# crispitagorico/sigkernel

Hardware: AMD Instinct MI355X
Metric: Gram entries/sec (fp64) (higher is better)
Workload: dtype f64; 1 GPU; BASELINE configs[2]: batch 512x512, len 128, dim 8, LinearKernel, dyadic 1, fp64, compute_Gram sym=False; step=compute_Gram, batch_x=512, rows_per_gpu=512, batch_y=512, len_x=128, len_y=128, dim=8, static_kernel=linear, dyadic_order=1, parallelism=SigKernel(process_group): gram rows sharded over 1 GPU(s), 1 all-gather per Gram

## Files before the change

include/sigkernel_amd.h:

```cpp
#ifndef SIGKERNEL_AMD_H
#define SIGKERNEL_AMD_H

#include <stddef.h>
#include <stdint.h>

#ifdef __cplusplus
extern "C" {
#endif

typedef enum sk_status {
    SK_OK = 0,
    SK_ERR_BAD_ARG = 1,
    SK_ERR_UNSUPPORTED = 2,
    SK_ERR_LAUNCH = 3,
    SK_ERR_WORKSPACE = 4,
    SK_ERR_NO_DEVICE = 5
} sk_status;

#define SK_SCHEME_DEFAULT 0
#define SK_SCHEME_NAIVE 1

#define SK_FLAG_NONE 0
#define SK_FLAG_EXACT 1
#define SK_FLAG_SIMPLE 2
// ... 50 lines not shown
int sk_static_adjoint_f64(int kind, double param, const double *X, const double *Y, const double *W, int64_t ldw,
                          const double *scale, int64_t A, int64_t B, int M, int N, int D, double *out, void *stream);
int sk_static_adjoint_f32(int kind, double param, const float *X, const float *Y, const float *W, int64_t ldw,
                          const float *scale, int64_t A, int64_t B, int M, int N, int D, float *out, void *stream);

int sk_static_adjoint_param_f64(int kind, double param, const double *X, const double *Y, const double *W, int64_t ldw,
                                const double *scale, int64_t A, int64_t B, int M, int N, int D, double *out_dX, double *out_partials,
                                int64_t *n_partials, void *stream);

int sk_linear_adjoint_f64(const double *dYt, int64_t ldy, const double *W, int64_t ldw, const double *scale, int64_t A,
                          int64_t B, int Mc, int Nc, int D, double *out, void *stream);
int sk_linear_adjoint_f32(const double *dYt, int64_t ldy, const float *W, int64_t ldw, const float *scale, int64_t A, int64_t B,
                          int Mc, int Nc, int D, float *out, void *stream);

int sk_linear_adjoint_fused_f64(const double *dXr, const double *dYt, int64_t A, int64_t B, int Mrows, int Mc, int Nc, int Ncp,
                                int dyadic, int scheme, const double *edges, const double *scale, double *tpart,
                                size_t tpart_doubles, double *err, double *ypart, size_t ypart_doubles, int *ppg_out, int *rows_out,
                                int *ycols_out, const double *kfinal, double screen, double tol, void *rescue_ws,
                                size_t rescue_ws_bytes, void *stream);

int sk_rbf_adjoint_fused_f64(const double *Xr, const double *Yt, int64_t A, int64_t B, int Mrows, int Mc, int Nc, int Ncp, int D,
                             int dyadic, int scheme, double sigma, const double *edges, const double *scale, double *gpart,
                             size_t gpart_doubles, double *err, double *ypart, size_t ypart_doubles, int *ppg_out, int *rows_out,
                             int *outw_out, int *ycols_out, const double *kfinal, double screen, double tol, void *rescue_ws,
                             size_t rescue_ws_bytes, void *stream);

size_t sk_solve_deriv_static_workspace_bytes(int64_t P, int Mc, int Nc, int dyadic, int D, int *mrows);
int sk_solve_deriv_static_f64(int kind, double param, const double *X0r, const double *X1r, const double *X2r, const double *Yt, int64_t A,
                              int64_t B, int Mrows, int Mc, int Nc, int Ncp, int D, int fd, int dyadic, int scheme, double eps, double *out_k,
                              double *out_kd, double *out_kdd, void *workspace, size_t workspace_bytes, void *stream);

int sk_rbf_adjoint_fused_mb_layout(int64_t P, int Mc, int Nc, int dyadic, int D, int *mrows, int *rows, int *outw, int *ncols,
                                   int64_t *edge_doubles, size_t *workspace_bytes);
int sk_rbf_adjoint_fused_mb_f64(const double *Xr, const void *Yt, int yt_f32, int64_t A, int64_t B, int Mrows, int Mc, int Nc, int Ncp, int D, int fd,
                                int dyadic, int scheme, double sigma, const double *edges, const double *scale, double *gpart,
                                size_t gpart_doubles, double *n0, size_t n0_doubles, double *err, void *workspace, size_t workspace_bytes,
                                const double *yt64, const double *kfinal, double screen, double tol, void *rescue_ws, size_t rescue_ws_bytes,
                                void *stream);

int sk_linear_adjoint_fused_mb_layout(int64_t P, int Mc, int Nc, int dyadic, int D, int *mrows, int *rows, int *outw, int64_t *edge_doubles,
                                      size_t *workspace_bytes);
int sk_linear_adjoint_fused_mb_f64(const double *dXr, const double *dYt, int64_t A, int64_t B, int Mrows, int Mc, int Nc, int Ncp, int D, int fd,
                                   int dyadic, int scheme, const double *edges, const double *scale, double *gpart, size_t gpart_doubles,
                                   double *err, void *workspace, size_t workspace_bytes, const double *kfinal, double screen, double tol,
                                   void *rescue_ws, size_t rescue_ws_bytes, void *stream);

size_t sk_fused_rescue_workspace_bytes(int kind, int64_t P, int Mc, int Nc, int dyadic, int blocks);

int sk_static_adjoint2_f64(int kind, double param, const double *X, const double *Y, const double *dXr, int Mrows,
                           const double *W, int64_t ldw, const double *scale, int64_t A, int64_t B, int b0, int M, int N, int D,
                           double *out, void *stream);
int sk_static_adjoint2_f32(int kind, double param, const float *X, const float *Y, const double *dXr, int Mrows, const float *W,
                           int64_t ldw, const float *scale, int64_t A, int64_t B, int b0, int M, int N, int D, float *out,
                           void *stream);

int sk_increments_adjoint_f64(const double *W, int64_t ldw, const double *scale, int64_t P, int M, int N, double *dG,
                              void *stream);
int sk_increments_adjoint_f32(const float *W, int64_t ldw, const float *scale, int64_t P, int M, int N, float *dG,
                              void *stream);

int sk_prep_paths_f64(const double *X, int64_t A, int M, int D, int diff, int dim_major, double scale, double *out, int rows, int fd,
                      void *stream);
int sk_prep_paths_f32(const float *X, int64_t A, int M, int D, int diff, int dim_major, double scale, double *out, int rows, int fd,
                      void *stream);
int sk_prep_pair_f64(const double *X, int64_t A, int M, const double *Y, int64_t B, int N, int D, int diff, double scale_x, double scale_y,
                     double *out_x, int rows_x, double *out_y, int rows_y, int fd, void *stream);
int sk_prep_pair_f32(const float *X, int64_t A, int M, const float *Y, int64_t B, int N, int D, int diff, double scale_x, double scale_y,
                     double *out_x, int rows_x, double *out_y, int rows_y, int fd, void *stream);

int sk_solve_fwd_f64(const double *inc_c, int64_t ld, int64_t P, int Mc, int Nc, int dyadic, int scheme, int flags,
                     double *out_final, double *out_grid, double *out_edges, void *stream);
int sk_solve_fwd_f32(const float *inc_c, int64_t ld, int64_t P, int Mc, int Nc, int dyadic, int scheme, int flags,
                     float *out_final, float *out_grid, double *out_edges, void *stream);

int sk_solve_fwd_linear_f64(const double *dXr, const double *dYt, int64_t A, int64_t B, int Mrows, int Mc, int Nc, int Ncp, int D,
                            int dyadic, int scheme, double *out_final, void *queue, void *stream);
int sk_solve_fwd_linear_f32(const double *dXr, const double *dYt, int64_t A, int64_t B, int Mrows, int Mc, int Nc, int Ncp, int D,
                            int dyadic, int scheme, float *out_final, void *queue, void *stream);

int sk_solve_fwd_rbf_f64(const double *Xr, const double *Yt, int64_t A, int64_t B, int Mrows, int Mc, int Nc, int Ncp, int D,
                         int dyadic, int scheme, double inv_sigma, double *out_final, void *queue, void *stream);
int sk_solve_fwd_rbf_f32(const double *Xr, const double *Yt, int64_t A, int64_t B, int Mrows, int Mc, int Nc, int Ncp, int D,
                         int dyadic, int scheme, double inv_sigma, float *out_final, void *queue, void *stream);
int sk_solve_prefix_linear_f64(const double *dXr, const double *dYt, int64_t A, int64_t B, int Mrows, int Mc, int Nc, int Ncp, int D,
                               int dyadic, int scheme, double *out, int64_t ldo, void *queue, void *stream);
int sk_solve_prefix_linear_f32(const double *dXr, const double *dYt, int64_t A, int64_t B, int Mrows, int Mc, int Nc, int Ncp, int D,
                               int dyadic, int scheme, float *out, int64_t ldo, void *queue, void *stream);
int sk_solve_prefix_rbf_f64(const double *Xr, const double *Yt, int64_t A, int64_t B, int Mrows, int Mc, int Nc, int Ncp, int D,
                            int dyadic, int scheme, double inv_sigma, double *out, int64_t ldo, void *queue, void *stream);
int sk_solve_prefix_rbf_f32(const double *Xr, const double *Yt, int64_t A, int64_t B, int Mrows, int Mc, int Nc, int Ncp, int D,
                            int dyadic, int scheme, double inv_sigma, float *out, int64_t ldo, void *queue, void *stream);
#define SK_NODES_ALL 0
#define SK_NODES_DIAGONAL 1
#define SK_NODES_LAST_ROW 2
#define SK_NODES_LAST_COL 3
int sk_solve_prefix_nodes_linear_f64(const double *dXr, const double *dYt, int64_t A, int64_t B, int Mrows, int Mc, int Nc, int Ncp, int D,
                                     int dyadic, int scheme, int nodes, double *out, int64_t ldo, void *queue, void *stream);
int sk_solve_prefix_nodes_linear_f32(const double *dXr, const double *dYt, int64_t A, int64_t B, int Mrows, int Mc, int Nc, int Ncp, int D,
                                     int dyadic, int scheme, int nodes, float *out, int64_t ldo, void *queue, void *stream);
int sk_solve_prefix_nodes_rbf_f64(const double *Xr, const double *Yt, int64_t A, int64_t B, int Mrows, int Mc, int Nc, int Ncp, int D,
                                  int dyadic, int scheme, double inv_sigma, int nodes, double *out, int64_t ldo, void *queue, void *stream);
int sk_solve_prefix_nodes_rbf_f32(const double *Xr, const double *Yt, int64_t A, int64_t B, int Mrows, int Mc, int Nc, int Ncp, int D,
                                  int dyadic, int scheme, double inv_sigma, int nodes, float *out, int64_t ldo, void *queue, void *stream);
#define SK_NODES_AT 4
int sk_solve_prefix_at_linear_f64(const double *dXr, const double *dYt, int64_t A, int64_t B, int Mrows, int Mc, int Nc, int Ncp, int D,
                                  int dyadic, int scheme, const int *len_x, const int *len_y, double *out, void *queue, void *stream);
int sk_solve_prefix_at_linear_f32(const double *dXr, const double *dYt, int64_t A, int64_t B, int Mrows, int Mc, int Nc, int Ncp, int D,
                                  int dyadic, int scheme, const int *len_x, const int *len_y, float *out, void *queue, void *stream);
int sk_solve_prefix_at_rbf_f64(const double *Xr, const double *Yt, int64_t A, int64_t B, int Mrows, int Mc, int Nc, int Ncp, int D,
                               int dyadic, int scheme, double inv_sigma, const int *len_x, const int *len_y, double *out, void *queue,
                               void *stream);
int sk_solve_prefix_at_rbf_f32(const double *Xr, const double *Yt, int64_t A, int64_t B, int Mrows, int Mc, int Nc, int Ncp, int D,
                               int dyadic, int scheme, double inv_sigma, const int *len_x, const int *len_y, float *out, void *queue,
                               void *stream);
int sk_truncated_gram_f64(const double *Xr, const double *Yt, int64_t A, int64_t B, int Mrows, int M, int N, int Ncp, int D, int fd,
                          int num_levels, int order, const double *sigma, double *out, void *stream);
int sk_truncated_gram_f32(const double *Xr, const double *Yt, int64_t A, int64_t B, int Mrows, int M, int N, int Ncp, int D, int fd,
                          int num_levels, int order, const double *sigma, float *out, void *stream);
int sk_truncated_paired_f64(const double *Xr, const double *Yt, int64_t P, int Mrows, int M, int N, int Ncp, int D, int fd, int num_levels,
                            int order, const double *sigma, double *out, void *stream);
int sk_truncated_paired_f32(const double *Xr, const double *Yt, int64_t P, int Mrows, int M, int N, int Ncp, int D, int fd, int num_levels,
                            int order, const double *sigma, float *out, void *stream);
int sk_truncated_levels_f64(const double *Xr, const double *Yt, int64_t A, int64_t B, int Mrows, int M, int N, int Ncp, int D, int fd,
                            int num_levels, int order, double *out, void *stream);
int sk_truncated_levels_f32(const double *Xr, const double *Yt, int64_t A, int64_t B, int Mrows, int M, int N, int Ncp, int D, int fd,
                            int num_levels, int order, float *out, void *stream);
int sk_truncated_levels_paired_f64(const double *Xr, const double *Yt, int64_t P, int Mrows, int M, int N, int Ncp, int D, int fd,
                                   int num_levels, int order, double *out, void *stream);
int sk_truncated_levels_paired_f32(const double *Xr, const double *Yt, int64_t P, int Mrows, int M, int N, int Ncp, int D, int fd,
                                   int num_levels, int order, float *out, void *stream);
int sk_truncated_points_f64(const double *Xr, const double *Yt, int64_t A, int64_t B, int Mrows, int M, int N, int Ncp, int D, int fd,
                            int num_levels, int order, int kind, double param, int paired, int levels, const double *sigma, double *out,
                            void *stream);
int sk_truncated_points_f32(const double *Xr, const double *Yt, int64_t A, int64_t B, int Mrows, int M, int N, int Ncp, int D, int fd,
                            int num_levels, int order, int kind, double param, int paired, int levels, const double *sigma, float *out,
                            void *stream);
int sk_truncated_long_plan(int64_t A, int64_t B, int M, int N, int D, int num_levels, int paired, size_t workspace_bytes, int64_t *plan);
int sk_truncated_long_f64(const double *Xr, const double *Yt, int64_t A, int64_t B, int Mrows, int M, int N, int Ncp, int D, int fd,
                          int num_levels, int order, int paired, int levels, const double *sigma, double *slab, size_t slab_bytes, double *out,
                          void *stream);
int sk_truncated_long_f32(const double *Xr, const double *Yt, int64_t A, int64_t B, int Mrows, int M, int N, int Ncp, int D, int fd,
                          int num_levels, int order, int paired, int levels, const double *sigma, double *slab, size_t slab_bytes, float *out,
                          void *stream);
int sk_truncated_long_adjoint_plan(int64_t A, int64_t B, int M, int N, int D, int num_levels, int paired, size_t workspace_bytes,
                                   int64_t *plan);
int sk_truncated_long_adjoint(const double *Xr, const double *Yt, int64_t A, int64_t B, int Mrows, int M, int N, int Ncp, int D, int fd,
                              int num_levels, const double *w, double *Tpart, int64_t n_chunks, double *slab, size_t slab_bytes, void *stream,
                              int paired);
int sk_truncated_wide_adjoint_plan(int64_t A, int64_t B, int M, int N, int D, int num_levels, int paired, size_t workspace_bytes,
                                   int64_t *plan);
int sk_truncated_wide_adjoint(const double *Xr, const double *Yt, int64_t A, int64_t B, int Mrows, int M, int N, int Ncp, int D, int fd,
                              int num_levels, const double *w, double *Tpart, int64_t n_chunks, double *slab, size_t slab_bytes, void *stream,
                              int paired);
int sk_truncated_adjoint_plan(int64_t A, int64_t B, int M, int N, int D, int num_levels, int paired, size_t workspace_bytes, int64_t *plan);
int sk_truncated_adjoint(const double *Xr, const double *Yt, int64_t A, int64_t B, int Mrows, int M, int N, int Ncp, int D, int fd,
                         int num_levels, const double *w, double *Tpart, int64_t n_chunks, double *slab, size_t slab_bytes, void *stream,
                         int paired);
int sk_truncated_points_adjoint_plan(int64_t A, int64_t B, int M, int N, int D, int num_levels, int paired, size_t workspace_bytes,
                                     int64_t *plan);
int sk_truncated_points_adjoint(const double *Xr, const double *Yt, int64_t A, int64_t B, int Mrows, int M, int N, int Ncp, int D, int fd,
                                int num_levels, double param, const double *w, double *Tpart, int64_t n_chunks, double *slab,
                                size_t slab_bytes, void *stream, int paired);
int sk_solve_fwd_linear_sym_f64(const double *dXr, const double *dXt, const int *pair_tab, int64_t A, int Mrows, int Mc, int Nc, int Ncp, int D, int dyadic,
                                int scheme, double *out, void *queue, void *stream);
int sk_solve_fwd_linear_sym_f32(const double *dXr, const double *dXt, const int *pair_tab, int64_t A, int Mrows, int Mc, int Nc, int Ncp, int D, int dyadic,
                                int scheme, float *out, void *queue, void *stream);
// ... 79 lines not shown
```

sigkernel_amd/_lib.py:

```python
import ctypes
import os

import torch

from ._routes import routes

_HERE = os.path.dirname(os.path.abspath(__file__))
LIB_PATH = os.path.join(_HERE, "libsigkernel_amd.so")

SK_OK = 0
OP_FORWARD, OP_ADJOINT, OP_ADJOINT_SYM, OP_PREFIX, OP_TRUNCATED, OP_TRUNCATED_ADJOINT, OP_TRUNCATED_RBF = 0, 1, 2, 3, 4, 5, 6
OP_TRUNCATED_RBF_ADJOINT = 7
OP_TRUNCATED_LONG = 8
OP_TRUNCATED_LONG_ADJOINT = 9
OP_TRUNCATED_WIDE_ADJOINT = 10
ROUTE_STREAM, ROUTE_FUSED, ROUTE_FUSED_MB, ROUTE_FUSED_MB_SWAP, ROUTE_FUSED_SWAP = 0, 1, 2, 3, 4
ROUTE_NO_STREAM = 1
ROUTE_NO_SWAP = 2
SCHEME_DEFAULT = 0
SCHEME_NAIVE = 1
FLAG_EXACT = 1
FLAG_SIMPLE = 2
FLAG_FAST_ONLY = 4
FLAG_EDGES_GIVEN = 8
FLAG_DISCRETE = 16
FLAG_RAGGED = 32
FLAG_SOURCES = 64
PREFIX_NODES = {"all": 0, "diagonal": 1, "last_row": 2, "last_col": 3}


def prefix_nodes_len(nodes, M, N):
    return {"diagonal": min(M, N), "last_row": N, "last_col": M}[nodes]

_lib = None

_vp = ctypes.c_void_p
_i64 = ctypes.c_int64
_int = ctypes.c_int
_sz = ctypes.c_size_t

SIGNATURES = {
    "sk_version": (_int, []),
    "sk_build_info": (ctypes.c_char_p, []),
    "sk_route_query": (_int, [_int, _int, _int, _int, _int, _int, _int, _int, _int]),
    "sk_cost_query": (ctypes.c_double, [_int]),
    "sk_cost_name": (ctypes.c_char_p, [_int]),
    "sk_cost_note": (ctypes.c_char_p, [_int]),
    "sk_solve_fwd_static_cols": (_int, [_int, _int]),
    "sk_reload_knobs": (None, []),
    "sk_launch_trace": (_int, [_int]),
    "sk_launch_trace_dump": (ctypes.c_size_t, [ctypes.c_char_p, ctypes.c_size_t, _int]),
    "sk_linear_prescale": (ctypes.c_double, [_int]),
    "sk_pair_div_magic": (_int, [_i64, ctypes.POINTER(ctypes.c_uint32), ctypes.POINTER(ctypes.c_int)]),
    "sk_status_string": (ctypes.c_char_p, [_int]),
    "sk_device_count": (_int, []),
    "sk_increments_f64": (_int, [_vp, _i64, _int, _int, _vp, _i64, _vp]),
    "sk_increments_f32": (_int, [_vp, _i64, _int, _int, _vp, _i64, _vp]),
    "sk_static_increments_f64": (_int, [_int, ctypes.c_double, _vp, _vp, _i64, _i64, _int, _int, _int, _vp, _i64, _vp]),
    "sk_static_increments_f32": (_int, [_int, ctypes.c_double, _vp, _vp, _i64, _i64, _int, _int, _int, _vp, _i64, _vp]),
    "sk_static_adjoint_f64": (_int, [_int, ctypes.c_double, _vp, _vp, _vp, _i64, _vp, _i64, _i64, _int, _int, _int, _vp, _vp]),
    "sk_static_adjoint_f32": (_int, [_int, ctypes.c_double, _vp, _vp, _vp, _i64, _vp, _i64, _i64, _int, _int, _int, _vp, _vp]),
    "sk_static_adjoint_param_f64": (_int, [_int, ctypes.c_double, _vp, _vp, _vp, _i64, _vp, _i64, _i64, _int, _int, _int, _vp, _vp,
                                           ctypes.POINTER(ctypes.c_int64), _vp]),
    "sk_linear_adjoint_f64": (_int, [_vp, _i64, _vp, _i64, _vp, _i64, _i64, _int, _int, _int, _vp, _vp]),
    "sk_linear_adjoint_f32": (_int, [_vp, _i64, _vp, _i64, _vp, _i64, _i64, _int, _int, _int, _vp, _vp]),
    "sk_static_adjoint2_f64": (_int, [_int, ctypes.c_double, _vp, _vp, _vp, _int, _vp, _i64, _vp, _i64, _i64, _int, _int, _int, _int,
                                      _vp, _vp]),
    "sk_static_adjoint2_f32": (_int, [_int, ctypes.c_double, _vp, _vp, _vp, _int, _vp, _i64, _vp, _i64, _i64, _int, _int, _int, _int,
                                      _vp, _vp]),
    "sk_increments_adjoint_f64": (_int, [_vp, _i64, _vp, _i64, _int, _int, _vp, _vp]),
    "sk_increments_adjoint_f32": (_int, [_vp, _i64, _vp, _i64, _int, _int, _vp, _vp]),
    "sk_solve_fwd_f64": (_int, [_vp, _i64, _i64, _int, _int, _int, _int, _int, _vp, _vp, _vp, _vp]),
    "sk_solve_fwd_f32": (_int, [_vp, _i64, _i64, _int, _int, _int, _int, _int, _vp, _vp, _vp, _vp]),
    "sk_solve_fwd_linear_f64": (_int, [_vp, _vp, _i64, _i64, _int, _int, _int, _int, _int, _int, _int, _vp, _vp, _vp]),
    "sk_solve_fwd_linear_f32": (_int, [_vp, _vp, _i64, _i64, _int, _int, _int, _int, _int, _int, _int, _vp, _vp, _vp]),
    "sk_solve_fwd_rbf_f64": (_int, [_vp, _vp, _i64, _i64, _int, _int, _int, _int, _int, _int, _int, ctypes.c_double, _vp, _vp, _vp]),
    "sk_solve_fwd_rbf_f32": (_int, [_vp, _vp, _i64, _i64, _int, _int, _int, _int, _int, _int, _int, ctypes.c_double, _vp, _vp, _vp]),
    "sk_solve_prefix_linear_f64": (_int, [_vp, _vp, _i64, _i64, _int, _int, _int, _int, _int, _int, _int, _vp, _i64, _vp, _vp]),
    "sk_solve_prefix_linear_f32": (_int, [_vp, _vp, _i64, _i64, _int, _int, _int, _int, _int, _int, _int, _vp, _i64, _vp, _vp]),
    "sk_solve_prefix_rbf_f64": (_int, [_vp, _vp, _i64, _i64, _int, _int, _int, _int, _int, _int, _int, ctypes.c_double, _vp, _i64, _vp, _vp]),
    "sk_solve_prefix_rbf_f32": (_int, [_vp, _vp, _i64, _i64, _int, _int, _int, _int, _int, _int, _int, ctypes.c_double, _vp, _i64, _vp, _vp]),
    "sk_solve_prefix_nodes_linear_f64": (_int, [_vp, _vp, _i64, _i64, _int, _int, _int, _int, _int, _int, _int, _int, _vp, _i64, _vp, _vp]),
    "sk_solve_prefix_nodes_linear_f32": (_int, [_vp, _vp, _i64, _i64, _int, _int, _int, _int, _int, _int, _int, _int, _vp, _i64, _vp, _vp]),
    "sk_solve_prefix_nodes_rbf_f64": (_int, [_vp, _vp, _i64, _i64, _int, _int, _int, _int, _int, _int, _int, ctypes.c_double, _int, _vp, _i64, _vp, _vp]),
    "sk_solve_prefix_nodes_rbf_f32": (_int, [_vp, _vp, _i64, _i64, _int, _int, _int, _int, _int, _int, _int, ctypes.c_double, _int, _vp, _i64, _vp, _vp]),
    "sk_solve_prefix_at_linear_f64": (_int, [_vp, _vp, _i64, _i64, _int, _int, _int, _int, _int, _int, _int, _vp, _vp, _vp, _vp, _vp]),
    "sk_solve_prefix_at_linear_f32": (_int, [_vp, _vp, _i64, _i64, _int, _int, _int, _int, _int, _int, _int, _vp, _vp, _vp, _vp, _vp]),
    "sk_solve_prefix_at_rbf_f64": (_int, [_vp, _vp, _i64, _i64, _int, _int, _int, _int, _int, _int, _int, ctypes.c_double, _vp, _vp, _vp, _vp, _vp]),
    "sk_solve_prefix_at_rbf_f32": (_int, [_vp, _vp, _i64, _i64, _int, _int, _int, _int, _int, _int, _int, ctypes.c_double, _vp, _vp, _vp, _vp, _vp]),
    "sk_truncated_gram_f64": (_int, [_vp, _vp, _i64, _i64, _int, _int, _int, _int, _int, _int, _int, _int, _vp, _vp, _vp]),
    "sk_truncated_gram_f32": (_int, [_vp, _vp, _i64, _i64, _int, _int, _int, _int, _int, _int, _int, _int, _vp, _vp, _vp]),
    "sk_truncated_paired_f64": (_int, [_vp, _vp, _i64, _int, _int, _int, _int, _int, _int, _int, _int, _vp, _vp, _vp]),
    "sk_truncated_paired_f32": (_int, [_vp, _vp, _i64, _int, _int, _int, _int, _int, _int, _int, _int, _vp, _vp, _vp]),
    "sk_truncated_levels_f64": (_int, [_vp, _vp, _i64, _i64, _int, _int, _int, _int, _int, _int, _int, _int, _vp, _vp]),
    "sk_truncated_levels_f32": (_int, [_vp, _vp, _i64, _i64, _int, _int, _int, _int, _int, _int, _int, _int, _vp, _vp]),
    "sk_truncated_levels_paired_f64": (_int, [_vp, _vp, _i64, _int, _int, _int, _int, _int, _int, _int, _int, _vp, _vp]),
    "sk_truncated_levels_paired_f32": (_int, [_vp, _vp, _i64, _int, _int, _int, _int, _int, _int, _int, _int, _vp, _vp]),
    "sk_truncated_points_f64": (_int, [_vp, _vp, _i64, _i64, _int, _int, _int, _int, _int, _int, _int, _int, _int, ctypes.c_double, _int, _int, _vp, _vp, _vp]),
    "sk_truncated_points_f32": (_int, [_vp, _vp, _i64, _i64, _int, _int, _int, _int, _int, _int, _int, _int, _int, ctypes.c_double, _int, _int, _vp, _vp, _vp]),
    "sk_truncated_long_plan": (_int, [_i64, _i64, _int, _int, _int, _int, _int, _sz, _vp]),
    "sk_truncated_long_f64": (_int, [_vp, _vp, _i64, _i64, _int, _int, _int, _int, _int, _int, _int, _int, _int, _int, _vp, _vp, _sz, _vp, _vp]),
    "sk_truncated_long_f32": (_int, [_vp, _vp, _i64, _i64, _int, _int, _int, _int, _int, _int, _int, _int, _int, _int, _vp, _vp, _sz, _vp, _vp]),
    "sk_truncated_adjoint_plan": (_int, [_i64, _i64, _int, _int, _int, _int, _int, _sz, _vp]),
    "sk_truncated_long_adjoint_plan": (_int, [_i64, _i64, _int, _int, _int, _int, _int, _sz, _vp]),
    "sk_truncated_long_adjoint": (_int, [_vp, _vp, _i64, _i64, _int, _int, _int, _int, _int, _int, _int, _vp, _vp, _i64, _vp, _sz, _vp, _int]),
    "sk_truncated_wide_adjoint_plan": (_int, [_i64, _i64, _int, _int, _int, _int, _int, _sz, _vp]),
    "sk_truncated_wide_adjoint": (_int, [_vp, _vp, _i64, _i64, _int, _int, _int, _int, _int, _int, _int, _vp, _vp, _i64, _vp, _sz, _vp, _int]),
    "sk_truncated_adjoint": (_int, [_vp, _vp, _i64, _i64, _int, _int, _int, _int, _int, _int, _int, _vp, _vp, _i64, _vp, _sz, _vp, _int]),
    "sk_truncated_points_adjoint_plan": (_int, [_i64, _i64, _int, _int, _int, _int, _int, _sz, _vp]),
    "sk_truncated_points_adjoint": (_int, [_vp, _vp, _i64, _i64, _int, _int, _int, _int, _int, _int, _int, ctypes.c_double, _vp, _vp, _i64, _vp, _sz,
                                           _vp, _int]),
    "sk_prep_pair_f64": (_int, [_vp, _i64, _int, _vp, _i64, _int, _int, _int, ctypes.c_double, ctypes.c_double, _vp, _int, _vp, _int, _int, _vp]),
    "sk_prep_pair_f32": (_int, [_vp, _i64, _int, _vp, _i64, _int, _int, _int, ctypes.c_double, ctypes.c_double, _vp, _int, _vp, _int, _int, _vp]),
    "sk_solve_fwd_static_workspace_bytes": (_sz, [_int, _i64, _int, _int, _int, _int]),
    "sk_solve_fwd_static_rows": (_int, [_int, _int, _int]),
    "sk_solve_fwd_static_split": (_int, [_int, _i64, _int, _int, _int, _int]),
    "sk_solve_fwd_static_f64": (_int, [_int, ctypes.c_double, _vp, _vp, _i64, _i64, _int, _int, _int, _int, _int, _int, _int, _int, _vp,
                                       _vp, _vp, _sz, _vp]),
    "sk_solve_fwd_static_f32": (_int, [_int, ctypes.c_double, _vp, _vp, _int, _i64, _i64, _int, _int, _int, _int, _int, _int, _int, _int,
                                       _vp, _vp, _vp, _sz, _vp]),
    "sk_solve_deriv_static_workspace_bytes": (_sz, [_i64, _int, _int, _int, _int, _vp]),
    "sk_solve_deriv_static_f64": (_int, [_int, ctypes.c_double, _vp, _vp, _vp, _vp, _i64, _i64, _int, _int, _int, _int, _int, _int, _int, _int,
                                         ctypes.c_double, _vp, _vp, _vp, _vp, _sz, _vp]),
    "sk_linear_adjoint_fused_mb_layout": (_int, [_i64, _int, _int, _int, _int, _vp, _vp, _vp, _vp, _vp]),
    "sk_linear_adjoint_fused_mb_f64": (_int, [_vp, _vp, _i64, _i64, _int, _int, _int, _int, _int, _int, _int, _int, _vp, _vp, _vp, _sz, _vp, _vp,
                                              _sz, _vp, ctypes.c_double, ctypes.c_double, _vp, _sz, _vp]),
    "sk_rbf_adjoint_fused_mb_layout": (_int, [_i64, _int, _int, _int, _int, _vp, _vp, _vp, _vp, _vp, _vp]),
    "sk_rbf_adjoint_fused_mb_f64": (_int, [_vp, _vp, _int, _i64, _i64, _int, _int, _int, _int, _int, _int, _int, _int, ctypes.c_double, _vp, _vp,
                                           _vp, _sz, _vp, _sz, _vp, _vp, _sz, _vp, _vp, ctypes.c_double, ctypes.c_double, _vp, _sz, _vp]),
    "sk_solve_fwd_linear_sym_f64": (_int, [_vp, _vp, _vp, _i64, _int, _int, _int, _int, _int, _int, _int, _vp, _vp, _vp]),
    "sk_solve_fwd_linear_sym_f32": (_int, [_vp, _vp, _vp, _i64, _int, _int, _int, _int, _int, _int, _int, _vp, _vp, _vp]),
    "sk_solve_fwd_rbf_sym_f64": (_int, [_vp, _vp, _vp, _i64, _int, _int, _int, _int, _int, _int, _int, ctypes.c_double, _vp, _vp, _vp]),
    "sk_solve_fwd_rbf_sym_f32": (_int, [_vp, _vp, _vp, _i64, _int, _int, _int, _int, _int, _int, _int, ctypes.c_double, _vp, _vp, _vp]),
    "sk_solve_fwd_rbf_edges_f64": (_int, [_vp, _vp, _i64, _i64, _int, _int, _int, _int, _int, _int, _int, ctypes.c_double, _vp, _vp, _vp, _vp]),
    "sk_solve_fwd_linear_edges_f64": (_int, [_vp, _vp, _i64, _i64, _int, _int, _int, _int, _int, _int, _int, _vp, _vp, _vp, _vp]),
    "sk_linear_adjoint_fused_f64": (_int, [_vp, _vp, _i64, _i64, _int, _int, _int, _int, _int, _int, _vp, _vp, _vp, _sz, _vp, _vp, _sz, _vp,
                                           _vp, _vp, _vp, ctypes.c_double, ctypes.c_double, _vp, _sz, _vp]),
    "sk_rbf_adjoint_fused_f64": (_int, [_vp, _vp, _i64, _i64, _int, _int, _int, _int, _int, _int, _int, ctypes.c_double, _vp, _vp, _vp,
                                        _sz, _vp, _vp, _sz, _vp, _vp, _vp, _vp, _vp, ctypes.c_double, ctypes.c_double, _vp, _sz, _vp]),
    "sk_fused_rescue_workspace_bytes": (_sz, [_int, _i64, _int, _int, _int, _int]),
    "sk_adj_workspace_bytes": (_sz, [_i64, _int, _int, _int, _int, _int]),
    "sk_adj_rescue_slot_bytes": (_sz, [_int, _int, _int]),
    "sk_plan_wave_shares": (_int, [_i64, _int, _i64, _i64, _int, _int, _vp, _vp, _vp]),
    "sk_plan_group_chunks": (_int, [_i64, _i64, _i64, _i64, _int, _int, _int, _i64, _vp, _vp, _vp]),
    "sk_adj_rescue_f64": (_int, [_vp, _i64, _i64, _int, _int, _int, _int, _vp, ctypes.c_double, _vp, _vp, _i64, _vp, _sz, _vp]),
    "sk_adj_rescue_f32": (_int, [_vp, _i64, _i64, _int, _int, _int, _int, _vp, ctypes.c_double, _vp, _vp, _i64, _vp, _sz, _vp]),
    "sk_prep_paths_f64": (_int, [_vp, _i64, _int, _int, _int, _int, ctypes.c_double, _vp, _int, _int, _vp]),
    "sk_prep_paths_f32": (_int, [_vp, _i64, _int, _int, _int, _int, ctypes.c_double, _vp, _int, _int, _vp]),
    "sk_strip_edges_bytes": (_sz, [_i64, _int, _int, _int, _int]),
    "sk_solve_fwd_edges_f64": (_int, [_vp, _i64, _i64, _int, _int, _int, _int, _vp, _vp, _vp]),
    "sk_solve_fwd_edges_f32": (_int, [_vp, _i64, _i64, _int, _int, _int, _int, _vp, _vp, _vp]),
    "sk_solve_adj_f64": (_int, [_vp, _i64, _i64, _int, _int, _int, _int, _int, _vp, _vp, _i64, _vp, _vp, _sz, _vp]),
    "sk_solve_adj_f32": (_int, [_vp, _i64, _i64, _int, _int, _int, _int, _int, _vp, _vp, _i64, _vp, _vp, _sz, _vp]),
    "sk_deriv_increments_f64": (_int, [_vp, _vp, _vp, ctypes.c_double, _i64, _int, _int, _vp, _vp, _vp, _i64, _vp]),
    "sk_deriv_increments_f32": (_int, [_vp, _vp, _vp, ctypes.c_double, _i64, _int, _int, _vp, _vp, _vp, _i64, _vp]),
    "sk_static_deriv_increments_f64": (_int, [_int, ctypes.c_double, _vp, _vp, _vp, _vp, _i64, _i64, _int, _int, _int,
                                              ctypes.c_double, _vp, _vp, _vp, _i64, _vp]),
    "sk_static_deriv_increments_f32": (_int, [_int, ctypes.c_double, _vp, _vp, _vp, _vp, _i64, _i64, _int, _int, _int,
                                              ctypes.c_double, _vp, _vp, _vp, _i64, _vp]),
    "sk_solve_deriv_f64": (_int, [_vp, _vp, _vp, _i64, _i64, _int, _int, _int, _int, _vp, _vp, _vp, _vp]),
# ... 97 lines not shown


def _suffix(t):
    if t.dtype == torch.float64:
        return "f64"
    if t.dtype == torch.float32:
        return "f32"
    raise TypeError("sigkernel_amd supports float64 and float32 tensors, got %s" % t.dtype)


def _dev(t, name):
    if t.device.type != "cuda":
        raise RuntimeError(
            "sigkernel_amd runs on MI355X only: tensor `%s` is on %s; move it to a HIP device "
            "('cuda' in PyTorch-ROCm). There is no CPU fallback." % (name, t.device))
    if not t.is_contiguous():
        raise ValueError("tensor `%s` must be contiguous" % name)
    return t


def _rbf_extra_row(Mc, dyadic):
    rc = 4 >> min(int(dyadic), 2)
    cap = 8 * rc
    while cap < Mc:
        cap *= 2
    return 1 if (cap == Mc and cap < 64 * rc) else 0


def _padded_ld(n, elem_size):
    q = 128 // elem_size
    return (n + q - 1) // q * q


def _row_stride(t, name):
    if t.device.type != "cuda":
        _dev(t, name)
    Mc, Nc = t.shape[-2:]
    if t.dim() >= 2 and t.stride(-1) == 1 and t.stride(-2) >= Nc:
        ld = t.stride(-2)
        expect, ok = Mc * ld, True
        for size, stride in zip(reversed(t.shape[:-2]), reversed(t.stride()[:-2])):
            if size != 1 and stride != expect:
                ok = False
                break
            expect *= size
        if ok:
            return t, ld
    t = t.contiguous()
    return t, Nc


_raw_stream = getattr(torch._C, "_cuda_getCurrentRawStream", None)


def _stream(t):
    if _raw_stream is not None:
        idx = t.device.index
        return _raw_stream(torch.cuda.current_device() if idx is None else idx)
    return torch.cuda.current_stream(t.device).cuda_stream


class _NoGuard:
    def __enter__(self):
        return None

    def __exit__(self, *exc):
        return False


_NO_GUARD = _NoGuard()


def _device(dev):
    idx = dev.index
    if idx is None or idx == torch.cuda.current_device():
        return _NO_GUARD
    return torch.cuda.device(dev)


def _ptr(t):
    return None if t is None else t.data_ptr()


def _queue(dev, pairs=1 << 30):
    return torch.empty(8, dtype=torch.int64, device=dev) if pairs >= 16384 else None


def _prep_paths(X, diff, dim_major, scale, rows, fd=8):
    A, M, D = X.shape
    out = torch.empty((A, fd, rows) if dim_major else (A, rows, fd), dtype=torch.float64, device=X.device)
    fn = getattr(load(), "sk_prep_paths_" + _suffix(X))
    _check(fn(_ptr(X), A, M, D, int(bool(diff)), int(bool(dim_major)), float(scale), _ptr(out), int(rows), int(fd), _stream(X)),
           "sk_prep_paths")
    return out


def _prep_pair(X, Y, diff, scale_x, rows_x, rows_y, fd=8):
    A, M, D = X.shape
    B, N = Y.shape[0], Y.shape[1]
    nx = A * rows_x * fd
    buf = torch.empty(nx + B * fd * rows_y, dtype=torch.float64, device=X.device)
    out_x, out_y = buf[:nx].view(A, rows_x, fd), buf[nx:].view(B, fd, rows_y)
    fn = getattr(load(), "sk_prep_pair_" + _suffix(X))
    _check(fn(_ptr(X), A, M, _ptr(Y), B, N, D, int(bool(diff)), float(scale_x), 1.0, _ptr(out_x), int(rows_x), _ptr(out_y), int(rows_y), int(fd),
              _stream(X)), "sk_prep_pair")
    return out_x, out_y


def _truncated_staging(D, N):
    return (8 if D <= 8 else 16), (N + 15) // 16 * 16


_TRUNCATED_ADJOINTS = {
    "plain": (OP_TRUNCATED_ADJOINT, "sk_truncated_adjoint_plan", "sk_truncated_adjoint"),
    "points": (OP_TRUNCATED_RBF_ADJOINT, "sk_truncated_points_adjoint_plan", "sk_truncated_points_adjoint"),
    "long": (OP_TRUNCATED_LONG_ADJOINT, "sk_truncated_long_adjoint_plan", "sk_truncated_long_adjoint"),
    "wide": (OP_TRUNCATED_WIDE_ADJOINT, "sk_truncated_wide_adjoint_plan", "sk_truncated_wide_adjoint"),
}


class _WorstResidual:
    __slots__ = ("err",)

    def __init__(self, err):
        self.err = err

    def tensor(self):
        return self.err.max()

    def __float__(self):
        return float(self.err.max())


def _pair_gemm_sum(Wv, Yv, scale, gram):
    if not gram:
        T = torch.matmul(Wv, Yv)
        return T * scale[:, None, None] if scale is not None else T
    A, B, R, D = Wv.shape[0], Wv.shape[1], Wv.shape[2], Yv.shape[2]
    step = max(1, int((256 << 20) // max(1, A * R * D * Wv.element_size())))
    T = None
    for b0 in range(0, B, step):
        Tm = torch.matmul(Wv[:, b0:b0 + step], Yv[b0:b0 + step])
        if scale is not None:
            Tm = Tm.mul_(scale[:, b0:b0 + step, None, None])
        T = Tm.sum(1) if T is None else T.add_(Tm.sum(1))
        del Tm
    if T is None:
        T = torch.zeros(A, R, D, dtype=Wv.dtype, device=Wv.device)
    return T


class HipBackend:

    name = "hip"
    last_split_status = None

    @staticmethod
    def route(op, kind, D, M, N, dyadic, naive, elem_size, no_stream=False, no_swap=False):
        return int(load().sk_route_query(int(op), int(kind), int(D), int(M), int(N), int(dyadic), SCHEME_NAIVE if naive else SCHEME_DEFAULT,
                                         int(elem_size), (ROUTE_NO_STREAM if no_stream else 0) | (ROUTE_NO_SWAP if no_swap else 0)))

    def increments(self, G):
        _dev(G, "G")
        M, N = G.shape[-2:]
        P = G.numel() // (M * N)
        ld = _padded_ld(N - 1, G.element_size())
        out = torch.empty(G.shape[:-2] + (M - 1, ld), dtype=G.dtype, device=G.device)
        with _device(G.device):
            fn = getattr(load(), "sk_increments_" + _suffix(G))
            _check(fn(_ptr(G), P, M, N, _ptr(out), ld, _stream(G)), "sk_increments")
        return out[..., : N - 1]

    MAX_FUSED_DIM = 32

    def static_increments(self, kind, param, X, Y, gram):
        _dev(X, "X")
        _dev(Y, "Y")
        A, M, D = X.shape
        B, N = Y.shape[0], Y.shape[1]
        if M < 2 or N < 2:
            return None
        ld = _padded_ld(N - 1, X.element_size())
        shape = (A, B, M - 1, ld) if gram else (A, M - 1, ld)
        out = torch.empty(shape, dtype=X.dtype, device=X.device)
        with _device(X.device):
            fn = getattr(load(), "sk_static_increments_" + _suffix(X))
            _check(fn(int(kind), float(param), _ptr(X), _ptr(Y), A, B if gram else 0, M, N, D, _ptr(out), ld, _stream(X)),
                   "sk_static_increments")
        return out[..., : N - 1]

    def solve_fwd_fused_linear(self, X, Y, scale, dyadic, naive, gram, keep_edges=False):
        _dev(X, "X")
        _dev(Y, "Y")
        A, M, D = X.shape
        B, N = Y.shape[0], Y.shape[1]
        Mc, Nc = M - 1, N - 1
        if D > 8 or dyadic > 2 or Mc < 1 or Nc < 1 or Mc > 64 * (4 >> min(dyadic, 2)):
            return None
        Mrows, Ncp = _stage_rows(0, M, gram), (Nc + 15) // 16 * 16
        dev = X.device
        out = torch.empty((A, B) if gram else (A,), dtype=X.dtype, device=dev)
        scheme = SCHEME_NAIVE if naive else SCHEME_DEFAULT
        lib = load()
        with _device(dev):
            kappa = float(lib.sk_linear_prescale(int(dyadic)))
            dXr, dYt = _prep_pair(X, Y, True, kappa * float(scale) ** 2, Mrows, Ncp)
            if keep_edges and X.dtype == torch.float64 and 0 <= dyadic <= 2:
                P = A * B if gram else A
                nbytes = int(lib.sk_strip_edges_bytes(P, Mc, Nc, int(dyadic), 8))
                if nbytes:
                    edges = torch.empty(nbytes // 8, dtype=torch.float64, device=dev)
                    rc = lib.sk_solve_fwd_linear_edges_f64(_ptr(dXr), _ptr(dYt), A, B if gram else 0, Mrows, Mc, Nc, Ncp, D,
                                                           int(dyadic), scheme, _ptr(out), _ptr(edges), _ptr(_queue(dev, A * B if gram else A)), _stream(X))
                    if rc == SK_OK:
                        return out, edges
                    if rc != 2:
                        _check(rc, "sk_solve_fwd_linear_edges")
            fn = getattr(lib, "sk_solve_fwd_linear_" + _suffix(X))
            rc = fn(_ptr(dXr), _ptr(dYt), A, B if gram else 0, Mrows, Mc, Nc, Ncp, D, int(dyadic), scheme, _ptr(out), _ptr(_queue(dev, A * B if gram else A)), _stream(X))
        if rc == 2:
            return None
        _check(rc, "sk_solve_fwd_linear")
        return (out, None) if keep_edges else out

    def solve_fwd_fused_rbf(self, X, Y, sigma, dyadic, naive, gram, keep_edges=False):
        _dev(X, "X")
        _dev(Y, "Y")
        A, M, D = X.shape
        B, N = Y.shape[0], Y.shape[1]
        Mc, Nc = M - 1, N - 1
        if D > 8 or dyadic > 2 or Mc < 1 or Nc < 1 or M > 64 * (4 >> min(dyadic, 2)) or not float(sigma) > 0:
            return None
        Mrows, Ncp = _stage_rows(1, M, gram), (N + 15) // 16 * 16
        dev = X.device
        out = torch.empty((A, B) if gram else (A,), dtype=X.dtype, device=dev)
        scheme = SCHEME_NAIVE if naive else SCHEME_DEFAULT
        lib = load()
        with _device(dev):
            Xr, Yt = _prep_pair(X, Y, False, 1.0, Mrows, Ncp)
            if keep_edges and X.dtype == torch.float64:
                P = A * B if gram else A
                nbytes = int(lib.sk_strip_edges_bytes(P, Mc + _rbf_extra_row(Mc, dyadic), Nc + (1 if Nc % 16 == 0 else 0), int(dyadic), 8))
                if nbytes:
                    edges = torch.empty(nbytes // 8, dtype=torch.float64, device=dev)
                    rc = lib.sk_solve_fwd_rbf_edges_f64(_ptr(Xr), _ptr(Yt), A, B if gram else 0, Mrows, Mc, Nc, Ncp, D, int(dyadic),
                                                        scheme, 1.0 / float(sigma), _ptr(out), _ptr(edges), _ptr(_queue(dev, A * B if gram else A)), _stream(X))
                    if rc == SK_OK:
                        return out, edges
                    if rc != 2:
                        _check(rc, "sk_solve_fwd_rbf_edges")
            fn = getattr(lib, "sk_solve_fwd_rbf_" + _suffix(X))
            rc = fn(_ptr(Xr), _ptr(Yt), A, B if gram else 0, Mrows, Mc, Nc, Ncp, D, int(dyadic), scheme, 1.0 / float(sigma),
                    _ptr(out), _ptr(_queue(dev, A * B if gram else A)), _stream(X))
        if rc == 2:
            return None
        _check(rc, "sk_solve_fwd_rbf")
        return (out, None) if keep_edges else out

    def solve_prefix_fused(self, kind, param, X, Y, dyadic, naive, gram, out=None, nodes="all"):
        _dev(X, "X")
        _dev(Y, "Y")
        if nodes not in PREFIX_NODES:
            raise ValueError("nodes must be one of %s, not %r" % (", ".join(repr(n) for n in PREFIX_NODES), nodes))
        A, M, D = X.shape
        B, N = Y.shape[0], Y.shape[1]
        Mc, Nc = M - 1, N - 1
        if Mc < 1 or Nc < 1 or (kind == 1 and not float(param) > 0) or \
                self.route(OP_PREFIX, kind, D, M, N, dyadic, naive, X.element_size()) != ROUTE_FUSED:
            return None
        mode = PREFIX_NODES[nodes]
        tail = (M, N) if mode == 0 else (prefix_nodes_len(nodes, M, N),)
        shape = ((A, B) if gram else (A,)) + tail
        if out is None:
            out = torch.empty(shape, dtype=X.dtype, device=X.device)
        if tuple(out.shape) != shape or out.dtype != X.dtype or out.device != X.device:
            raise ValueError("out must be a %s tensor of shape %s on %s" % (X.dtype, shape, X.device))
        if A == 0 or (gram and B == 0):
            return out
        ldo = out.stride(1) if gram else out.stride(0)
        if mode == 0:
            if out.stride(-1) != 1 or out.stride(-2) != N or ldo < M * N or (gram and A > 1 and out.stride(0) != B * ldo):
                raise ValueError("out: every pair's (M, N) grid must be dense and the pairs evenly spaced")
        elif out.stride(-1) != 1 or ldo < tail[0] or (gram and A > 1 and out.stride(0) != B * ldo):
            raise ValueError("out: every pair's slice must be dense and the pairs evenly spaced")
        Mrows = _stage_rows(kind, M, gram)
        Ncp = ((Nc if kind == 0 else N) + 15) // 16 * 16
        dev = X.device
        scheme = SCHEME_NAIVE if naive else SCHEME_DEFAULT
        lib = load()
        pairs = A * B if gram else A
        which = ("sk_solve_prefix_" if mode == 0 else "sk_solve_prefix_nodes_") + ("linear_" if kind == 0 else "rbf_") + _suffix(X)
        sel = () if mode == 0 else (mode,)
        with _device(dev):
            if kind == 0:
                kappa = float(lib.sk_linear_prescale(int(dyadic)))
                dXr, dYt = _prep_pair(X, Y, True, kappa * float(param) ** 2, Mrows, Ncp)
                rc = getattr(lib, which)(_ptr(dXr), _ptr(dYt), A, B if gram else 0, Mrows, Mc, Nc, Ncp, D, int(dyadic), scheme, *sel,
                                         _ptr(out), ldo, _ptr(_queue(dev, pairs)), _stream(X))
            else:
                Xr, Yt = _prep_pair(X, Y, False, 1.0, Mrows, Ncp)
                rc = getattr(lib, which)(_ptr(Xr), _ptr(Yt), A, B if gram else 0, Mrows, Mc, Nc, Ncp, D, int(dyadic), scheme,
                                         1.0 / float(param), *sel, _ptr(out), ldo, _ptr(_queue(dev, pairs)), _stream(X))
        if rc == 2:
            return None
        _check(rc, "sk_solve_prefix")
        if mode == 0:
            out[..., 0, :] = 1
        else:
            out[..., 0] = 1
        return out

    def solve_prefix_at(self, kind, param, X, Y, len_x, len_y, dyadic, naive, gram):
        _dev(X, "X")
        _dev(Y, "Y")
        A, M, D = X.shape
        B, N = Y.shape[0], Y.shape[1]
        Mc, Nc = M - 1, N - 1
        if Mc < 1 or Nc < 1 or (kind == 1 and not float(param) > 0) or \
                self.route(OP_PREFIX, kind, D, M, N, dyadic, naive, X.element_size()) != ROUTE_FUSED:
            return None
        for name, t, n in (("len_x", len_x, A), ("len_y", len_y, B)):
            if t.dtype != torch.int32 or t.device != X.device or tuple(t.shape) != (n,) or not t.is_contiguous():
                raise ValueError("%s must be a contiguous int32 tensor of shape (%d,) on %s" % (name, n, X.device))
        out = torch.ones((A, B) if gram else (A,), dtype=X.dtype, device=X.device)
        if A == 0 or (gram and B == 0):
            return out
        Mrows = _stage_rows(kind, M, gram)
        Ncp = ((Nc if kind == 0 else N) + 15) // 16 * 16
        dev = X.device
        scheme = SCHEME_NAIVE if naive else SCHEME_DEFAULT
        lib = load()
        pairs = A * B if gram else A
        fn = getattr(lib, "sk_solve_prefix_at_" + ("linear_" if kind == 0 else "rbf_") + _suffix(X))
        with _device(dev):
            if kind == 0:
                kappa = float(lib.sk_linear_prescale(int(dyadic)))
# ... 1057 lines not shown
```

sigkernel_amd/csrc/sk_abi.hip:

```cpp
#include <algorithm>
#include <atomic>
#include <cstdlib>
#include <cstring>
#include <mutex>
#include <string>
#include <unordered_map>
#include <utility>
#include <vector>

#include "sk_internal.h"
#include "sk_wave_common.h"

using namespace sk;

namespace {

bool bad_common(const void *inc, int64_t P, int Mc, int Nc, int dyadic, int scheme, int flags) {
    if (!inc || P < 0 || Mc < 1 || Nc < 1 || dyadic < 0 || dyadic > 16) return true;
    if (scheme != SK_SCHEME_DEFAULT && scheme != SK_SCHEME_NAIVE) return true;
    if (flags & ~(SK_FLAG_EXACT | SK_FLAG_SIMPLE | SK_FLAG_FAST_ONLY | SK_FLAG_EDGES_GIVEN)) return true;
    if ((flags & SK_FLAG_EDGES_GIVEN) && (flags & (SK_FLAG_EXACT | SK_FLAG_SIMPLE))) return true;
    if ((flags & SK_FLAG_FAST_ONLY) && (flags & (SK_FLAG_EXACT | SK_FLAG_SIMPLE))) return true;
    if (((int64_t)Mc << dyadic) > (1 << 24) || ((int64_t)Nc << dyadic) > (1 << 24)) return true;
    return false;
// ... 133 lines not shown
template <typename TO>
int solve_prefix_at(int kind, const double *Xr, const double *Yt, int64_t A, int64_t B, int Mrows, int Mc, int Nc, int Ncp, int D, int dyadic,
                    int scheme, double inv_sigma, const int *len_x, const int *len_y, TO *out, void *queue, void *stream) {
    if (D < 1 || !Xr || !Yt || !out || A < 0 || B < 0 || Mc < 1 || Nc < 1 || dyadic < 0 || dyadic > 16) return SK_ERR_BAD_ARG;
    if (scheme != SK_SCHEME_DEFAULT && scheme != SK_SCHEME_NAIVE) return SK_ERR_BAD_ARG;
    if (kind == 1 && (!(inv_sigma > 0.0) || !(inv_sigma < 1e300))) return SK_ERR_BAD_ARG;
    if (!len_x || !len_y) return SK_ERR_BAD_ARG;
    if (A == 0) return SK_OK;
    const Geom g = make_geom(B > 0 ? A * B : A, Mc, Nc, dyadic, scheme);
    return launch_fwd_prefix<TO>(kind, Xr, Yt, A, B, Mrows, Ncp, D, g, inv_sigma, out, 1, queue, (hipStream_t)stream, SK_NODES_AT, len_x, len_y);
}

template <typename TO>
int truncated(const double *Xr, const double *Yt, int64_t A, int64_t B, int Mrows, int M, int N, int Ncp, int D, int fd, int num_levels,
              int order, const double *sigma, TO *out, void *stream, int paired, int levels, int kind = 0, double param = 0.0,
              bool long_mode = false, double *slab = nullptr, size_t slab_bytes = 0) {
    if (paired) B = A;
    if ((kind != 0 && kind != 1) || (long_mode && kind) || (kind == 1 && (!(param > 0.0) || !(param < 1e300)))) return SK_ERR_BAD_ARG;
    if (D < 1 || !Xr || !Yt || !out || (!sigma && !levels) || A < 0 || B < 0 || M < 1 || N < 1 || num_levels < 1 || Mrows < M || Ncp < N ||
        fd < D || (slab_bytes && !slab))
        return SK_ERR_BAD_ARG;
    if (A == 0 || B == 0) return SK_OK;
    if (long_mode)
        return launch_truncated_long<TO>(Xr, Yt, A, B, Mrows, M, N, Ncp, D, fd, num_levels, order, sigma, out, (hipStream_t)stream, paired, levels,
                                         slab, slab_bytes);
    return launch_truncated<TO>(Xr, Yt, A, B, Mrows, M, N, Ncp, D, fd, num_levels, order, sigma, out, (hipStream_t)stream, paired, levels, kind,
                                param);
}

int truncated_adjoint_plan_abi(int mode, int64_t A, int64_t B, int M, int N, int D, int num_levels, int paired, size_t workspace_bytes,
                               int64_t *plan, bool block_entry) {
    if (!plan || A < 1 || B < 1 || M < 1 || N < 1 || D < 1 || num_levels < 1) return SK_ERR_BAD_ARG;
    size_t block = 0;
    const int rc = truncated_adjoint_plan(mode, A, B, M, N, D, num_levels, paired, workspace_bytes, plan, plan + 1, &block);
    if (rc == SK_OK) {
        plan[2] = plan[1] * (int64_t)block;
        if (block_entry) plan[3] = (int64_t)block;
    }
    return rc;
}

int truncated_adjoint_abi(int mode, const double *Xr, const double *Yt, int64_t A, int64_t B, int Mrows, int M, int N, int Ncp, int D, int fd,
                          int num_levels, double param, const double *w, double *Tpart, int64_t n_chunks, double *slab, size_t slab_bytes,
                          void *stream, int paired, bool pairs_must_match, bool slab_required, bool param_required) {
    if (paired && !pairs_must_match) B = A;
    if (D < 1 || !Xr || !Yt || !w || !Tpart || A < 0 || B < 0 || M < 1 || N < 1 || num_levels < 1 || Mrows < M || Ncp < N || fd < D ||
        (slab_required ? !slab || !slab_bytes : slab_bytes && !slab) || (paired && A != B) || (param_required && !(param > 0.0)))
        return SK_ERR_BAD_ARG;
    if (A == 0 || B == 0) return SK_OK;
    return launch_truncated_adjoint(mode, Xr, Yt, A, B, Mrows, M, N, Ncp, D, fd, num_levels, param, w, Tpart, n_chunks, slab, slab_bytes,
                                    (hipStream_t)stream, paired);
}

}

namespace sk {
namespace {
int knob_int(const char *name) {
    const char *v = getenv(name);
    return v && *v ? atoi(v) : 0;
}
RankW knob_shares(const char *name) {
    RankW r{};
    const char *e = getenv(name);
    if (e && *e)
        for (const char *q = e; *q && r.n < 4; ++r.n) {
            r.w[r.n] = atof(q);
            while (*q && *q != ',') ++q;
            if (*q == ',') ++q;
        }
    return r;
}
Knobs parse_knobs() {
    Knobs k{};
    k.wave_wpc = knob_int("SK_WAVE_WPC"); k.wave_wpb = knob_int("SK_WAVE_WPB");
    k.adj_wpc = knob_int("SK_ADJ_WPC"); k.adj_wpb = knob_int("SK_ADJ_WPB");
    k.adjf_wpc = knob_int("SK_ADJF_WPC"); k.adjf_wpb = knob_int("SK_ADJF_WPB");
    k.adjr_wpc = knob_int("SK_ADJR_WPC"); k.adjr_wpb = knob_int("SK_ADJR_WPB");
    k.adjmb_wpc = knob_int("SK_ADJMB_WPC"); k.adjmb_wpb = knob_int("SK_ADJMB_WPB"); k.adjmb_q_static = knob_int("SK_ADJMB_Q_STATIC");
    k.derivf_wpc = knob_int("SK_DERIVF_WPC"); k.derivf_wpb = knob_int("SK_DERIVF_WPB"); k.derivf_noshift = knob_int("SK_DERIVF_NOSHIFT");
    k.deriv_wpc = knob_int("SK_DERIV_WPC"); k.deriv_wpb = knob_int("SK_DERIV_WPB");
    k.fused_wpc = knob_int("SK_FUSED_WPC"); k.fused_wpb = knob_int("SK_FUSED_WPB"); k.fused_q_static = knob_int("SK_FUSED_Q_STATIC");
    k.fused_mid = getenv("SK_FUSED_MID") ? knob_int("SK_FUSED_MID") : 1;
    k.fusedmb_wpc = knob_int("SK_FUSEDMB_WPC"); k.fusedmb_wpb = knob_int("SK_FUSEDMB_WPB"); k.fusedmb_q_static = knob_int("SK_FUSEDMB_Q_STATIC");
    k.fusedmb_split = getenv("SK_FUSEDMB_SPLIT") ? knob_int("SK_FUSEDMB_SPLIT") : 1;
    k.fusedmb_lead = knob_int("SK_FUSEDMB_LEAD");
    k.prefix_store = knob_int("SK_PREFIX_STORE");
    k.rank_w = knob_shares("SK_RANK_W"); k.wave_rank_w = knob_shares("SK_WAVE_RANK_W"); k.adj_rank_w = knob_shares("SK_ADJ_RANK_W");
    k.adjf_rank_w = knob_shares("SK_ADJF_RANK_W"); k.adjr_rank_w = knob_shares("SK_ADJR_RANK_W");
    k.deriv_rank_w = knob_shares("SK_DERIV_RANK_W"); k.fused_rank_w = knob_shares("SK_FUSED_RANK_W");
    k.fusedmb_rank_w = knob_shares("SK_FUSEDMB_RANK_W");
    return k;
}
Knobs g_knobs = parse_knobs();
std::atomic<int> g_cu_count[16];
std::atomic<int> g_trace{knob_int("SK_TRACE_LAUNCHES") != 0 ? 1 : 0};
std::mutex g_trace_mu;
std::unordered_map<const void *, unsigned long long> g_trace_counts;
}
const Knobs &knobs() { return g_knobs; }
bool trace_on() { return g_trace.load(std::memory_order_relaxed) != 0; }
void trace_launch(const void *host_stub) {
    std::lock_guard<std::mutex> lock(g_trace_mu);
    g_trace_counts[host_stub] += 1;
}
int device_cu_count() {
    int dev = 0;
    if (hipGetDevice(&dev) != hipSuccess || dev < 0 || dev >= 16) return 256;
    int n = g_cu_count[dev].load(std::memory_order_relaxed);
    if (n == 0) {
        int v = 0;
        n = hipDeviceGetAttribute(&v, hipDeviceAttributeMultiprocessorCount, dev) == hipSuccess && v > 0 ? v : 256;
        g_cu_count[dev].store(n, std::memory_order_relaxed);
    }
    return n;
}
}

extern "C" {

int sk_version(void) { return 340; }

int sk_launch_trace(int enable) {
    const int prev = sk::g_trace.load(std::memory_order_relaxed);
    if (enable == 0 || enable == 1) sk::g_trace.store(enable, std::memory_order_relaxed);
    return prev;
}

size_t sk_launch_trace_dump(char *buf, size_t n, int reset) {
    std::string out;
    {
        std::lock_guard<std::mutex> lock(sk::g_trace_mu);
        std::vector<std::pair<std::string, unsigned long long>> rows;
        for (const auto &kv : sk::g_trace_counts) {
            const char *name = hipKernelNameRefByPtr(kv.first, nullptr);
            rows.emplace_back(name ? name : "?", kv.second);
        }
        std::sort(rows.begin(), rows.end());
        for (const auto &r : rows) out += std::to_string(r.second) + "\t" + r.first + "\n";
        if (reset) sk::g_trace_counts.clear();
    }
    if (buf && n) {
        const size_t c = out.size() < n - 1 ? out.size() : n - 1;
        memcpy(buf, out.data(), c);
        buf[c] = 0;
    }
    return out.size() + 1;
}

void sk_reload_knobs(void) { sk::g_knobs = sk::parse_knobs(); }

double sk_linear_prescale(int dyadic) { return dyadic < 0 || dyadic > 16 ? 0.0 : 1.0 / ((double)(1LL << (2 * dyadic)) * 3.4641016151377544); }

int sk_plan_wave_shares(int64_t P, int G, int64_t waves, int64_t resident, int wpb, int n_cu, int64_t *first, int64_t *end, int *ppg) {
    if (P < 0 || G < 1 || waves < 1 || wpb < 1 || n_cu < 1 || !first || !end || !ppg) return SK_ERR_BAD_ARG;
    const sk::RankSplit rs = sk::rank_split(P, G, waves, resident, wpb, n_cu, sk::RankW{});
    for (int64_t w = 0; w < waves; ++w) sk::rank_share(rs, w, G, P, ppg[w], first[w], end[w]);
    return rs.nranks;
}

int sk_plan_group_chunks(int64_t A, int64_t B, int64_t PPG, int64_t max_groups, int G, int wpb, int n_cu, int64_t n_groups,
                         int64_t *first, int64_t *slot, int *ppg) {
    if (A < 1 || B < 0 || PPG < 1 || G < 1 || wpb < 1 || n_cu < 1 || !first || !slot || !ppg) return SK_ERR_BAD_ARG;
    const sk::ChunkSplit cs = sk::chunk_split(A, B, PPG, max_groups, G, wpb, n_cu, sk::RankW{});
    const int64_t P = B > 0 ? A * B : A;
    for (int64_t gi = 0; gi < n_groups; ++gi) sk::chunk_share(cs, gi, A, B, P, first[gi], slot[gi], ppg[gi]);
// ... 52 lines not shown
                                         (hipStream_t)stream);
}
int sk_static_adjoint_f32(int kind, double param, const float *X, const float *Y, const float *W, int64_t ldw,
                          const float *scale, int64_t A, int64_t B, int M, int N, int D, float *out, void *stream) {
    if (!X || !Y || !W || !out || A < 0 || B < 0 || M < 2 || N < 2 || D < 1 || (kind != 0 && kind != 1)) return SK_ERR_BAD_ARG;
    if ((ldw != 0 && ldw < N - 1) || (kind == 1 && !(param > 0))) return SK_ERR_BAD_ARG;
    if (A == 0) return SK_OK;
    return launch_static_adjoint<float>(kind, param, X, Y, W, ldw ? ldw : N - 1, scale, A, B, M, N, D, out,
                                        (hipStream_t)stream);
}

int sk_static_adjoint_param_f64(int kind, double param, const double *X, const double *Y, const double *W, int64_t ldw,
                                const double *scale, int64_t A, int64_t B, int M, int N, int D, double *out_dX, double *out_partials,
                                int64_t *n_partials, void *stream) {
    if (!n_partials || A < 0 || B < 0 || M < 2 || N < 2 || D < 1 || (kind != 0 && kind != 1)) return SK_ERR_BAD_ARG;
    if (kind == 0 || D > 32) return SK_ERR_UNSUPPORTED;
    const int64_t need = static_adjoint_param_partials(A, M, D);
    if (!out_dX && !out_partials) {
        *n_partials = need;
        return SK_OK;
    }
    if (!X || !Y || !W || !out_dX || !out_partials || *n_partials != need) return SK_ERR_BAD_ARG;
    if ((ldw != 0 && ldw < N - 1) || !(param > 0) || out_partials != out_dX + A * (int64_t)M * D) return SK_ERR_BAD_ARG;
    if (A == 0) return SK_OK;
    return launch_static_adjoint_param(param, X, Y, W, ldw ? ldw : N - 1, scale, A, B, M, N, D, out_dX, (hipStream_t)stream);
}

int sk_linear_adjoint_f64(const double *dYt, int64_t ldy, const double *W, int64_t ldw, const double *scale, int64_t A,
                          int64_t B, int Mc, int Nc, int D, double *out, void *stream) {
    if (!dYt || !W || !out || A < 0 || B < 0 || Mc < 1 || Nc < 1 || D < 1 || ldy < Nc || (ldw != 0 && ldw < Nc)) return SK_ERR_BAD_ARG;
    if (A == 0) return SK_OK;
    return launch_linear_adjoint_dyt<double>(dYt, ldy, W, ldw ? ldw : Nc, scale, A, B, Mc, Nc, D, out, (hipStream_t)stream);
}
int sk_linear_adjoint_f32(const double *dYt, int64_t ldy, const float *W, int64_t ldw, const float *scale, int64_t A, int64_t B,
                          int Mc, int Nc, int D, float *out, void *stream) {
    if (!dYt || !W || !out || A < 0 || B < 0 || Mc < 1 || Nc < 1 || D < 1 || ldy < Nc || (ldw != 0 && ldw < Nc)) return SK_ERR_BAD_ARG;
    if (A == 0) return SK_OK;
    return launch_linear_adjoint_dyt<float>(dYt, ldy, W, ldw ? ldw : Nc, scale, A, B, Mc, Nc, D, out, (hipStream_t)stream);
}

int sk_static_adjoint2_f64(int kind, double param, const double *X, const double *Y, const double *dXr, int Mrows,
                           const double *W, int64_t ldw, const double *scale, int64_t A, int64_t B, int b0, int M, int N, int D,
                           double *out, void *stream) {
    if (!W || !out || A < 0 || B < 1 || b0 < 0 || b0 > B || M < 2 || N < 2 || D < 1 || (kind != 0 && kind != 1)) return SK_ERR_BAD_ARG;
    if ((ldw != 0 && ldw < N - 1) || (kind == 1 && (!(param > 0) || !X || !Y)) || (kind == 0 && (!dXr || Mrows < M - 1)))
        return SK_ERR_BAD_ARG;
    if (A == 0) return SK_OK;
    return launch_static_adjoint2<double>(kind, param, X, Y, dXr, Mrows, W, ldw ? ldw : N - 1, scale, A, B, b0, M, N, D, out,
                                          (hipStream_t)stream);
}
int sk_static_adjoint2_f32(int kind, double param, const float *X, const float *Y, const double *dXr, int Mrows, const float *W,
                           int64_t ldw, const float *scale, int64_t A, int64_t B, int b0, int M, int N, int D, float *out,
                           void *stream) {
    if (!W || !out || A < 0 || B < 1 || b0 < 0 || b0 > B || M < 2 || N < 2 || D < 1 || (kind != 0 && kind != 1)) return SK_ERR_BAD_ARG;
    if ((ldw != 0 && ldw < N - 1) || (kind == 1 && (!(param > 0) || !X || !Y)) || (kind == 0 && (!dXr || Mrows < M - 1)))
        return SK_ERR_BAD_ARG;
    if (A == 0) return SK_OK;
    return launch_static_adjoint2<float>(kind, param, X, Y, dXr, Mrows, W, ldw ? ldw : N - 1, scale, A, B, b0, M, N, D, out,
                                         (hipStream_t)stream);
}

int sk_increments_adjoint_f64(const double *W, int64_t ldw, const double *scale, int64_t P, int M, int N, double *dG,
                              void *stream) {
    if (!W || !dG || P < 0 || M < 2 || N < 2 || (ldw != 0 && ldw < N - 1)) return SK_ERR_BAD_ARG;
    if (P == 0) return SK_OK;
    return launch_increments_adjoint<double>(W, ldw ? ldw : N - 1, scale, P, M, N, dG, (hipStream_t)stream);
}
int sk_increments_adjoint_f32(const float *W, int64_t ldw, const float *scale, int64_t P, int M, int N, float *dG,
                              void *stream) {
    if (!W || !dG || P < 0 || M < 2 || N < 2 || (ldw != 0 && ldw < N - 1)) return SK_ERR_BAD_ARG;
    if (P == 0) return SK_OK;
    return launch_increments_adjoint<float>(W, ldw ? ldw : N - 1, scale, P, M, N, dG, (hipStream_t)stream);
}

int sk_solve_fwd_f64(const double *inc_c, int64_t ld, int64_t P, int Mc, int Nc, int dyadic, int scheme, int flags, double *out_final,
                     double *out_grid, double *out_edges, void *stream) {
    return solve_fwd<double>(inc_c, ld, P, Mc, Nc, dyadic, scheme, flags, out_final, out_grid, out_edges, stream);
}
int sk_solve_fwd_f32(const float *inc_c, int64_t ld, int64_t P, int Mc, int Nc, int dyadic, int scheme, int flags, float *out_final,
                     float *out_grid, double *out_edges, void *stream) {
    return solve_fwd<float>(inc_c, ld, P, Mc, Nc, dyadic, scheme, flags, out_final, out_grid, out_edges, stream);
}

int sk_solve_fwd_linear_f64(const double *dXr, const double *dYt, int64_t A, int64_t B, int Mrows, int Mc, int Nc, int Ncp, int D,
                            int dyadic, int scheme, double *out_final, void *queue, void *stream) {
    if (D < 1 || !dXr || !dYt || !out_final || A < 0 || B < 0 || Mc < 1 || Nc < 1 || dyadic < 0 || dyadic > 16) return SK_ERR_BAD_ARG;
    if (scheme != SK_SCHEME_DEFAULT && scheme != SK_SCHEME_NAIVE) return SK_ERR_BAD_ARG;
    if (A == 0) return SK_OK;
    const Geom g = make_geom(B > 0 ? A * B : A, Mc, Nc, dyadic, scheme);
    return launch_fwd_fused_linear<double>(dXr, dYt, A, B, Mrows, Ncp, D, g, out_final, nullptr, queue, (hipStream_t)stream);
}
int sk_solve_fwd_linear_f32(const double *dXr, const double *dYt, int64_t A, int64_t B, int Mrows, int Mc, int Nc, int Ncp, int D,
                            int dyadic, int scheme, float *out_final, void *queue, void *stream) {
    if (D < 1 || !dXr || !dYt || !out_final || A < 0 || B < 0 || Mc < 1 || Nc < 1 || dyadic < 0 || dyadic > 16) return SK_ERR_BAD_ARG;
    if (scheme != SK_SCHEME_DEFAULT && scheme != SK_SCHEME_NAIVE) return SK_ERR_BAD_ARG;
    if (A == 0) return SK_OK;
    const Geom g = make_geom(B > 0 ? A * B : A, Mc, Nc, dyadic, scheme);
    return launch_fwd_fused_linear<float>(dXr, dYt, A, B, Mrows, Ncp, D, g, out_final, nullptr, queue, (hipStream_t)stream);
}

int sk_solve_fwd_rbf_f64(const double *Xr, const double *Yt, int64_t A, int64_t B, int Mrows, int Mc, int Nc, int Ncp, int D, int dyadic,
                         int scheme, double inv_sigma, double *out_final, void *queue, void *stream) {
    if (D < 1 || !Xr || !Yt || !out_final || A < 0 || B < 0 || Mc < 1 || Nc < 1 || dyadic < 0 || dyadic > 16) return SK_ERR_BAD_ARG;
    if (scheme != SK_SCHEME_DEFAULT && scheme != SK_SCHEME_NAIVE) return SK_ERR_BAD_ARG;
    if (!(inv_sigma > 0.0) || !(inv_sigma < 1e300)) return SK_ERR_BAD_ARG;
    if (A == 0) return SK_OK;
    const Geom g = make_geom(B > 0 ? A * B : A, Mc, Nc, dyadic, scheme);
    return launch_fwd_fused_rbf<double>(Xr, Yt, A, B, Mrows, Ncp, D, g, inv_sigma, out_final, nullptr, queue, (hipStream_t)stream);
}
int sk_solve_fwd_rbf_f32(const double *Xr, const double *Yt, int64_t A, int64_t B, int Mrows, int Mc, int Nc, int Ncp, int D, int dyadic,
                         int scheme, double inv_sigma, float *out_final, void *queue, void *stream) {
    if (D < 1 || !Xr || !Yt || !out_final || A < 0 || B < 0 || Mc < 1 || Nc < 1 || dyadic < 0 || dyadic > 16) return SK_ERR_BAD_ARG;
    if (scheme != SK_SCHEME_DEFAULT && scheme != SK_SCHEME_NAIVE) return SK_ERR_BAD_ARG;
    if (!(inv_sigma > 0.0) || !(inv_sigma < 1e300)) return SK_ERR_BAD_ARG;
    if (A == 0) return SK_OK;
    const Geom g = make_geom(B > 0 ? A * B : A, Mc, Nc, dyadic, scheme);
    return launch_fwd_fused_rbf<float>(Xr, Yt, A, B, Mrows, Ncp, D, g, inv_sigma, out_final, nullptr, queue, (hipStream_t)stream);
}

int sk_solve_prefix_linear_f64(const double *dXr, const double *dYt, int64_t A, int64_t B, int Mrows, int Mc, int Nc, int Ncp, int D,
                               int dyadic, int scheme, double *out, int64_t ldo, void *queue, void *stream) {
    return solve_prefix<double>(0, dXr, dYt, A, B, Mrows, Mc, Nc, Ncp, D, dyadic, scheme, 0.0, out, ldo, queue, stream);
}
int sk_solve_prefix_linear_f32(const double *dXr, const double *dYt, int64_t A, int64_t B, int Mrows, int Mc, int Nc, int Ncp, int D,
                               int dyadic, int scheme, float *out, int64_t ldo, void *queue, void *stream) {
    return solve_prefix<float>(0, dXr, dYt, A, B, Mrows, Mc, Nc, Ncp, D, dyadic, scheme, 0.0, out, ldo, queue, stream);
}
int sk_truncated_gram_f64(const double *Xr, const double *Yt, int64_t A, int64_t B, int Mrows, int M, int N, int Ncp, int D, int fd,
                          int num_levels, int order, const double *sigma, double *out, void *stream) {
    return truncated<double>(Xr, Yt, A, B, Mrows, M, N, Ncp, D, fd, num_levels, order, sigma, out, stream, 0, 0);
}
int sk_truncated_gram_f32(const double *Xr, const double *Yt, int64_t A, int64_t B, int Mrows, int M, int N, int Ncp, int D, int fd,
                          int num_levels, int order, const double *sigma, float *out, void *stream) {
    return truncated<float>(Xr, Yt, A, B, Mrows, M, N, Ncp, D, fd, num_levels, order, sigma, out, stream, 0, 0);
}
int sk_truncated_paired_f64(const double *Xr, const double *Yt, int64_t P, int Mrows, int M, int N, int Ncp, int D, int fd, int num_levels,
                            int order, const double *sigma, double *out, void *stream) {
    return truncated<double>(Xr, Yt, P, P, Mrows, M, N, Ncp, D, fd, num_levels, order, sigma, out, stream, 1, 0);
}
int sk_truncated_paired_f32(const double *Xr, const double *Yt, int64_t P, int Mrows, int M, int N, int Ncp, int D, int fd, int num_levels,
                            int order, const double *sigma, float *out, void *stream) {
    return truncated<float>(Xr, Yt, P, P, Mrows, M, N, Ncp, D, fd, num_levels, order, sigma, out, stream, 1, 0);
}
int sk_truncated_levels_f64(const double *Xr, const double *Yt, int64_t A, int64_t B, int Mrows, int M, int N, int Ncp, int D, int fd,
                            int num_levels, int order, double *out, void *stream) {
    return truncated<double>(Xr, Yt, A, B, Mrows, M, N, Ncp, D, fd, num_levels, order, nullptr, out, stream, 0, 1);
}
int sk_truncated_levels_f32(const double *Xr, const double *Yt, int64_t A, int64_t B, int Mrows, int M, int N, int Ncp, int D, int fd,
                            int num_levels, int order, float *out, void *stream) {
    return truncated<float>(Xr, Yt, A, B, Mrows, M, N, Ncp, D, fd, num_levels, order, nullptr, out, stream, 0, 1);
}
int sk_truncated_levels_paired_f64(const double *Xr, const double *Yt, int64_t P, int Mrows, int M, int N, int Ncp, int D, int fd,
                                   int num_levels, int order, double *out, void *stream) {
    return truncated<double>(Xr, Yt, P, P, Mrows, M, N, Ncp, D, fd, num_levels, order, nullptr, out, stream, 1, 1);
}
int sk_truncated_levels_paired_f32(const double *Xr, const double *Yt, int64_t P, int Mrows, int M, int N, int Ncp, int D, int fd,
                                   int num_levels, int order, float *out, void *stream) {
    return truncated<float>(Xr, Yt, P, P, Mrows, M, N, Ncp, D, fd, num_levels, order, nullptr, out, stream, 1, 1);
}
int sk_truncated_points_f64(const double *Xr, const double *Yt, int64_t A, int64_t B, int Mrows, int M, int N, int Ncp, int D, int fd,
                            int num_levels, int order, int kind, double param, int paired, int levels, const double *sigma, double *out, void *stream) {
    return truncated<double>(Xr, Yt, A, B, Mrows, M, N, Ncp, D, fd, num_levels, order, sigma, out, stream, paired, levels, kind, param);
}
int sk_truncated_points_f32(const double *Xr, const double *Yt, int64_t A, int64_t B, int Mrows, int M, int N, int Ncp, int D, int fd,
                            int num_levels, int order, int kind, double param, int paired, int levels, const double *sigma, float *out, void *stream) {
    return truncated<float>(Xr, Yt, A, B, Mrows, M, N, Ncp, D, fd, num_levels, order, sigma, out, stream, paired, levels, kind, param);
}
int sk_truncated_long_plan(int64_t A, int64_t B, int M, int N, int D, int num_levels, int paired, size_t workspace_bytes, int64_t *plan) {
    if (!plan || A < 1 || B < 1 || M < 1 || N < 1 || D < 1 || num_levels < 1) return SK_ERR_BAD_ARG;
    size_t block = 0;
    const int rc = truncated_long_plan(A, B, M, N, D, num_levels, paired, workspace_bytes, plan, &block);
    if (rc == SK_OK) {
        plan[1] = (int64_t)block;
        plan[2] = plan[0] * (int64_t)block;
    }
    return rc;
}
int sk_truncated_long_f64(const double *Xr, const double *Yt, int64_t A, int64_t B, int Mrows, int M, int N, int Ncp, int D, int fd,
                          int num_levels, int order, int paired, int levels, const double *sigma, double *slab, size_t slab_bytes, double *out,
                          void *stream) {
    return truncated<double>(Xr, Yt, A, B, Mrows, M, N, Ncp, D, fd, num_levels, order, sigma, out, stream, paired, levels, 0, 0.0, true, slab, slab_bytes);
}
int sk_truncated_long_f32(const double *Xr, const double *Yt, int64_t A, int64_t B, int Mrows, int M, int N, int Ncp, int D, int fd,
                          int num_levels, int order, int paired, int levels, const double *sigma, double *slab, size_t slab_bytes, float *out,
                          void *stream) {
    return truncated<float>(Xr, Yt, A, B, Mrows, M, N, Ncp, D, fd, num_levels, order, sigma, out, stream, paired, levels, 0, 0.0, true, slab, slab_bytes);
}
int sk_truncated_adjoint_plan(int64_t A, int64_t B, int M, int N, int D, int num_levels, int paired, size_t workspace_bytes, int64_t *plan) {
    return truncated_adjoint_plan_abi(TR_ADJOINT, A, B, M, N, D, num_levels, paired, workspace_bytes, plan, false);
}
int sk_truncated_adjoint(const double *Xr, const double *Yt, int64_t A, int64_t B, int Mrows, int M, int N, int Ncp, int D, int fd,
                         int num_levels, const double *w, double *Tpart, int64_t n_chunks, double *slab, size_t slab_bytes, void *stream,
                         int paired) {
    return truncated_adjoint_abi(TR_ADJOINT, Xr, Yt, A, B, Mrows, M, N, Ncp, D, fd, num_levels, 0.0, w, Tpart, n_chunks, slab, slab_bytes, stream,
                                 paired, false, false, false);
}
int sk_truncated_long_adjoint_plan(int64_t A, int64_t B, int M, int N, int D, int num_levels, int paired, size_t workspace_bytes,
                                   int64_t *plan) {
    return truncated_adjoint_plan_abi(TR_LONG_ADJOINT, A, B, M, N, D, num_levels, paired, workspace_bytes, plan, true);
}
// ... 434 lines not shown
```

sigkernel_amd/csrc/sk_internal.h:

```cpp
#pragma once
#include <hip/hip_runtime.h>
#include <stdint.h>
#include "../../include/sigkernel_amd.h"

namespace sk {

struct RankW { int n; double w[4]; };
struct Knobs {
    int wave_wpc, wave_wpb;
    int adj_wpc, adj_wpb;
    int adjf_wpc, adjf_wpb;
    int adjr_wpc, adjr_wpb;
    int adjmb_wpc, adjmb_wpb, adjmb_q_static;
    int derivf_wpc, derivf_wpb, derivf_noshift;
    int deriv_wpc, deriv_wpb;
    int fused_wpc, fused_wpb, fused_q_static, fused_mid;
    int fusedmb_wpc, fusedmb_wpb, fusedmb_q_static, fusedmb_split, fusedmb_lead;
    int prefix_store;
    RankW rank_w, wave_rank_w, adj_rank_w, adjf_rank_w, adjr_rank_w, deriv_rank_w, fused_rank_w, fusedmb_rank_w;
};
const Knobs &knobs();
double cost_value(int which);
const char *cost_name(int which);
const char *cost_note(int which);
double cost_by_name(const char *name);
int device_cu_count();

bool trace_on();
void trace_launch(const void *host_stub);
#define SK_LAUNCH(kern, ...)                                                   \
    do {                                                                        \
        if (::sk::trace_on()) ::sk::trace_launch((const void *)(kern));         \
        hipLaunchKernelGGL(kern, __VA_ARGS__);                                  \
    } while (0)

struct ChunkSplit {
    int nr;
    int cpr, nch;
    int64_t gpr;
    int size[4];
    int off[4];
    int uneven;
    int ppp;
    int B;
};

struct FusedRescue {
    const double *kfinal;
    double screen, tol;
    void *ws;
    size_t ws_bytes;
};

struct Geom {
    int64_t P;
    int Mc, Nc, dyadic;
    int MM, NN;
    int naive;
    int64_t ld;
};

inline Geom make_geom(int64_t P, int Mc, int Nc, int dyadic, int scheme, int64_t ld = 0) {
    Geom g;
    g.P = P; g.Mc = Mc; g.Nc = Nc; g.dyadic = dyadic;
    g.MM = Mc << dyadic; g.NN = Nc << dyadic;
    g.naive = (scheme == SK_SCHEME_NAIVE);
    g.ld = ld > 0 ? ld : Nc;
    return g;
}

template <typename T>
int launch_fwd_simple(const T *inc_c, const Geom &g, T *out_final, T *out_grid, double *out_edges, hipStream_t s);
template <typename T>
int launch_adj_simple(const T *inc_c, const Geom &g, T *out_final, T *W, int64_t ldw, void *ws, size_t ws_bytes, hipStream_t s,
                      bool discrete = false, bool ragged = false, bool sources = false);
size_t adj_ragged_head_bytes(int64_t P);
template <typename T>
int launch_deriv_simple(const T *inc, const T *inc_d, const T *inc_dd, const Geom &g, T *out_k, T *out_kd, T *out_kdd,
                        hipStream_t s);
template <typename T>
int launch_adj_rescue(const T *inc_c, const Geom &g, const double *err, double tol, T *out_final, T *W, int64_t ldw, void *ws,
                      size_t ws_bytes, hipStream_t s);
size_t adj_simple_workspace_bytes(const Geom &g);
size_t simple_lds_bytes(const Geom &g);

template <typename T>
int launch_fwd_wave(const T *inc_c, int64_t ld, const Geom &g, T *out_final, double *strip_edges, hipStream_t s);

struct Strip {
    int NUp, logL, nb, RC;
    int NNp, MMp;
    bool ok;
};
inline Strip strip_geom(const Geom &g, int elem_size) {
    Strip st{};
    const int CW = 16 / elem_size, DY = g.dyadic;
    st.RC = DY == 0 ? 4 : DY == 1 ? 2 : 1;
    const int NU = (g.Nc + CW - 1) / CW;
    st.NUp = (NU + 7) / 8 * 8;
    st.logL = 3;
    while (st.logL < 6 && (st.RC << st.logL) < g.Mc) ++st.logL;
    int L = 1 << st.logL;
    st.nb = (g.Mc + L * st.RC - 1) / (L * st.RC);
    st.ok = true;
    if (st.nb > 1) {
        while (L > st.NUp && st.logL > 3) { --st.logL; L >>= 1; }
        if (L > st.NUp) st.ok = false;
        st.nb = (g.Mc + L * st.RC - 1) / (L * st.RC);
    }
    st.NNp = (st.NUp * CW) << DY;
    st.MMp = (st.nb * L * st.RC) << DY;
    return st;
}
inline Geom rbf_edge_geom(const Geom &g) {
    Geom e = g;
    if (g.Nc % 16 == 0) { e.Nc += 1; e.NN = e.Nc << e.dyadic; }
    const int rc = g.dyadic == 0 ? 4 : g.dyadic == 1 ? 2 : 1;
    int cap = 8 * rc;
    while (cap < g.Mc) cap *= 2;
    if (cap == g.Mc && cap < 64 * rc) { e.Mc += 1; e.MM = e.Mc << e.dyadic; }
    return e;
}
inline size_t strip_edge_doubles(const Geom &g, int elem_size) {
    const Strip st = strip_geom(g, elem_size);
    return st.ok ? (size_t)st.NNp + (size_t)st.MMp : 0;
}

template <typename T>
int launch_adj_wave(const T *inc_c, int64_t ld, const Geom &g, const double *edges, T *W, int64_t ldw, double *err,
                    hipStream_t s);

template <typename T>
int launch_deriv_wave(const T *inc, const T *inc_d, const T *inc_dd, int64_t ld, const Geom &g, T *out_k, T *out_kd,
                      T *out_kdd, hipStream_t s);

template <typename TO>
int launch_fwd_fused_linear(const double *dXr, const double *dYt, int64_t A, int64_t B, int Mrows, int Ncp, int D, const Geom &g,
                            TO *out, double *strip_edges, void *queue, hipStream_t s, int tri = 0, const int64_t *loss = nullptr);

template <typename TO>
int launch_fwd_fused_rbf(const double *Xr, const double *Yt, int64_t A, int64_t B, int Mrows, int Ncp, int D, const Geom &g,
                         double inv_sigma, TO *out, double *strip_edges, void *queue, hipStream_t s, int tri = 0, const int64_t *loss = nullptr);

template <typename TO>
int launch_fwd_prefix(int kind, const double *dXr, const double *dYt, int64_t A, int64_t B, int Mrows, int Ncp, int D, const Geom &g,
                      double inv_sigma, TO *out, int64_t ldo, void *queue, hipStream_t s, int nodes = 0, const int *len_x = nullptr,
                      const int *len_y = nullptr);
bool prefix_in_scope(int kind, int D, int Mc, int dyadic);

template <typename TO>
int launch_truncated(const double *Xr, const double *Yt, int64_t A, int64_t B, int Mrows, int M, int N, int Ncp, int D, int fd, int L,
                     int order, const double *sigma, TO *out, hipStream_t s, int paired = 0, int levels = 0, int kind = 0, double param = 0.0);
bool truncated_in_scope(int D, int M, int N, int L, int order);
bool truncated_points_in_scope(int D, int M, int N, int L, int order);
int truncated_long_plan(int64_t A, int64_t B, int M, int N, int D, int L, int paired, size_t workspace, int64_t *blocks, size_t *block_bytes);
template <typename TO>
int launch_truncated_long(const double *Xr, const double *Yt, int64_t A, int64_t B, int Mrows, int M, int N, int Ncp, int D, int fd, int L,
                          int order, const double *sigma, TO *out, hipStream_t s, int paired, int levels, double *slab, size_t slab_bytes);
bool truncated_long_in_scope(int D, int M, int N, int L, int order);
int truncated_long_logw(int M, int Ncp, int fd, int paired);
int64_t truncated_long_steps(int D, int M, int N);
enum TruncMode : int { TR_FORWARD = 0, TR_ADJOINT = 1, TR_POINTS = 2, TR_POINTS_ADJOINT = 3, TR_LONG = 4, TR_LONG_ADJOINT = 5, TR_WIDE_ADJOINT = 6 };
int truncated_adjoint_plan(int mode, int64_t A, int64_t B, int M, int N, int D, int L, int paired, size_t workspace, int64_t *n_chunks,
                           int64_t *blocks, size_t *block_bytes);
int launch_truncated_adjoint(int mode, const double *Xr, const double *Yt, int64_t A, int64_t B, int Mrows, int M, int N, int Ncp, int D, int fd,
                             int L, double param, const double *w, double *Tpart, int64_t n_chunks, double *slab, size_t slab_bytes,
                             hipStream_t s, int paired);
bool truncated_adjoint_in_scope(int D, int M, int N, int L, int order);
bool truncated_points_adjoint_in_scope(int D, int M, int N, int L, int order);
bool truncated_long_adjoint_in_scope(int D, int M, int N, int L, int order);
bool truncated_wide_adjoint_in_scope(int D, int M, int N, int L, int order);

template <typename T>
int launch_prep_cat(const T *X, int64_t A, const T *Y, int64_t B, int M, int D, int diff, double scale_rows, double scale_rows2, double *out_rows,
                    double *out_rows2, int rows, double *out_cols, int cols, int FDp, int *pair_tab, int64_t tri_n, hipStream_t s);
int launch_loss_value(const double *out, int64_t A, int64_t B, int with_yy, double *value, double *wb, hipStream_t s);
int launch_loss_weights(int64_t A, int64_t B, const double *grad_out, double *go, hipStream_t s);
int launch_rbf_adjoint_finish(const double *gpart, int64_t A, int64_t chunks, int rows, int outw, const double *X, int M, int D, double sigma,
                              const double *gscale, double *grad, hipStream_t s);
int launch_linear_adjoint_finish(const double *tpart, int64_t A, int64_t chunks, int rows, int M, int D, double scale2, const double *gscale,
                                 double *grad, hipStream_t s);

template <typename TO>
int launch_fwd_fused_mb(int kind, const double *Xr, const void *Yt, int yt_f32, int64_t A, int64_t B, int Mrows, int Ncp, int D,
                        int fd, const Geom &g, double inv_sigma, TO *out, double *edges, void *ws, size_t ws_bytes, hipStream_t s);
size_t fused_mb_workspace_bytes(int kind, int64_t P, int Mc, int Nc, int dyadic, int D);
int fused_mb_split(int kind, int64_t P, int Mc, int Nc, int dyadic, int D);
int fused_mb_rows(int kind, int Mc, int dyadic, bool edges = false);
int fused_mb_cols(int kind, int Nc);

int route_query(int op, int kind, int D, int M, int N, int dyadic, int naive, int elem_size, int flags);

size_t deriv_fused_workspace_bytes(int64_t P, int Mc, int Nc, int dyadic, int D, int *mrows);
int launch_deriv_fused(int kind, const double *X0r, const double *X1r, const double *X2r, const double *Yt, int64_t A, int64_t B, int Mrows,
                       int Ncp, int D, int fd, const Geom &g, double inv_sigma, double eps, double *out_k, double *out_kd, double *out_kdd,
                       void *ws, size_t ws_bytes, hipStream_t s);

bool adj_fused_mb_layout(int64_t P, int Mc, int Nc, int dyadic, int D, int *mrows, int *rows, int *outw, int *ncols, int64_t *edge_doubles,
                         int *nb, int *nup, size_t *ws_bytes, int kind = 1);
int launch_adj_fused_linear_mb(const double *dXr, const double *dYt, int64_t A, int64_t B, int Mrows, int Ncp, int D, int fd, const Geom &g,
                               const double *edges, const double *scale, double *gpart, size_t gpart_doubles, double *err, void *ws,
                               size_t ws_bytes, const FusedRescue *rescue, hipStream_t s);
int launch_adj_fused_rbf_mb(const double *Xr, const void *Yt, int yt_f32, int64_t A, int64_t B, int Mrows, int Ncp, int D, int fd, const Geom &g,
                            double inv_sigma, const double *edges, const double *scale, double *gpart, size_t gpart_doubles, double *n0,
                            size_t n0_doubles, double *err, void *ws, size_t ws_bytes, const FusedRescue *rescue, const double *Yt64,
                            hipStream_t s);

int launch_adj_fused_linear(const double *dXr, const double *dYt, int64_t A, int64_t B, int Mrows, int Ncp, const Geom &g,
                            const double *edges, const double *scale, double *tpart, size_t tpart_doubles, double *err, double *ypart,
                            size_t ypart_doubles, int *ppg_out, int *rows_out, int *ycols_out, const FusedRescue *rescue, hipStream_t s);

template <typename T>
int launch_prep_pair(const T *X, int64_t A, int M, const T *Y, int64_t B, int N, int D, int diff, double scale_x, double scale_y, double *out_x,
                     int rows_x, double *out_y, int rows_y, int FDp, hipStream_t s);
template <typename T>
int launch_prep_paths(const T *X, int64_t A, int M, int D, int diff, int dim_major, double scale, double *out, int rows, int FDp,
                      hipStream_t s);

int launch_adj_fused_rbf(const double *Xr, const double *Yt, int64_t A, int64_t B, int Mrows, int Ncp, int D, const Geom &g,
                         double inv_sigma, const double *edges, const double *scale, double *gpart, size_t gpart_doubles, double *err,
                         double *ypart, size_t ypart_doubles, int want_yside, int *ppg_out, int *rows_out, int *outw_out, int *ycols_out,
                         const FusedRescue *rescue, hipStream_t s);

size_t fused_rescue_workspace_bytes(int kind, int64_t P, int Mc, int Nc, int dyadic, int blocks);
int launch_fused_screen(const double *kfinal, const double *scale, int64_t P, double screen, double *scale_eff, double *err, hipStream_t s);
// ... 112 lines not shown
```

sigkernel_amd/csrc/sk_pair_stream.h:

```cpp
#pragma once
#include "sk_wave_common.h"

namespace sk {
namespace {

__device__ __forceinline__ void lds_read_dims_issue(d2_t (&t)[8], unsigned a_even, unsigned a_odd) {
    asm volatile("ds_read_b128 %0, %8\n\t"
                 "ds_read_b128 %1, %9\n\t"
                 "ds_read_b128 %2, %8 offset:256\n\t"
                 "ds_read_b128 %3, %9 offset:256\n\t"
                 "ds_read_b128 %4, %8 offset:512\n\t"
                 "ds_read_b128 %5, %9 offset:512\n\t"
                 "ds_read_b128 %6, %8 offset:768\n\t"
                 "ds_read_b128 %7, %9 offset:768"
                 : "=&v"(t[0]), "=&v"(t[1]), "=&v"(t[2]), "=&v"(t[3]), "=&v"(t[4]), "=&v"(t[5]), "=&v"(t[6]), "=&v"(t[7])
                 : "v"(a_even), "v"(a_odd)
                 : "memory");
}
__device__ __forceinline__ void lds_read_dims_issue(d2_t (&t)[4], unsigned a_even, unsigned a_odd) {
    asm volatile("ds_read_b128 %0, %4\n\t"
                 "ds_read_b128 %1, %5\n\t"
                 "ds_read_b128 %2, %4 offset:256\n\t"
                 "ds_read_b128 %3, %5 offset:256"
                 : "=&v"(t[0]), "=&v"(t[1]), "=&v"(t[2]), "=&v"(t[3])
// ... 32 lines not shown
}
__device__ __forceinline__ void lds_load_row(d2_t (&r)[2], unsigned a) {
    asm volatile("ds_read_b128 %0, %2\n\tds_read_b128 %1, %2 offset:16" : "+v"(r[0]), "+v"(r[1]) : "v"(a) : "memory");
}

constexpr unsigned NOPAIR = 0xffffffffu;

template <bool TRI, int FD, class PRM>
__device__ __forceinline__ int64_t pair_split(const PRM &prm, int64_t p, bool want_b) {
    if (prm.B <= 0) return p;
    if constexpr (TRI) {
        if (prm.tri) {
            const int *tab = reinterpret_cast<const int *>(prm.dYt + prm.B * (int64_t)FD * prm.Ncp);
            return (int64_t)tab[2 * p + (want_b ? 1 : 0)];
        }
    }
    if (want_b) return (int64_t)((uint32_t)p % (uint32_t)prm.B);
    return (int64_t)((uint32_t)p / (uint32_t)prm.B);
}


constexpr int x_window(int kind, int nd, int rc, bool edges) { return (kind == 0 && nd == 8 && rc == 4 && !edges) ? 4 : 8; }
constexpr int y_slab_pitch(int nd) { return nd * 128; }
constexpr int X_SLOTS = 2;
constexpr int x_row_bytes(int nd) { return nd == 4 ? 32 : 64; }

struct OneBandGeom {
    int NUp, logL, L, G, JMAX, GY;
    bool shy;
    size_t lds_bytes;
    int64_t n_pos;
};
struct OneBandShape {
    int kind, Mc, Nc, Mrows, Ncp, RC, nd;
    bool edges;
    int64_t A, B, P;
    int tri, logL_fixed;
};
inline int one_band_geometry(const OneBandShape &in, OneBandGeom &o) {
    const int NU = in.kind == 1 ? (in.Nc + 2) / 2 : (in.Nc + 1) / 2;
    const int rows = in.kind == 1 ? in.Mc + 1 : in.Mc;
    o.NUp = (NU + LINE_UNITS - 1) / LINE_UNITS * LINE_UNITS;
    if (in.Ncp < o.NUp * 2 || (in.Ncp & 1)) return SK_ERR_UNSUPPORTED;
    o.logL = 3;
    while (o.logL < 6 && (in.RC << o.logL) < rows) ++o.logL;
    if (in.logL_fixed > 0) o.logL = in.logL_fixed;
    o.L = 1 << o.logL;
    if (o.L * in.RC < rows) return SK_ERR_UNSUPPORTED;
    if (in.Mrows < o.L * in.RC) return SK_ERR_UNSUPPORTED;
    o.G = WAVE / o.L;
    o.JMAX = (o.L + o.NUp - 1) / o.NUp;
    o.shy = in.B > 0 && in.tri == 0 && !in.edges && o.G >= 2 && in.A > 0 && in.A <= 0x7fffffff && in.P == in.A * in.B;
    o.GY = o.shy ? 1 : o.G;
    o.lds_bytes = (size_t)o.GY * (((o.L >> 3) + 2) * y_slab_pitch(in.nd)) +
                  (size_t)o.G * (X_SLOTS * o.JMAX * in.RC * x_window(in.kind, in.nd, in.RC, in.edges) * x_row_bytes(in.nd));
    o.n_pos = o.shy ? (in.A + o.G - 1) / o.G * in.B : in.P;
    if (o.lds_bytes > 160 * 1024) return SK_ERR_UNSUPPORTED;
    return SK_OK;
}

inline int div_magic(uint32_t B, unsigned &m, int &shift) {
    if (B < 1 || B >= 0x80000000u) return 1;
    int l = 0;
    while ((1ull << l) < B) ++l;
    const unsigned long long num = 1ull << (31 + l);
    const unsigned long long mm = (num + B - 1) / B;
    if (mm >> 32) return 1;
    m = (unsigned)mm;
    shift = l;
    return 0;
}

inline void even_share(int64_t P, int G, int64_t max_waves, int64_t &waves, int64_t &per) {
    waves = (P + G - 1) / G;
    if (waves > max_waves) waves = max_waves;
    per = (P + waves * G - 1) / (waves * G);
}

struct StreamPlan {
    int64_t waves, per;
    int64_t q_first;
    int C0, n_big, logC;
    bool queue;
};
inline int plan_pair_stream(int64_t P, int G, int NUp, int L, int lag, int waves_per_cu, int n_cu, int pct, bool has_queue, StreamPlan &o) {
    const int64_t max_waves = (int64_t)n_cu * waves_per_cu;
    even_share(P, G, max_waves, o.waves, o.per);
    if (o.per > 0x1fffffff / NUp) return SK_ERR_UNSUPPORTED;
    if (P >= 0x7ff00000LL) return SK_ERR_UNSUPPORTED;
    const int span = (L - 1 + lag + 24) / NUp + 2;
    int logC = 0;
    while ((span >> logC) + 1 > 3) ++logC;
    while ((o.per * (100 - pct) / 100) >> (logC + 1) >= 24 && logC < 8) ++logC;
    o.logC = logC;
    o.queue = has_queue && o.waves == max_waves && o.per >= (8 << logC) && pct < 100;
    if (o.queue) {
        o.C0 = (int)(o.per * pct / 100);
        o.n_big = 0;
        o.q_first = o.waves * G * (int64_t)o.C0;
    } else {
        const int64_t base = P / (o.waves * G), rem = P - base * o.waves * G;
        o.C0 = (int)base;
        o.n_big = (int)((rem + G - 1) / G);
        if (base == 0) o.waves = o.n_big;
        o.q_first = P;
    }
    return SK_OK;
}

}
}
```

sigkernel_amd/csrc/sk_route.hip:

```cpp
#include "sk_internal.h"
#include <cstring>

namespace sk {

namespace {
constexpr int MB_MIN_UNITS = 80;

inline int rc_of(int d) { return d == 0 ? 4 : d == 1 ? 2 : 1; }
inline long mb_steps(int kind, int Mc, int Nc, int d) {
    const int nb = (Mc + 64 * rc_of(d) - 1) / (64 * rc_of(d));
    int nup = ((kind == 1 ? (Nc + 2) / 2 : (Nc + 1) / 2) + 7) / 8 * 8;
    if (nup < MB_MIN_UNITS) nup = MB_MIN_UNITS;
    return (long)nb * nup;
}
inline double mb_efficiency(int kind, int Mc, int Nc, int d, int rc) {
    const int rows = Mc + (kind == 1 ? 1 : 0);
    const int nb = (rows + 64 * rc - 1) / (64 * rc);
    const int nu = kind == 1 ? (Nc + 2) / 2 : (Nc + 1) / 2;
    int nup = (nu + 7) / 8 * 8;
    if (nup < MB_MIN_UNITS) nup = MB_MIN_UNITS;
    return (double)rows / (double)(nb * 64 * rc) * (double)nu / (double)nup;
}
struct CostEntry { const char *name; double value; const char *note; };
const CostEntry COSTS[] = {
    {"mb_min_eff", 0.45,
     "least sweep efficiency rows / (bands 64 RC) x units / max(80, units) at which the multi-band fused kernels are the default instead of the "
     "streaming route (forward and adjoint, LinearKernel and RBFKernel alike); r05_thresholds, 128 x 128 pairs, same box: linear dim 12 d = 0: 128 points "
     "(0.40) 1.38 ms multi-band vs 1.18 streamed, 140 points (0.48) 1.37 vs 2.04; rbf dim 7 d = 0, 140 points (0.48) 1.64 vs 2.06; with a "
     "gradient linear dim 12 d = 1, 140 points (0.48) 7.7 vs 9.0 ms"},
    {"stream_one_strip_cells", 128,
     "... but never while BOTH paths have at most this many increments: there the streaming kernels sweep a pair in one strip and win whatever "
     "the efficiency (r05_thresholds: linear dim 12 d = 1 with a gradient, 128 points (0.79): 4.14 ms multi-band vs 3.52 streamed, 100 points "
     "(0.48) 4.14 vs 2.75; rbf dim 12 d = 1, 128 points 5.99 vs 5.36; rbf dim 7 d = 1, 110 points 3.59 vs 3.27) -- round 4's per-kernel "
     "thresholds (0.5 / 0.9 / never) were this cliff seen through the efficiency"},
    {"mb_min_eff_rbf16_forward", 0.85,
     "the rbf FORWARD with 9..16 dims of fp64 paths (16 staged fp64 dims leave the multi-band kernel one wave per SIMD) needs fuller bands: "
     "r05_thresholds2, 64 x 64 pairs, dim 16: d = 2: 140 points (0.64) 1.25 ms multi-band vs 1.13 streamed, 200 (0.75) 1.95 vs 1.82, 300 (0.93) "
     "3.30 vs 3.46, 512 (1.0) 8.2 vs 11.1; d = 0: 140 (0.48) 0.95 vs 0.79, 300 (0.77) 2.59 vs 2.79; with a gradient the multi-band route wins "
     "from 140 points on (0.77 .. 0.39x) and takes the common threshold"},
    {"mb_swap_steps_ratio", 0.8, "forward: solve k(y, x) when that orientation sweeps at most this share of the macro-steps of k(x, y)"},
    {"sym_tiles", 8, "row blocks of compute_Gram(X, X, sym=True) beyond the one-band triangle launch: (T + 1) / (2 T) of the square is solved; "
     "16 with a gradient on 64 T rows and more (C4: -1 %)"},
    {"sym_min_cells", 5e9,
     "grid cells of K_XX from which the blocked triangle (and, for the loss wrappers, the composition of three Gram calls) beats one launch over "
     "the square / the merged block K(X, [X; Y]): 128 x 128 pairs of 64 points take 0.4 ms in one launch, 0.8 ms in 8 blocks; merged loss "
     "15.1 vs 15.5 ms composed at 512 x 512 (4e9 cells, r04_merged_loss), C4 (2.7e11) 349 ms composed"},
    {"sym_min_rows", 32, "least rows per block of the triangular adjoint: 64 paths of length 700 in 8 blocks of 8 rows: backward 60 -> 74 ms"},
    {"sym_stream_min_paths", 224,
     "compute_Gram(X, X, sym=True) without a gradient on the STREAMING route (wide paths, dyadic >= 3, user-defined kernels): paths from "
     "which the blocked triangle replaces the one block of all pairs whatever the grid -- the node evaluation and the increments are most of a "
     "pair's cost there (r06_sym_stream, rbf dim 20, 64 points, d = 1: 192 paths 0.91x, 256 paths 1.52 -> 1.09 ms, 512 paths 5.76 -> 3.48; "
     "rbf dim 3 d = 3: 192 paths 1.15x, 256 paths 0.84x)"},
    {"paired_merge_cells", 2e9,
     "grid cells of a paired batch below which compute_distance solves k(X, X) and k(X, Y) as ONE batch of 2n pairs (launch- and fill-bound there)"},
    {"mmd_streams_max_pairs", 16384,
     "pairs per Gram matrix up to which a CAPTURED composed compute_mmd forks its three matrices onto three streams (replays 10-15 % faster at 16..64 paths)"},
    {"keep_edges_fraction", 0.5, "share of the transient budget the edges kept between forward and backward may take"},
    {"keep_increments_fraction", 0.125,
     "share of the transient budget the STREAMING route's increments of a one-tile Gram block may keep between forward and backward (beside the edges): "
     "backward then skips the second evaluation of the node kernel -- r06_keep_inc, 256 x 256 pairs of 64 points, forward + backward: rbf dim 20 "
     "5.96 -> 5.02 ms, linear dim 20 3.89 -> 3.23; 2.1 GB held there, 6 GB at most under the default budget"},
    {"loss_launch_free_bytes", 268435456.0,
     "bytes the one-launch loss route (sk_solve_fwd_loss_f64: values, weights, pair table and the rectangle's edges, allocated in one piece and held until "
     "backward) may take without asking the device for its free memory -- hipMemGetInfo costs 20-30 us, a tenth of a 32 + 32-path step; above it the "
     "call is held to keep_edges_fraction of the budget like every other route (ADVICE r5)"},
    {"fused_mid_min_pairs_per_rank", 4,
     "pairs per lane group and rank from which a no-queue fused forward that fills the chip deals out shares by wave age rank: 64-row shard of the "
     "headline Gram 0.695 -> 0.640 ms, 128 + 128 path mmd step 1.237 -> 1.171 ms (r05, same box)"},
    {"fused_static_share_linear", 35,
     "per cent of a lane group's equal share the one-band fused forward deals out before its work queue (SK_FUSED_Q_STATIC overrides): the headline "
     "Gram 4.06 ms at 35, 4.09 at 20, 4.10 at 3, 4.42 at 65, 4.80 at 92 -- waves of a SIMD run at different speeds, the queue evens them out"},
    {"fused_static_share_rbf", 20,
     "... the RBF variants (longer macro-steps, a draw costs less of one): 2048 x 2048 pairs, dyadic 2: 52.0 ms at 35, 50.9 at 20, 50.6 at 3; "
     "512 / 1024 paths: 3.41 -> 3.34, 13.0 -> 12.8 ms; C4 335.6 -> 334.5 (profiles/r05_qstatic.txt)"},
    {"mb_split_max_resident_share", 0.5,
     "few pairs of long paths: bands of a pair on several waves when the pairs fill at most this share of the resident waves (r05: 16 x 16 pairs "
     "of 4096 points 18.7 -> 4.7 ms; 32 x 32 pairs of 700 points 2.18 -> 1.96 ms)"},
    {"mb_split_min_units", 256, "... and a band has at least this many two-column units (second paths of ~512 points): the trailing is cheap, and "
     "a band's first windows never reach into the last chunks of the band above"},
};
constexpr int N_COSTS = (int)(sizeof(COSTS) / sizeof(COSTS[0]));
inline double cost(const char *name) {
    for (int i = 0; i < N_COSTS; ++i)
        if (!strcmp(COSTS[i].name, name)) return COSTS[i].value;
    return 0.0;
}
inline bool prefer_stream(int Mc, int Nc, double eff, bool rbf16_forward = false) {
    const int strip = (int)cost("stream_one_strip_cells");
    if (Mc <= strip && Nc <= strip) return true;
    const double eff_stream = Mc > strip ? (double)Mc / (double)(((Mc + strip - 1) / strip) * strip) : 1.0;
    return eff < cost(rbf16_forward ? "mb_min_eff_rbf16_forward" : "mb_min_eff") * (rbf16_forward ? 1.0 : eff_stream);
}
}

double cost_value(int which) { return which >= 0 && which < N_COSTS ? COSTS[which].value : 0.0; }
const char *cost_name(int which) { return which >= 0 && which < N_COSTS ? COSTS[which].name : nullptr; }
const char *cost_note(int which) { return which >= 0 && which < N_COSTS ? COSTS[which].note : nullptr; }
double cost_by_name(const char *name) { return cost(name); }

int64_t truncated_long_steps(int D, int M, int N) {
    const int fd = D <= 8 ? 8 : 16, Ncp = (N + 15) / 16 * 16;
    const int W = 1 << truncated_long_logw(M, Ncp, fd, 0), Tc = 2048 / fd;
    const int64_t bands = (M + 2 * W - 1) / (2 * W), tiles = (N + Tc - 1) / Tc;
    return bands * (N + tiles * (W - 1)) * W;
}

int route_query(int op, int kind, int D, int M, int N, int d, int naive, int elem_size, int flags) {
    const bool may_stream = !(flags & SK_ROUTE_NO_STREAM);
    if (op == SK_OP_TRUNCATED) {
        if (elem_size != 8 && elem_size != 4) return SK_ROUTE_STREAM;
        if (truncated_in_scope(D, M, N, d, kind)) return SK_ROUTE_FUSED;
        if (!(flags & SK_ROUTE_NO_SWAP) && truncated_in_scope(D, N, M, d, kind)) return SK_ROUTE_FUSED_SWAP;
        return SK_ROUTE_STREAM;
    }
    if (op == SK_OP_TRUNCATED_RBF) {
        if (elem_size != 8 && elem_size != 4) return SK_ROUTE_STREAM;
        if (truncated_points_in_scope(D, M, N, d, kind)) return SK_ROUTE_FUSED;
        if (!(flags & SK_ROUTE_NO_SWAP) && truncated_points_in_scope(D, N, M, d, kind)) return SK_ROUTE_FUSED_SWAP;
        return SK_ROUTE_STREAM;
    }
    if (op == SK_OP_TRUNCATED_ADJOINT) {
        if (elem_size != 8 && elem_size != 4) return SK_ROUTE_STREAM;
        return truncated_adjoint_in_scope(D, M, N, d, kind) ? SK_ROUTE_FUSED : SK_ROUTE_STREAM;
    }
    if (op == SK_OP_TRUNCATED_RBF_ADJOINT) {
        if (elem_size != 8 && elem_size != 4) return SK_ROUTE_STREAM;
        return truncated_points_adjoint_in_scope(D, M, N, d, kind) ? SK_ROUTE_FUSED : SK_ROUTE_STREAM;
    }
    if (op == SK_OP_TRUNCATED_LONG) {
        if (elem_size != 8 && elem_size != 4) return SK_ROUTE_STREAM;
        if (!truncated_long_in_scope(D, M, N, d, kind)) return SK_ROUTE_STREAM;
        if ((flags & SK_ROUTE_NO_SWAP) || truncated_long_steps(D, M, N) <= truncated_long_steps(D, N, M)) return SK_ROUTE_FUSED;
        return SK_ROUTE_FUSED_SWAP;
    }
    if (op == SK_OP_TRUNCATED_LONG_ADJOINT) {
        if (elem_size != 8 && elem_size != 4) return SK_ROUTE_STREAM;
        return truncated_long_adjoint_in_scope(D, M, N, d, kind) ? SK_ROUTE_FUSED : SK_ROUTE_STREAM;
    }
    if (op == SK_OP_TRUNCATED_WIDE_ADJOINT) {
        if (elem_size != 8 && elem_size != 4) return SK_ROUTE_STREAM;
        return truncated_wide_adjoint_in_scope(D, M, N, d, kind) ? SK_ROUTE_FUSED : SK_ROUTE_STREAM;
    }
    if ((kind != 0 && kind != 1) || D < 1 || D > 16 || M < 2 || N < 2 || d < 0 || d > 2) return SK_ROUTE_STREAM;
    if (elem_size != 8 && elem_size != 4) return SK_ROUTE_STREAM;
    const int Mc = M - 1, Nc = N - 1;
    if (op == SK_OP_FORWARD) {
        const int rows = kind == 1 ? M : Mc;
        const bool two_rows = kind == 1 && d == 0 && (D > 4 || naive || elem_size != 8);
        bool one_band = D <= 8 && rows <= 64 * (two_rows ? 2 : rc_of(d));
        if (one_band) return SK_ROUTE_FUSED;
        {
            const int rows_s = kind == 1 ? N : Nc;
            const bool one_band_s = D <= 8 && rows_s <= 64 * (two_rows ? 2 : rc_of(d));
            if (one_band_s) return SK_ROUTE_FUSED_SWAP;
        }
        const bool swap = (double)mb_steps(kind, Nc, Mc, d) <= cost("mb_swap_steps_ratio") * (double)mb_steps(kind, Mc, Nc, d);
        const double eff = swap ? mb_efficiency(kind, Nc, Mc, d, rc_of(d)) : mb_efficiency(kind, Mc, Nc, d, rc_of(d));
// ... 29 lines not shown
```

sigkernel_amd/csrc/sk_wave_fused.hip:

```cpp
#include "sk_pair_stream.h"
#include <algorithm>

namespace sk {
namespace {

constexpr int FD = 8;
struct FusedParams {
    const double *dXr;
    const double *dYt;
    void *out;
    double *edges;
    int64_t P, B;
    int Mrows, Ncp;
    int Mc, Nc, NUp, logL, PPG, n_steps;
    int u_f, lam_f, sel_f, naive;
    double inv_sigma;
    int dims;
    int e_NUp, e_L;
    int tri;
    WaveGroup wg;
    unsigned long long *queue;
    int64_t q_first;
    int C0, logC;
    int n_big;
    int rk_n, rk_wpr;
    unsigned long long rk_cnt;
    int shy_A;
    unsigned div_m;
    int div_s;
};
template <int N>
__device__ __forceinline__ void lds_read_units(d2_t (&v)[N], unsigned addr);
__device__ __forceinline__ void lds_read_half_rows(d2_t (&v)[4], unsigned a) {
    asm volatile("ds_read_b128 %0, %4\n\t"
                 "ds_read_b128 %1, %4 offset:16\n\t"
                 "ds_read_b128 %2, %4 offset:64\n\t"
                 "ds_read_b128 %3, %4 offset:80\n\t"
                 "s_waitcnt lgkmcnt(0)"
                 : "=&v"(v[0]), "=&v"(v[1]), "=&v"(v[2]), "=&v"(v[3])
                 : "v"(a)
                 : "memory");
}
__device__ __forceinline__ void lds_read_line(d2_t (&v)[8], unsigned a) {
    asm volatile("ds_read_b128 %0, %8\n\t"
                 "ds_read_b128 %1, %8 offset:16\n\t"
                 "ds_read_b128 %2, %8 offset:32\n\t"
                 "ds_read_b128 %3, %8 offset:48\n\t"
                 "ds_read_b128 %4, %8 offset:64\n\t"
                 "ds_read_b128 %5, %8 offset:80\n\t"
                 "ds_read_b128 %6, %8 offset:96\n\t"
                 "ds_read_b128 %7, %8 offset:112\n\t"
                 "s_waitcnt lgkmcnt(0)"
                 : "=&v"(v[0]), "=&v"(v[1]), "=&v"(v[2]), "=&v"(v[3]), "=&v"(v[4]), "=&v"(v[5]), "=&v"(v[6]), "=&v"(v[7])
                 : "v"(a)
                 : "memory");
}
template <>
__device__ __forceinline__ void lds_read_units<4>(d2_t (&v)[4], unsigned a) {
    asm volatile("ds_read_b128 %0, %4\n\t"
                 "ds_read_b128 %1, %4 offset:16\n\t"
                 "ds_read_b128 %2, %4 offset:32\n\t"
                 "ds_read_b128 %3, %4 offset:48\n\t"
                 "s_waitcnt lgkmcnt(0)"
                 : "=&v"(v[0]), "=&v"(v[1]), "=&v"(v[2]), "=&v"(v[3])
                 : "v"(a)
                 : "memory");
}

template <typename TO, int DY, bool NAIVE, bool FULLWAVE, bool EDGES, int KIND, int ND, int RCX = 0>
__global__ __launch_bounds__(4 * WAVE) void k_fwd_fused(const FusedParams prm) {
    constexpr bool RBF = KIND == 1;
    constexpr bool AHEAD = !(RBF && EDGES && ND == 8);
    constexpr int LAG = RBF ? 2 : 0;
    constexpr int CW = 2;
    constexpr int RC = RCX ? RCX : Tile<DY>::RC, R = RC << DY, S = CW << DY, r = 1 << DY;
    constexpr int XROW = x_row_bytes(ND);
    constexpr int XW = x_window(KIND, ND, RC, EDGES);
    constexpr int XSLAB = RC * XW * XROW;
    constexpr int Y_SLAB_PITCH = y_slab_pitch(ND);
    extern __shared__ __attribute__((aligned(16))) char lds_block[];
    char *lds;
    const int64_t wave_id = wave_slot(prm.wg, lds_block, lds);
    if (wave_id < 0) return;
    const unsigned lds0 = lds_offset(lds);

    const int lane = threadIdx.x & (WAVE - 1);
    const int L = 1 << prm.logL, G = WAVE >> prm.logL;
    const int lam = lane & (L - 1), grp = lane >> prm.logL;
    const int NUp = prm.NUp;
    const int NSLAB = (L >> 3) + 2;
    const unsigned y_bytes = (unsigned)(NSLAB * Y_SLAB_PITCH);
    const bool shy = !EDGES && !FULLWAVE && prm.shy_A > 0;
    const int GY = shy ? 1 : G;
    auto shy_a = [&]() __attribute__((always_inline)) -> int {
        if (EDGES || FULLWAVE) return 0;
        int v = prm.shy_A;
        asm volatile("" : "+s"(v));
        return v;
    };
    const unsigned x_base0 = (unsigned)GY * y_bytes;
    const double sc = 1.0 / (double)(1 << (2 * DY));
    const double c_half = 0.5 * sc, c_12 = sc * sc / 12.0;

    int u, ps;
    {
        ps = floor_div(-lam, NUp);
        u = -lam - ps * NUp;
    }
    int uk = u, psk = ps;
    if (RBF) {
        psk = floor_div(-lam - LAG, NUp);
        uk = -lam - LAG - psk * NUp;
    }
    int yslab, ypar;
    {
        const int s0 = floor_div(-lam, 8);
        yslab = ((s0 % NSLAB) + NSLAB) % NSLAB;
        ypar = (s0 + (shy ? 0 : grp)) & 1;
    }
    const int my_uf = lam == prm.lam_f ? prm.u_f : -1;
    const int lam7 = lam & 7;
    constexpr bool CUR = EDGES;
    constexpr bool MID = false;
    constexpr bool INFLIGHT_X = !(KIND == 1 && DY == 0 && ND == 8 && RCX == 0);
    int tm = 0, tq = 0;
    int c_u0 = lam % NUp, c_uk0 = (lam + LAG) % NUp;
    int c_out = lam == prm.lam_f ? (lam + LAG + prm.u_f) % NUp : -1;
    int c_kq = floor_div(-lam - LAG, NUp), c_kr = (-lam - LAG) - c_kq * NUp;
    int c_u0m1 = (c_u0 + NUp - 1) % NUp;
    asm volatile("" : "+v"(c_u0), "+v"(c_uk0), "+v"(c_out), "+v"(c_kq), "+v"(c_kr), "+v"(c_u0m1));
    constexpr bool RESET_AT_END = !CUR && !RBF && !FULLWAVE && !MID;
    unsigned a_e;
    constexpr bool CARRY = RESET_AT_END;
    unsigned y_off = 0;
    const unsigned P32 = (unsigned)prm.P;
    auto edge_pairs = [&]() __attribute__((always_inline)) -> unsigned {
        return (prm.tri & 3) == 2 ? (unsigned)((prm.tri >> 2) & 0x7fff) * (unsigned)prm.B : P32;
    };
    const int w32 = __builtin_amdgcn_readfirstlane((int)wave_id);
    int c0_ = prm.C0 + (w32 < prm.n_big ? 1 : 0);
    unsigned cb0_ = (unsigned)(GY * (w32 * prm.C0 + (w32 < prm.n_big ? w32 : prm.n_big)));
    if (prm.rk_n > 0) {
        int rr = w32 / prm.rk_wpr;
        rr = rr >= prm.rk_n ? prm.rk_n - 1 : rr;
        const unsigned long long pk = prm.rk_cnt;
        c0_ = (int)((pk >> (16 * rr)) & 0xffffu);
        const unsigned long long below = pk & ((1ull << (16 * rr)) - 1ull);
        const unsigned used = (unsigned)(below & 0xffffu) + (unsigned)((below >> 16) & 0xffffu) + (unsigned)((below >> 32) & 0xffffu);
        cb0_ = (used * (unsigned)prm.rk_wpr + (unsigned)((w32 - rr * prm.rk_wpr) * c0_)) * (unsigned)GY;
    }
    const int C0 = __builtin_amdgcn_readfirstlane(c0_), logC = prm.logC, CQ = 1 << logC;
    unsigned cb0 = (unsigned)__builtin_amdgcn_readfirstlane((int)cb0_), cb1 = NOPAIR, cb2 = NOPAIR, cb3 = NOPAIR;
    int have = 1;
    int t_end = 0x7fffffff;
    auto ring_at = [&](int kk) __attribute__((always_inline)) -> unsigned {
        return (cb0 & -(unsigned)(kk == 0)) | (cb1 & -(unsigned)(kk == 1)) | (cb2 & -(unsigned)(kk == 2)) | (cb3 & -(unsigned)(kk == 3));
    };
    auto chunk_of = [&](int i, int &off) __attribute__((always_inline)) -> int {
        if (i < C0) { off = i; return 0; }
        off = (i - C0) & (CQ - 1);
        return 1 + ((i - C0) >> logC);
    };
    auto stream_pair_left = [&](int g, int i, int &left) __attribute__((always_inline)) -> unsigned {
        left = 0;
        if (i < 0) return NOPAIR;
        int off;
        const int k = chunk_of(i, off);
        const int size = k == 0 ? C0 : CQ;
        left = size - 1 - off;
        const unsigned b = ring_at(k & 3);
        const unsigned p = b + (unsigned)((shy_a() > 0 ? 0 : g * size) + off);
        return (b >= P32 || p >= P32) ? NOPAIR : p;
    };
    auto stream_pair = [&](int g, int i) __attribute__((always_inline)) -> unsigned {
        int left;
        return stream_pair_left(g, i, left);
    };
    auto lane_pair = [&](int i) __attribute__((always_inline)) -> unsigned {
        int left;
        return stream_pair_left(grp, i, left);
    };
    auto ensure = [&](int f) __attribute__((always_inline)) {
        int off;
        const int kf = chunk_of(f, off);
        while (have <= kf) {
            unsigned b = NOPAIR;
            if (prm.queue && t_end == 0x7fffffff) {
                unsigned long long v = 0;
                if (lane == 0) v = atomicAdd(prm.queue, (unsigned long long)((shy_a() > 0 ? 1 : G) * CQ));
                const unsigned long long q = (unsigned long long)prm.q_first +
                                             (((unsigned long long)(unsigned)__builtin_amdgcn_readfirstlane((int)(v >> 32)) << 32) |
                                              (unsigned)__builtin_amdgcn_readfirstlane((int)v));
                b = q < (unsigned long long)P32 ? (unsigned)q : NOPAIR;
            }
            if (b == NOPAIR && t_end == 0x7fffffff)
                t_end = EDGES ? (C0 + (have - 1) * CQ) * NUp + (L - 1) + LAG
                              : (C0 + (have - 1) * CQ - 1) * NUp + prm.u_f + prm.lam_f + LAG + 1;
            const int kk = have & 3;
            const unsigned m0 = -(unsigned)(kk == 0), m1 = -(unsigned)(kk == 1), m2 = -(unsigned)(kk == 2), m3 = -(unsigned)(kk == 3);
            cb0 = (unsigned)__builtin_amdgcn_readfirstlane((int)((cb0 & ~m0) | (b & m0)));
            cb1 = (unsigned)__builtin_amdgcn_readfirstlane((int)((cb1 & ~m1) | (b & m1)));
            cb2 = (unsigned)__builtin_amdgcn_readfirstlane((int)((cb2 & ~m2) | (b & m2)));
            cb3 = (unsigned)__builtin_amdgcn_readfirstlane((int)((cb3 & ~m3) | (b & m3)));
            have += 1;
        }
    };
    const unsigned long long top_lanes = __builtin_amdgcn_ballot_w64(lam == 0);
    const unsigned my_y = lds0 + (shy ? 0u : (unsigned)grp * y_bytes);
    const unsigned y_lim = my_y + y_bytes;
    unsigned y_flip = 0;
    if constexpr (CARRY) {
        y_flip = shy ? 0u : (unsigned)(grp & 1) << 7;
        asm volatile("" : "+v"(y_flip));
    }
    const unsigned ring_bytes = FULLWAVE ? (unsigned)(((WAVE >> 3) + 2) * Y_SLAB_PITCH) : y_bytes;
    {
        const unsigned ya = my_y + (unsigned)(yslab * Y_SLAB_PITCH + ((-lam & 7) << 4));
        a_e = ya + (unsigned)(ypar << 7);
    }
    const int JMAX = (L + NUp - 1) / NUp;
    const unsigned my_x = lds0 + x_base0 + (unsigned)((grp * X_SLOTS * JMAX) * XSLAB + (lam / NUp) * XSLAB) +
                          (unsigned)((lam & (XW - 1)) * RC * XROW);

    auto div_b = [&](unsigned p) __attribute__((always_inline)) -> unsigned {
        unsigned m = prm.div_m;
        int sh = prm.div_s;
        asm volatile("" : "+s"(m), "+s"(sh));
        return __umulhi(p << 1, m) >> sh;
    };
    auto split_ab = [&](unsigned p, bool want_b) __attribute__((always_inline)) -> int {
        if (prm.B <= 0) return (int)p;
        if (prm.tri) {
            const int *tab = reinterpret_cast<const int *>(prm.dYt + prm.B * (int64_t)FD * prm.Ncp);
            return __builtin_amdgcn_readfirstlane(tab[2 * (int64_t)p + (want_b ? 1 : 0)]);
        }
        const unsigned q = div_b(p);
        return (int)(want_b ? p - q * (unsigned)prm.B : q);
    };
    constexpr bool PARK = !(EDGES && ((KIND == 0 && DY == 0 && ND == 4 && !FULLWAVE) || (KIND == 1 && DY == 2 && ND == 8 && FULLWAVE)));
    int pos_ab = 0;
    auto dma_lane = [&]() __attribute__((always_inline)) -> int {
        int l = lane;
        if constexpr (!PARK) asm volatile("" : "+v"(l));
        return l;
    };
    const int NS = L >> 3;
    int y_pi = 0, y_u0 = 0, y_slot = 0, y_par = 0;
    auto issue_y = [&]() __attribute__((always_inline)) {
        const int gy = shy_a() > 0 ? 1 : G;
        if constexpr (!PARK) pos_ab = 0;
        const int ln = dma_lane();
        if (!PARK || y_u0 == 0) {
            ensure(y_pi);
            for (int g = 0; g < gy; ++g) {
                const unsigned sp = stream_pair(g, y_pi);
                const int b = split_ab(sp == NOPAIR ? 0u : sp, true);
                pos_ab = lane == 8 + g ? b : pos_ab;
            }
        }
        for (int g = 0; g < gy; ++g) {
            const int b = __builtin_amdgcn_readlane(pos_ab, 8 + g);
            const int krow = (ln >> 3) ^ ((y_par + g) & 1);
            const char *src = reinterpret_cast<const char *>(prm.dYt) + (int64_t)b * (FD * 8) * (int64_t)prm.Ncp;
            const unsigned so = ((unsigned)krow * (unsigned)prm.Ncp + (unsigned)(y_u0 + (ln & 7)) * 2u) * 8u;
            if (ND == 8 || ln < 32)
                __builtin_amdgcn_global_load_lds(src + so, (lds_void *)(lds + g * y_bytes + y_slot * Y_SLAB_PITCH), 16, 0, 0);
        }
        y_slot = y_slot + 1 == NSLAB ? 0 : y_slot + 1;
        y_par ^= 1;
        y_u0 += 8;
        if (y_u0 == NUp) { y_u0 = 0; y_pi += 1; }
    };
    int x_q0 = 0, x_lam0 = 0, x_slot = 0;
    auto issue_x = [&]() __attribute__((always_inline)) {
        if constexpr (!PARK) pos_ab = 0;
        const int ln = dma_lane();
        if (!PARK || x_lam0 == 0) {
            ensure(x_q0);
            const int sA = shy_a();
            for (int jd = 0; jd < (PARK ? 1 : JMAX); ++jd) {
                const int at = ((x_q0 - jd) & (NS - 1)) * G;
                int qa = 0;
                for (int g = 0; g < G; ++g) {
                    if (sA <= 0 || g == 0) {
                        const unsigned sp = stream_pair(g, x_q0 - jd);
                        qa = split_ab(sp == NOPAIR ? 0u : sp, false);
                    }
                    int a = qa;
                    if constexpr (!EDGES && !FULLWAVE) {
                        if (sA > 0) {
                            const int64_t ag = (int64_t)qa * G + g;
                            a = ag >= sA ? 0 : (int)ag;
                        }
                    }
                    pos_ab = lane == at + g ? a : pos_ab;
                }
            }
        }
        for (int j = 0; j < JMAX; ++j) {
            const int lamj = x_lam0 + j * NUp;
            if (lamj >= L) break;
            const int at = ((x_q0 - j) & (NS - 1)) * G;
            for (int g = 0; g < G; ++g) {
                const int a = __builtin_amdgcn_readlane(pos_ab, at + g);
                const char *src = reinterpret_cast<const char *>(prm.dXr + ((int64_t)a * prm.Mrows + (int64_t)lamj * RC) * FD);
                char *dst = lds + x_base0 + ((g * X_SLOTS + x_slot) * JMAX + j) * XSLAB;
#pragma unroll
                for (int c = 0; c < (XSLAB + 1023) / 1024; ++c)
                    if (c * 1024 + ln * 16 < XSLAB) {
                        const unsigned so = XROW == 64 ? c * 1024 + ln * 16 : (c * 32 + (ln >> 1)) * 64 + (ln & 1) * 16;
                        __builtin_amdgcn_global_load_lds(src + so, (lds_void *)(dst + c * 1024), 16, 0, 0);
                    }
            }
        }
        x_slot = x_slot + 1 == X_SLOTS ? 0 : x_slot + 1;
        x_lam0 += XW;
        if (x_lam0 == NUp) { x_lam0 = 0; x_q0 += 1; }
    };

    d2_t dxq[RC][ND / 2];
#pragma unroll
    for (int k = 0; k < RC; ++k)
#pragma unroll
        for (int j = 0; j < ND / 2; ++j) dxq[k][j] = d2_t{0.0, 0.0};
    auto load_x_rows = [&](unsigned xa) {
        if constexpr (RC % 2 == 0 && ND == 8) {
#pragma unroll
            for (int k = 0; k < RC; k += 2) lds_load_line(dxq[k], dxq[k + 1], xa + k * 64u);
        } else if constexpr (RC % 2 == 0) {
#pragma unroll
            for (int k = 0; k < RC; k += 2) lds_load_two_half_rows(dxq[k], dxq[k + 1], xa + k * (unsigned)XROW);
        } else {
#pragma unroll
            for (int k = 0; k < RC; ++k) lds_load_row(dxq[k], xa + k * (unsigned)XROW);
        }
    };
    double own[RBF ? RC : 1][6], bel[4];
    constexpr bool PIN_EXP = RBF && !EDGES;
    ExpCoef expc;
    if (PIN_EXP) expc.init();
#pragma unroll
    for (int k = 0; k < (RBF ? RC : 1); ++k)
#pragma unroll
        for (int c = 0; c < 6; ++c) own[k][c] = 1.0;
#pragma unroll
    for (int c = 0; c < 4; ++c) bel[c] = 1.0;
    double left[R], bot[S], ktop[S], corner = 1.0;
#pragma unroll
    for (int i = 0; i < R; ++i) left[i] = 1.0;
#pragma unroll
    for (int i = 0; i < S; ++i) { bot[i] = 1.0; ktop[i] = 1.0; }

    const int EP = EDGES ? (prm.e_NUp * S + prm.e_L * R) : 0;
    int erow_lim = EDGES && lam == prm.lam_f ? prm.e_NUp : 0;
    int ecol_uf = EDGES && lam < prm.e_L ? prm.u_f : -1;
    int ecol_off = EDGES ? prm.e_NUp * S + lam * R : 0;
    asm volatile("" : "+v"(erow_lim), "+v"(ecol_uf), "+v"(ecol_off));
    double *ep_cur = nullptr, *nx_ptr = nullptr;
    int ep_left = 0, nx_left = 0;
    int ep_ok = 0, nx_ok = 0;
    int ep_k = 0;
    auto refresh_next = [&]() __attribute__((always_inline)) {
        if (EDGES) {
            if (ep_k < have) {
                asm volatile("");
                const int size = ep_k == 0 ? C0 : CQ;
                const unsigned b = ring_at(ep_k & 3);
                const unsigned p = b + (unsigned)(grp * size);
                const unsigned ne = edge_pairs();
                const bool ok = b < P32 && p < P32 && p < ne;
                nx_ptr = ok ? prm.edges + (uint64_t)p * (uint64_t)(unsigned)EP : nullptr;
                nx_left = size - 1;
                const unsigned room = ok ? ne - 1u - p : 0u;
                nx_ok = (int)(room < (unsigned)(size - 1) ? room : (unsigned)(size - 1));
            }
        }
    };
    auto sweep_pair_is = [&](int pk) __attribute__((always_inline)) {
        if (EDGES) {
            if (ep_left > 0) {
                ep_left -= 1;
                if (ep_ok > 0) {
                    ep_ok -= 1;
                    ep_cur += EP;
                } else {
                    ep_cur = nullptr;
                }
            } else if (pk >= 0) {
                ep_cur = nx_ptr;
                ep_left = nx_left;
                ep_ok = nx_ok;
                ep_k += 1;
            } else {
                ep_cur = nullptr;
            }
        }
    };
    double *e_ptr = nullptr;
    double erow[S];
    int erow_at = -1, ecol_at = -1;
    const int k_f = (prm.Mc - 1) % RC;
    const bool row_in_bot = k_f == RC - 1;

    d2_t dyn[ND];
    auto read_y = [&]() {
        if constexpr (CUR) {
            const unsigned ya = my_y + (unsigned)(yslab * Y_SLAB_PITCH + ((u & 7) << 4));
            lds_read_dims_issue(dyn, ya + (unsigned)(ypar << 7), ya + (unsigned)((ypar ^ 1) << 7));
        } else {
            lds_read_dims_issue(dyn, a_e, a_e ^ 128u);
        }
    };
    unsigned x_rd_off = 0;
    static_assert(X_SLOTS == 2, "x_rd_off toggles between two slots");
    issue_y();
    issue_x();
    asm volatile("s_waitcnt vmcnt(0)" ::: "memory");
    issue_y();
    issue_x();
    refresh_next();
    sweep_pair_is(psk);
    refresh_next();
    if constexpr (!CUR) {
        if (c_u0 == 0) {
            load_x_rows(my_x);
#pragma unroll
            for (int k = 0; k < RC; ++k) lds_rows_wait(dxq[k]);
        }
    }
    if (AHEAD) read_y();
    double top[S];
#pragma unroll
    for (int i = 0; i < S; ++i) top[i] = 1.0;
    auto take_top = [&]() __attribute__((always_inline)) {
#pragma unroll
        for (int i = 0; i < S; ++i) top[i] = dpp_shr1_zero(bot[i]);
        if constexpr (CARRY) {
            a_e = (unsigned)__builtin_amdgcn_update_dpp((int)a_e, (int)a_e, 0x138 , 0xf, 0xf, false);
            set_one_and_address_in_lanes(top, a_e, y_off, y_flip, my_y, top_lanes);
        } else {
            set_one_in_lanes(top, top_lanes);
        }
    };
    for (int t = 0; t < t_end; ++t) {
        if (EDGES) {
            double *const ep = e_ptr;
            if (erow_at >= 0) {
#pragma unroll
                for (int cc = 0; cc < S; cc += 2) {
                    d2_t v = {row_in_bot ? bot[cc] : erow[cc], row_in_bot ? bot[cc + 1] : erow[cc + 1]};
                    *reinterpret_cast<d2_t *>(ep + erow_at + cc) = v;
                }
            }
            if (ecol_at >= 0) {
#pragma unroll
                for (int rr = 0; rr < R; rr += 2) {
                    d2_t v = {left[rr], left[rr + 1]};
                    *reinterpret_cast<d2_t *>(ep + ecol_at + rr) = v;
                }
            }
        }

        if (FULLWAVE) {
            asm volatile("v_mov_b64 %0, %1" : "=v"(corner) : "v"(ktop[S - 1]));
#pragma unroll
            for (int i = 0; i < S; ++i) {
                ktop[i] = dpp_shr1(bot[i], ktop[i]);
                top[i] = ktop[i];
            }
        } else if constexpr (!RESET_AT_END) {
            take_top();
        }

        if constexpr (RESET_AT_END) {
        } else if constexpr (!CUR) {
            if (tm == (RBF ? c_uk0 : c_u0)) {
                asm volatile("");
                corner = 1.0;
#pragma unroll
                for (int i = 0; i < R; ++i) left[i] = 1.0;
            }
        } else {
            if (RBF && uk == 0) {
                asm volatile("");
                corner = 1.0;
#pragma unroll
                for (int i = 0; i < R; ++i) left[i] = 1.0;
            }
            if (u == 0) {
                if (!RBF) {
                    asm volatile("");
                    corner = 1.0;
#pragma unroll
                    for (int i = 0; i < R; ++i) left[i] = 1.0;
                }
                load_x_rows(my_x + x_rd_off);
#pragma unroll
                for (int k = 0; k < RC; ++k) lds_rows_wait(dxq[k]);
            }
        }

        d2_t dyv[ND];
        if (!AHEAD) read_y();
        lds_dims_wait(dyv, dyn);

        double ca[RC][CW], cbm[RC][CW];
        double ginc[RC][CW];
        if constexpr (RBF) {
#pragma unroll
            for (int k = 0; k < RC; ++k)
#pragma unroll
                for (int q = 0; q < CW; ++q) {
                    double d2 = 0.0;
#pragma unroll
                    for (int j = 0; j < ND; ++j) {
                        const double df = dxq[k][j >> 1][j & 1] - dyv[j][q];
                        d2 = fma(df, df, d2);
                    }
                    const double ex = fma(-d2, prm.inv_sigma, d2 * 0.0);
                    own[k][4 + q] = PIN_EXP ? exp_nonpos(ex, expc) : exp_nonpos(ex);
                }
            bel[2] = dpp_shl1(own[0][4], bel[2]);
            bel[3] = dpp_shl1(own[0][5], bel[3]);
#pragma unroll
            for (int k = 0; k < RC; ++k)
#pragma unroll
                for (int q = 0; q < CW; ++q) {
                    const double t0 = own[k][q], t1 = own[k][q + 1];
                    const double b0 = k + 1 < RC ? own[(k + 1) % RC][q] : bel[q];
                    const double b1 = k + 1 < RC ? own[(k + 1) % RC][q + 1] : bel[q + 1];
                    ginc[k][q] = ((b1 + t0) - b0) - t1;
                }
            if (EDGES) {
#pragma unroll
                for (int k = 0; k < RC; ++k)
#pragma unroll
                    for (int q = 0; q < CW; ++q)
                        if (lam * RC + k >= prm.Mc || uk * CW + q >= prm.Nc) ginc[k][q] = 0.0;
            }
#pragma unroll
            for (int k = 0; k < RC; ++k)
#pragma unroll
                for (int c = 0; c < 4; ++c) { own[k][c] = own[k][c + 2]; asm volatile("" : "+v"(own[k][c])); }
            bel[0] = bel[2];
            bel[1] = bel[3];
            asm volatile("" : "+v"(bel[0]), "+v"(bel[1]));
        } else {
#pragma unroll
            for (int k = 0; k < RC; ++k)
#pragma unroll
                for (int q = 0; q < CW; ++q) {
                    double g = 0.0;
#pragma unroll
                    for (int j = 0; j < ND; ++j) g = fma(dxq[k][j >> 1][j & 1], dyv[j][q], g);
                    ginc[k][q] = g;
                }
        }
        auto fetch_next = [&]() {
            const bool turn = ((t + 1) & (XW - 1)) == 0;
            if (__builtin_expect(turn, 0)) asm volatile("s_waitcnt vmcnt(0)" ::: "memory");
            if constexpr (!CARRY) {
                asm("v_add_u32 %0, 16, %0" : "+v"(a_e));
                if (((t + 1) & 7) == lam7) {
                    asm volatile("");
                    const unsigned e = (a_e + (unsigned)(Y_SLAB_PITCH - 128)) ^ 128u;
                    a_e = e - (e >= y_lim ? ring_bytes : 0u);
                }
            }
            read_y();
            if (RESET_AT_END ? tm == c_u0 : tm == c_u0m1) {
                load_x_rows(my_x + (turn ? x_rd_off ^ (unsigned)(JMAX * XSLAB) : x_rd_off));
                if constexpr (!INFLIGHT_X) {
#pragma unroll
                    for (int k = 0; k < RC; ++k) lds_rows_wait(dxq[k]);
                }
                if constexpr (RESET_AT_END) {
                    corner = 1.0;
#pragma unroll
                    for (int i = 0; i < R; ++i) left[i] = 1.0;
                }
            }
        };
        if constexpr (!CUR && MID) fetch_next();
#pragma unroll
        for (int k = 0; k < RC; ++k)
#pragma unroll
            for (int q = 0; q < CW; ++q) {
                const double g = ginc[k][q];
                if constexpr (!RBF) {
                    if (NAIVE) {
                        ca[k][q] = fma(g, 1.7320508075688772, 1.0);
                        cbm[k][q] = 1.0;
                    } else {
                        ca[k][q] = fma(g, g + 1.7320508075688772, 1.0);
                        cbm[k][q] = fma(-g, g, 1.0);
                    }
                } else if (NAIVE) {
                    ca[k][q] = fma(g, c_half, 1.0);
                    cbm[k][q] = 1.0;
                } else {
                    const double g2 = g * g;
                    ca[k][q] = fma(g2, c_12, fma(g, c_half, 1.0));
                    cbm[k][q] = fma(g2, -c_12, 1.0);
                }
            }

        double cand[RC][CW];
        double rowv[RC][S];
#pragma unroll
        for (int cc = 0; cc < S; ++cc) {
            double above = top[cc];
            double diag = cc == 0 ? corner : top[cc - 1];
#pragma unroll
            for (int rr = 0; rr < R; ++rr) {
                const double a = ca[rr >> DY][cc >> DY], b = cbm[rr >> DY][cc >> DY];
                const double k10 = left[rr];
                double v;
                if (NAIVE) v = fma(above, a, fma(k10, a, -diag));
                else v = fma(above, a, fma(k10, a, -(diag * b)));
                diag = k10;
                above = v;
                left[rr] = v;
                if ((rr & (r - 1)) == r - 1 && (cc & (r - 1)) == r - 1) cand[rr >> DY][cc >> DY] = v;
                if (EDGES && (rr & (r - 1)) == r - 1) rowv[rr >> DY][cc] = v;
            }
            bot[cc] = above;
        }
        if constexpr (RESET_AT_END) {
            asm volatile("v_mov_b64 %0, %1" : "=v"(corner) : "v"(top[S - 1]));
            if constexpr (CARRY) {
                y_off += 16u;
                if (((t + 1) & 7) == 0) {
                    const unsigned e = (y_off + (unsigned)(Y_SLAB_PITCH - 128)) ^ 128u;
                    y_off = e - (e >= ring_bytes ? ring_bytes : 0u);
                }
                asm volatile("" : "+s"(y_off));
            }
            take_top();
        } else if (!FULLWAVE) {
            corner = top[S - 1];
        }

        if (EDGES) {
            const bool pair_ok = ep_cur != nullptr;
            e_ptr = ep_cur;
            erow_at = (pair_ok && uk < erow_lim) ? uk * S : -1;
            ecol_at = (pair_ok && uk == ecol_uf) ? ecol_off : -1;
            if (!row_in_bot) {
#pragma unroll
                for (int kk = 0; kk < RC - 1; ++kk)
                    if (kk == k_f) {
#pragma unroll
                        for (int cc = 0; cc < S; ++cc) erow[cc] = rowv[kk][cc];
                    }
            }
        }

        if (__builtin_expect(CUR ? uk == my_uf : tm == c_out, 0)) {
            int pv = CUR ? psk : tq + c_kq + (tm + c_kr >= NUp ? 1 : 0);
            asm volatile("" : "+v"(pv));
            unsigned pair_u = lane_pair(pv);
            const int sA = shy_a();
            if (sA > 0 && pair_u != NOPAIR) {
                unsigned dm = prm.div_m;
                int ds = prm.div_s;
                asm volatile("" : "+s"(dm), "+s"(ds));
                const unsigned Bu = (unsigned)prm.B, qa = __umulhi(pair_u << 1, dm) >> ds, a = qa * (unsigned)G + (unsigned)grp;
                pair_u = a < (unsigned)sA ? a * Bu + (pair_u - qa * Bu) : NOPAIR;
            }
            const int64_t pair_v = (int64_t)pair_u;
            if (pair_u != NOPAIR) {
                double v = cand[0][0];
#pragma unroll
                for (int k = 0; k < RC; ++k)
#pragma unroll
                    for (int q = 0; q < CW; ++q) {
                        double cv = cand[k][q];
                        asm volatile("" : "+v"(cv));
                        if (k * CW + q == prm.sel_f) v = cv;
                    }
                if ((prm.tri & 3) == 1) {
                    const int *tab = reinterpret_cast<const int *>(prm.dYt + prm.B * (int64_t)FD * prm.Ncp);
                    const int64_t a = tab[2 * pair_v], b = tab[2 * pair_v + 1];
                    static_cast<TO *>(prm.out)[a * prm.B + b] = (TO)v;
                    static_cast<TO *>(prm.out)[b * prm.B + a] = (TO)v;
                } else {
                    static_cast<TO *>(prm.out)[pair_v] = (TO)v;
                }
            }
        }

        if constexpr (!CUR) {
            if constexpr (!MID && !RESET_AT_END) fetch_next();
            tm += 1;
            if (tm == NUp) { tm = 0; tq += 1; }
            if constexpr (RESET_AT_END) {
                asm volatile("" : "+s"(tq));
                fetch_next();
            }
        }
        if (CUR && RBF) {
            uk += 1;
            if (uk == NUp) {
                uk = 0;
                psk += 1;
                sweep_pair_is(psk);
            }
        }
        if constexpr (CUR) u += 1;
        if (CUR && ((t + 1) & 7) == lam7) {
            yslab = yslab + 1 == NSLAB ? 0 : yslab + 1;
            ypar ^= 1;
            if (u == NUp) {
                u = 0;
                ps += 1;
                if (!RBF) sweep_pair_is(ps);
            }
        }
        if (CUR && !RBF) { uk = u; psk = ps; }
        if (__builtin_expect(((t + 1) & (XW - 1)) == 0, 0)) {
            asm volatile("s_waitcnt vmcnt(0)" ::: "memory");
            if (XW == 8 || ((t + 1) & 7) == 0) issue_y();
            issue_x();
            x_rd_off ^= (unsigned)(JMAX * XSLAB);
            if (XW == 8 || ((t + 1) & 7) == 0) refresh_next();
        }
        if (AHEAD && CUR) read_y();
    }
    if constexpr (!CUR) {
        asm volatile("s_waitcnt lgkmcnt(0)" ::: "memory");
    } else if (AHEAD) {
        d2_t drain[ND];
        lds_dims_wait(drain, dyn);
    }
    if (EDGES) {
        double *const ep = e_ptr;
        if (erow_at >= 0) {
#pragma unroll
            for (int cc = 0; cc < S; ++cc) ep[erow_at + cc] = row_in_bot ? bot[cc] : erow[cc];
        }
        if (ecol_at >= 0) {
#pragma unroll
            for (int rr = 0; rr < R; ++rr) ep[ecol_at + rr] = left[rr];
        }
    }
    asm volatile("s_waitcnt vmcnt(0)" ::: "memory");
}

struct FusedPlan {
    int64_t P;
    int G, NUp, L, lag;
    size_t lds_bytes;
    int waves_per_cu;
    int rcx;
};

template <typename TO, int DY, bool NAIVE, bool FULLWAVE, bool EDGES, int KIND, int ND, int RCX = 0>
int launch_fused_nd(FusedParams prm, const FusedPlan &pl, hipStream_t s) {
    auto kern = k_fwd_fused<TO, DY, NAIVE, FULLWAVE, EDGES, KIND, ND, RCX>;
    static const int vgprs = variant_vgprs(kern, 128);
    int waves_per_cu = waves_by_vgprs(pl.waves_per_cu, vgprs);
    int64_t waves, per;
    even_share(pl.P, pl.G, (int64_t)device_cu_count() * waves_per_cu, waves, per);
    if (per < 8 && waves_per_cu >= 8) {
        static const double rate_std[4] = {1.0, 1.0, 0.70, 0.60}, rate_dbl[4] = {1.0, 1.0, EDGES ? 0.79 : 0.69, 0.62};
        const double *rate = (RCX != 0 && RCX == 2 * Tile<DY>::RC) ? rate_dbl : rate_std;
        const int64_t nsimd = (int64_t)device_cu_count() * 4;
        const int fill = pl.L - 1 + pl.lag;
        double best = 0;
        int best_q = 0;
        for (int q = 1; q <= waves_per_cu / 4 && q <= 3; ++q) {
            int64_t W = (pl.P + pl.G - 1) / pl.G;
            if (W > nsimd * q) W = nsimd * q;
            const int64_t base = pl.P / (W * pl.G), rem = pl.P - base * W * pl.G, nbig = (rem + pl.G - 1) / pl.G;
            if (base == 0) W = nbig;
            const int64_t on_simd = (W + nsimd - 1) / nsimd, big_on_simd = std::min(on_simd, (nbig + nsimd - 1) / nsimd);
            const double longest = (double)((base + (big_on_simd > 0 ? 1 : 0)) * pl.NUp + fill), shortest = (double)(base * pl.NUp + fill);
            const double all = (on_simd > big_on_simd && base > 0) ? shortest : longest;
            const double cost = all * (double)on_simd * rate[on_simd] + (longest - all) * (double)big_on_simd * rate[big_on_simd > 0 ? big_on_simd : 1];
            if (best_q == 0 || cost < best * 0.98) { best = cost; best_q = q; }
        }
        if (best_q && knobs().fused_wpc <= 0) waves_per_cu = 4 * best_q;
    }
    const int pct = knobs().fused_q_static > 0 ? (knobs().fused_q_static > 100 ? 100 : knobs().fused_q_static)
                                                : (int)cost_by_name(KIND == 1 ? "fused_static_share_rbf" : "fused_static_share_linear");
    StreamPlan sp;
    if (const int rc = plan_pair_stream(pl.P, pl.G, pl.NUp, pl.L, pl.lag, waves_per_cu, device_cu_count(), pct, prm.queue != nullptr, sp))
        return rc;
    const int64_t max_waves = (int64_t)device_cu_count() * waves_per_cu;
    waves = sp.waves;
    per = sp.per;
    prm.C0 = sp.C0; prm.n_big = sp.n_big; prm.logC = sp.logC; prm.q_first = sp.q_first;
    if (sp.queue) {
        if (hipMemsetAsync(prm.queue, 0, sizeof(unsigned long long), s) != hipSuccess) return SK_ERR_LAUNCH;
    } else {
        prm.queue = nullptr;
        const int nr = waves_per_cu / 4;
        const WaveGroup wg0 = wave_group(pl.lds_bytes, waves, knobs().fused_wpb);
        const int64_t wpr = (int64_t)device_cu_count() * wg0.wpb;
        const int64_t T = (pl.P + wpr * pl.G - 1) / (wpr * pl.G);
        if (knobs().fused_mid != 0 && waves == max_waves && waves_per_cu % 4 == 0 && nr >= 2 && nr <= 4 && wg0.wpb == 4 &&
            wpr * nr == waves && T >= (int64_t)cost_by_name("fused_mid_min_pairs_per_rank") * nr) {
            static constexpr double dflt[5][4] = {{1, 0, 0, 0}, {1, 0, 0, 0}, {0.66, 0.34, 0, 0}, {0.53, 0.30, 0.17, 0}, {0.40, 0.27, 0.19, 0.14}};
            double w[4];
            for (int r = 0; r < 4; ++r) w[r] = dflt[nr][r];
            rank_override(knobs().fused_rank_w, nr, w);
            const double fill = (double)(pl.L - 1 + pl.lag), total = (double)T * pl.NUp + nr * fill;
            int64_t used = 0, cmax = 0;
            unsigned long long pack = 0;
            bool ok = true;
            for (int r = 0; r < nr; ++r) {
                int64_t c = r + 1 < nr ? (int64_t)((w[r] * total - fill) / pl.NUp + 0.5) : T - used;
                if (c < 1 || c > 0xffff || used + c > T - (nr - 1 - r)) { ok = false; break; }
                pack |= (unsigned long long)c << (16 * r);
                cmax = c > cmax ? c : cmax;
                used += c;
            }
            if (ok && (uint64_t)T * (uint64_t)wpr * (uint64_t)pl.G < 0x7ff00000ULL) {
                prm.rk_n = nr;
                prm.rk_wpr = (int)wpr;
                prm.rk_cnt = pack;
                per = cmax;
            }
        }
    }
    if (per > 0x1fffffff / pl.NUp) return SK_ERR_UNSUPPORTED;
    prm.wg = wave_group(pl.lds_bytes, waves, knobs().fused_wpb);
    prm.PPG = (int)per;
    prm.n_steps = 0;
    const size_t lds_block = wave_group_lds(prm.wg);
    if (lds_block > 64 * 1024)
        (void)hipFuncSetAttribute((const void *)kern, hipFuncAttributeMaxDynamicSharedMemorySize, (int)lds_block);
    SK_LAUNCH(kern, dim3(wave_group_blocks(prm.wg)), dim3(WAVE * prm.wg.wpb), lds_block, s, prm);
    return check_launch();
}

constexpr int fused_rcx(int kind, int dy, int nd, bool edges, bool plain ) {
    return dy == 1 ? ((kind == 0 || nd == 4) ? 4 : 0)
         : dy == 2 ? ((edges && plain && (kind == 0 || nd == 4)) ? 2 : 0)
         : ((kind == 1 && nd == 8) ? 2 : 0);
}
constexpr int fused_nd(int dims, bool plain) { return plain && dims <= 4 ? 4 : 8; }

template <typename TO, int DY, bool NAIVE, bool FULLWAVE, bool EDGES, int KIND, int ND>
int launch_fused_v(const FusedParams &prm, const FusedPlan &pl, hipStream_t s) {
    constexpr bool PLAIN = !NAIVE && sizeof(TO) == 8;
    constexpr int RCX = fused_rcx(KIND, DY, ND, EDGES, PLAIN);
    if (pl.rcx != RCX) return SK_ERR_UNSUPPORTED;
    if constexpr (FULLWAVE && RCX != 0 && RCX == 2 * Tile<DY>::RC) return SK_ERR_UNSUPPORTED;
    else if constexpr (KIND == 1 && DY == 0 && ND == 8 && EDGES && !PLAIN) return SK_ERR_UNSUPPORTED;
    else return launch_fused_nd<TO, DY, NAIVE, FULLWAVE, EDGES, KIND, ND, RCX>(prm, pl, s);
}

template <typename TO, int DY, bool NAIVE, bool FULLWAVE, bool EDGES, int KIND>
int launch_fused_e(const FusedParams &prm, const FusedPlan &pl, hipStream_t s) {
    if constexpr (!NAIVE && sizeof(TO) == 8) {
        if (prm.dims <= 4) return launch_fused_v<TO, DY, NAIVE, FULLWAVE, EDGES, KIND, 4>(prm, pl, s);
    }
    return launch_fused_v<TO, DY, NAIVE, FULLWAVE, EDGES, KIND, 8>(prm, pl, s);
}

template <typename TO, int DY, bool NAIVE, bool FULLWAVE, int KIND>
int launch_fused_one(const FusedParams &prm, const FusedPlan &pl, hipStream_t s) {
    if constexpr (sizeof(TO) == 8) {
        if (prm.edges) return launch_fused_e<TO, DY, NAIVE, FULLWAVE, true, KIND>(prm, pl, s);
    }
    if (prm.edges) return SK_ERR_UNSUPPORTED;
    return launch_fused_e<TO, DY, NAIVE, FULLWAVE, false, KIND>(prm, pl, s);
}

template <typename TO, int DY, int KIND>
int launch_fused_dy(const FusedParams &prm, const FusedPlan &pl, hipStream_t s) {
    const bool full = prm.logL == 6;
    if (prm.naive)
        return full ? launch_fused_one<TO, DY, true, true, KIND>(prm, pl, s) : launch_fused_one<TO, DY, true, false, KIND>(prm, pl, s);
    return full ? launch_fused_one<TO, DY, false, true, KIND>(prm, pl, s) : launch_fused_one<TO, DY, false, false, KIND>(prm, pl, s);
}

template <typename TO, int KIND>
int launch_fwd_fused(const double *dXr, const double *dYt, int64_t A, int64_t B, int Mrows, int Ncp, int D, const Geom &g,
                     double inv_sigma, TO *out, double *strip_edges, void *queue, hipStream_t s, int tri = 0, const int64_t *loss = nullptr) {
    if (tri == 1 && (strip_edges || A != B || g.P != A * (A + 1) / 2)) return SK_ERR_UNSUPPORTED;
    if (tri == 2 && (!loss || B <= 0 || loss[0] < 0 || loss[1] != A || loss[0] + loss[1] > B || A > B ||
                     g.P != A * B + (loss[0] > 1 ? loss[0] * (loss[0] - 1) / 2 : 0)))
        return SK_ERR_BAD_ARG;
    if (tri == 2 && (A > 0x7fff || loss[0] > 0x7fff || A * B >= 0x7ff00000LL)) return SK_ERR_UNSUPPORTED;
    const int DY = g.dyadic;
    if (DY > 2 || D < 1 || D > FD) return SK_ERR_UNSUPPORTED;
    const bool four_dim = !g.naive && sizeof(TO) == 8 && D <= 4;
    const bool rbf0_two_rows = KIND == 1 && DY == 0 && !four_dim;
    if (rbf0_two_rows && strip_edges && (g.naive || sizeof(TO) != 8)) return SK_ERR_UNSUPPORTED;
    const int nd_v = fused_nd(D, !g.naive && sizeof(TO) == 8);
    const int rcx = fused_rcx(KIND, DY, nd_v, strip_edges != nullptr, !g.naive && sizeof(TO) == 8);
    const int RC = rcx ? rcx : (DY == 0 ? 4 : DY == 1 ? 2 : 1);
    const bool doubled = rcx == 2 * (DY == 0 ? 4 : DY == 1 ? 2 : 1);
    int logL_fixed = 0;
    if (rbf0_two_rows && strip_edges) {
        const Strip st = strip_geom(rbf_edge_geom(g), 8);
        if (!st.ok || st.nb != 1 || st.logL > 5) return SK_ERR_UNSUPPORTED;
        logL_fixed = st.logL + 1;
    }
    const int nd = nd_v;
    OneBandGeom og;
    OneBandShape sh{};
    sh.kind = KIND, sh.Mc = g.Mc, sh.Nc = g.Nc, sh.Mrows = Mrows, sh.Ncp = Ncp, sh.RC = RC, sh.nd = nd;
    sh.edges = strip_edges != nullptr, sh.A = A, sh.B = B, sh.P = g.P, sh.tri = tri, sh.logL_fixed = logL_fixed;
    if (const int rc = one_band_geometry(sh, og)) return rc;
    const int NUp = og.NUp, logL = og.logL, L = og.L;
    const bool shy = og.shy;
    const size_t lds_bytes = og.lds_bytes;
    const int64_t n_pos = og.n_pos;

    int waves_per_cu = (int)((160 * 1024) / lds_bytes);
    const int wpc_env = knobs().fused_wpc;
    const int cap = wpc_env > 0 ? 16 : (DY == 0 ? 8 : (DY == 2 && nd == 4) ? 16 : 12);
    if (waves_per_cu > cap) waves_per_cu = cap;
    if (wpc_env > 0) waves_per_cu = waves_per_cu < wpc_env ? waves_per_cu : wpc_env;
    else if (waves_per_cu > 4) waves_per_cu &= ~3;
    if (waves_per_cu < 1) waves_per_cu = 1;
    const FusedPlan pl{n_pos, og.GY, NUp, L, KIND == 1 ? 2 : 0, lds_bytes, waves_per_cu, rcx};

    FusedParams prm;
    prm.dXr = dXr; prm.dYt = dYt; prm.out = out; prm.edges = strip_edges; prm.P = n_pos; prm.B = B;
    prm.Mrows = Mrows; prm.Ncp = Ncp; prm.Mc = g.Mc; prm.Nc = g.Nc; prm.NUp = NUp; prm.logL = logL;
    prm.inv_sigma = inv_sigma;
    prm.dims = D;
    prm.rk_n = 0; prm.rk_wpr = 1; prm.rk_cnt = 0;
    prm.tri = tri == 2 ? (2 | ((int)A << 2) | ((int)loss[0] << 17)) : tri;
    prm.queue = (unsigned long long *)queue;
    prm.e_NUp = NUp;
    prm.e_L = L;
    if (strip_edges) {
        const Strip st = strip_geom(KIND == 1 ? rbf_edge_geom(g) : g, 8);
        if (!st.ok || st.nb != 1 || (st.RC != RC && !rbf0_two_rows && !doubled) || ((1 << st.logL) * st.RC) % RC) return SK_ERR_UNSUPPORTED;
        prm.e_NUp = st.NUp;
        prm.e_L = ((1 << st.logL) * st.RC) / RC;
        if (prm.e_L > L) return SK_ERR_UNSUPPORTED;
    }
    prm.u_f = (g.Nc - 1) / 2;
    prm.lam_f = ((g.Mc - 1) / RC) % L;
    prm.sel_f = ((g.Mc - 1) % RC) * 2 + (g.Nc - 1) % 2;
    prm.naive = g.naive;
    prm.shy_A = shy ? (int)A : 0;
    prm.div_m = 0; prm.div_s = 0;
    if (B > 0) {
        if (B >= 0x7ff00000LL || div_magic((uint32_t)B, prm.div_m, prm.div_s)) return SK_ERR_UNSUPPORTED;
    }
    if ((int64_t)Ncp * 64 >= 0x100000000LL) return SK_ERR_UNSUPPORTED;
    switch (DY) {
        case 0: return launch_fused_dy<TO, 0, KIND>(prm, pl, s);
        case 1: return launch_fused_dy<TO, 1, KIND>(prm, pl, s);
        default: return launch_fused_dy<TO, 2, KIND>(prm, pl, s);
    }
}

}

extern "C" int sk_pair_div_magic(int64_t B, uint32_t *mul, int *shift) {
    if (!mul || !shift || B < 1 || B >= 0x80000000LL) return SK_ERR_BAD_ARG;
    unsigned m = 0;
    int sh = 0;
    if (div_magic((uint32_t)B, m, sh)) return SK_ERR_BAD_ARG;
    *mul = m;
    *shift = sh;
    return SK_OK;
}

template <typename TO>
int launch_fwd_fused_linear(const double *dXr, const double *dYt, int64_t A, int64_t B, int Mrows, int Ncp, int D, const Geom &g,
                            TO *out, double *strip_edges, void *queue, hipStream_t s, int tri, const int64_t *loss) {
    return launch_fwd_fused<TO, 0>(dXr, dYt, A, B, Mrows, Ncp, D, g, 0.0, out, strip_edges, queue, s, tri, loss);
}
template <typename TO>
int launch_fwd_fused_rbf(const double *Xr, const double *Yt, int64_t A, int64_t B, int Mrows, int Ncp, int D, const Geom &g,
                         double inv_sigma, TO *out, double *strip_edges, void *queue, hipStream_t s, int tri, const int64_t *loss) {
    return launch_fwd_fused<TO, 1>(Xr, Yt, A, B, Mrows, Ncp, D, g, inv_sigma, out, strip_edges, queue, s, tri, loss);
}

template int launch_fwd_fused_linear<double>(const double *, const double *, int64_t, int64_t, int, int, int, const Geom &, double *,
                                             double *, void *, hipStream_t, int, const int64_t *);
template int launch_fwd_fused_linear<float>(const double *, const double *, int64_t, int64_t, int, int, int, const Geom &, float *,
                                            double *, void *, hipStream_t, int, const int64_t *);
template int launch_fwd_fused_rbf<double>(const double *, const double *, int64_t, int64_t, int, int, int, const Geom &, double, double *,
                                          double *, void *, hipStream_t, int, const int64_t *);
template int launch_fwd_fused_rbf<float>(const double *, const double *, int64_t, int64_t, int, int, int, const Geom &, double, float *,
                                         double *, void *, hipStream_t, int, const int64_t *);

}
```

Baseline: 71.85 million entries/s.

## Deal fused forward Gram positions per row-block with per-row queues and stealing

Replaces the single global work queue of the fused one-band forward solver with per-Gram-row-block counters. Each wave gets a static chunk within one row-block, so consecutive positions share the same X path and X rows can stay resident (KEEPX). Once its own row-block is exhausted, a wave steals from up to a bounded number of following row-blocks. This is meant to improve X data reuse and cut global atomic contention, at the cost of more queue memory, more counters to zero, and possible load imbalance or extra probe round trips near the end.

```diff
diff --git a/include/sigkernel_amd.h b/include/sigkernel_amd.h
--- a/include/sigkernel_amd.h
+++ b/include/sigkernel_amd.h
@@ -156,6 +156,17 @@
                          int dyadic, int scheme, double inv_sigma, double *out_final, void *queue, void *stream);
 int sk_solve_fwd_rbf_f32(const double *Xr, const double *Yt, int64_t A, int64_t B, int Mrows, int Mc, int Nc, int Ncp, int D,
                          int dyadic, int scheme, double inv_sigma, float *out_final, void *queue, void *stream);
+int sk_solve_fwd_linear_rows_f64(const double *dXr, const double *dYt, int64_t A, int64_t B, int Mrows, int Mc, int Nc, int Ncp, int D,
+                                 int dyadic, int scheme, double *out_final, void *queue, int64_t queue_words, void *stream);
+int sk_solve_fwd_linear_rows_f32(const double *dXr, const double *dYt, int64_t A, int64_t B, int Mrows, int Mc, int Nc, int Ncp, int D,
+                                 int dyadic, int scheme, float *out_final, void *queue, int64_t queue_words, void *stream);
+int sk_solve_fwd_rbf_rows_f64(const double *Xr, const double *Yt, int64_t A, int64_t B, int Mrows, int Mc, int Nc, int Ncp, int D,
+                              int dyadic, int scheme, double inv_sigma, double *out_final, void *queue, int64_t queue_words, void *stream);
+int sk_solve_fwd_rbf_rows_f32(const double *Xr, const double *Yt, int64_t A, int64_t B, int Mrows, int Mc, int Nc, int Ncp, int D,
+                              int dyadic, int scheme, double inv_sigma, float *out_final, void *queue, int64_t queue_words, void *stream);
+int sk_plan_row_dealing(int64_t A, int64_t B, int G, int NUp, int L, int lag, int waves_per_cu, int n_cu, int pct, int64_t queue_words,
+                        int64_t *plan, int64_t waves_cap, int64_t *static_first, int64_t *static_end, int64_t queues_cap,
+                        int64_t *queue_first, int64_t *queue_end);
 int sk_solve_prefix_linear_f64(const double *dXr, const double *dYt, int64_t A, int64_t B, int Mrows, int Mc, int Nc, int Ncp, int D,
                                int dyadic, int scheme, double *out, int64_t ldo, void *queue, void *stream);
 int sk_solve_prefix_linear_f32(const double *dXr, const double *dYt, int64_t A, int64_t B, int Mrows, int Mc, int Nc, int Ncp, int D,
diff --git a/sigkernel_amd/_lib.py b/sigkernel_amd/_lib.py
--- a/sigkernel_amd/_lib.py
+++ b/sigkernel_amd/_lib.py
@@ -76,6 +76,11 @@
     "sk_solve_fwd_linear_f32": (_int, [_vp, _vp, _i64, _i64, _int, _int, _int, _int, _int, _int, _int, _vp, _vp, _vp]),
     "sk_solve_fwd_rbf_f64": (_int, [_vp, _vp, _i64, _i64, _int, _int, _int, _int, _int, _int, _int, ctypes.c_double, _vp, _vp, _vp]),
     "sk_solve_fwd_rbf_f32": (_int, [_vp, _vp, _i64, _i64, _int, _int, _int, _int, _int, _int, _int, ctypes.c_double, _vp, _vp, _vp]),
+    "sk_solve_fwd_linear_rows_f64": (_int, [_vp, _vp, _i64, _i64, _int, _int, _int, _int, _int, _int, _int, _vp, _vp, _i64, _vp]),
+    "sk_solve_fwd_linear_rows_f32": (_int, [_vp, _vp, _i64, _i64, _int, _int, _int, _int, _int, _int, _int, _vp, _vp, _i64, _vp]),
+    "sk_solve_fwd_rbf_rows_f64": (_int, [_vp, _vp, _i64, _i64, _int, _int, _int, _int, _int, _int, _int, ctypes.c_double, _vp, _vp, _i64, _vp]),
+    "sk_solve_fwd_rbf_rows_f32": (_int, [_vp, _vp, _i64, _i64, _int, _int, _int, _int, _int, _int, _int, ctypes.c_double, _vp, _vp, _i64, _vp]),
+    "sk_plan_row_dealing": (_int, [_i64, _i64, _int, _int, _int, _int, _int, _int, _int, _i64, _vp, _i64, _vp, _vp, _i64, _vp, _vp]),
     "sk_solve_prefix_linear_f64": (_int, [_vp, _vp, _i64, _i64, _int, _int, _int, _int, _int, _int, _int, _vp, _i64, _vp, _vp]),
     "sk_solve_prefix_linear_f32": (_int, [_vp, _vp, _i64, _i64, _int, _int, _int, _int, _int, _int, _int, _vp, _i64, _vp, _vp]),
     "sk_solve_prefix_rbf_f64": (_int, [_vp, _vp, _i64, _i64, _int, _int, _int, _int, _int, _int, _int, ctypes.c_double, _vp, _i64, _vp, _vp]),
@@ -339,8 +344,13 @@
     return None if t is None else t.data_ptr()
 
 
-def _queue(dev, pairs=1 << 30):
-    return torch.empty(8, dtype=torch.int64, device=dev) if pairs >= 16384 else None
+def _queue(dev, pairs=1 << 30, words=8):
+    return torch.empty(max(8, int(words)), dtype=torch.int64, device=dev) if pairs >= 16384 else None
+
+
+def _row_queue(dev, A, B, gram):
+    n = max(8, A // 2 + 1) if gram else 8
+    return _queue(dev, A * B if gram else A, n), n
 
 
 def _prep_paths(X, diff, dim_major, scale, rows, fd=8):
@@ -473,8 +483,9 @@
                         return out, edges
                     if rc != 2:
                         _check(rc, "sk_solve_fwd_linear_edges")
-            fn = getattr(lib, "sk_solve_fwd_linear_" + _suffix(X))
-            rc = fn(_ptr(dXr), _ptr(dYt), A, B if gram else 0, Mrows, Mc, Nc, Ncp, D, int(dyadic), scheme, _ptr(out), _ptr(_queue(dev, A * B if gram else A)), _stream(X))
+            fn = getattr(lib, "sk_solve_fwd_linear_rows_" + _suffix(X))
+            queue, words = _row_queue(dev, A, B, gram)
+            rc = fn(_ptr(dXr), _ptr(dYt), A, B if gram else 0, Mrows, Mc, Nc, Ncp, D, int(dyadic), scheme, _ptr(out), _ptr(queue), words, _stream(X))
         if rc == 2:
             return None
         _check(rc, "sk_solve_fwd_linear")
@@ -506,9 +517,10 @@
                         return out, edges
                     if rc != 2:
                         _check(rc, "sk_solve_fwd_rbf_edges")
-            fn = getattr(lib, "sk_solve_fwd_rbf_" + _suffix(X))
+            fn = getattr(lib, "sk_solve_fwd_rbf_rows_" + _suffix(X))
+            queue, words = _row_queue(dev, A, B, gram)
             rc = fn(_ptr(Xr), _ptr(Yt), A, B if gram else 0, Mrows, Mc, Nc, Ncp, D, int(dyadic), scheme, 1.0 / float(sigma),
-                    _ptr(out), _ptr(_queue(dev, A * B if gram else A)), _stream(X))
+                    _ptr(out), _ptr(queue), words, _stream(X))
         if rc == 2:
             return None
         _check(rc, "sk_solve_fwd_rbf")
diff --git a/sigkernel_amd/csrc/sk_abi.hip b/sigkernel_amd/csrc/sk_abi.hip
--- a/sigkernel_amd/csrc/sk_abi.hip
+++ b/sigkernel_amd/csrc/sk_abi.hip
@@ -239,6 +239,7 @@
     k.deriv_wpc = knob_int("SK_DERIV_WPC"); k.deriv_wpb = knob_int("SK_DERIV_WPB");
     k.fused_wpc = knob_int("SK_FUSED_WPC"); k.fused_wpb = knob_int("SK_FUSED_WPB"); k.fused_q_static = knob_int("SK_FUSED_Q_STATIC");
     k.fused_mid = getenv("SK_FUSED_MID") ? knob_int("SK_FUSED_MID") : 1;
+    k.fused_rows = getenv("SK_FUSED_ROWS") ? knob_int("SK_FUSED_ROWS") : 1; k.fused_row_steal = knob_int("SK_FUSED_ROW_STEAL");
     k.fusedmb_wpc = knob_int("SK_FUSEDMB_WPC"); k.fusedmb_wpb = knob_int("SK_FUSEDMB_WPB"); k.fusedmb_q_static = knob_int("SK_FUSEDMB_Q_STATIC");
     k.fusedmb_split = getenv("SK_FUSEDMB_SPLIT") ? knob_int("SK_FUSEDMB_SPLIT") : 1;
     k.fusedmb_lead = knob_int("SK_FUSEDMB_LEAD");
@@ -457,40 +458,60 @@
     return solve_fwd<float>(inc_c, ld, P, Mc, Nc, dyadic, scheme, flags, out_final, out_grid, out_edges, stream);
 }
 
+int sk_solve_fwd_linear_rows_f64(const double *dXr, const double *dYt, int64_t A, int64_t B, int Mrows, int Mc, int Nc, int Ncp, int D,
+                                 int dyadic, int scheme, double *out_final, void *queue, int64_t queue_words, void *stream) {
+    if (D < 1 || !dXr || !dYt || !out_final || A < 0 || B < 0 || Mc < 1 || Nc < 1 || dyadic < 0 || dyadic > 16) return SK_ERR_BAD_ARG;
+    if (scheme != SK_SCHEME_DEFAULT && scheme != SK_SCHEME_NAIVE) return SK_ERR_BAD_ARG;
+    if (A == 0) return SK_OK;
+    const Geom g = make_geom(B > 0 ? A * B : A, Mc, Nc, dyadic, scheme);
+    if (queue && queue_words < 1) return SK_ERR_BAD_ARG;
+    return launch_fwd_fused_linear<double>(dXr, dYt, A, B, Mrows, Ncp, D, g, out_final, nullptr, queue, (hipStream_t)stream, 0, nullptr, queue_words);
+}
 int sk_solve_fwd_linear_f64(const double *dXr, const double *dYt, int64_t A, int64_t B, int Mrows, int Mc, int Nc, int Ncp, int D,
                             int dyadic, int scheme, double *out_final, void *queue, void *stream) {
+    return sk_solve_fwd_linear_rows_f64(dXr, dYt, A, B, Mrows, Mc, Nc, Ncp, D, dyadic, scheme, out_final, queue, 1, stream);
+}
+int sk_solve_fwd_linear_rows_f32(const double *dXr, const double *dYt, int64_t A, int64_t B, int Mrows, int Mc, int Nc, int Ncp, int D,
+                                 int dyadic, int scheme, float *out_final, void *queue, int64_t queue_words, void *stream) {
     if (D < 1 || !dXr || !dYt || !out_final || A < 0 || B < 0 || Mc < 1 || Nc < 1 || dyadic < 0 || dyadic > 16) return SK_ERR_BAD_ARG;
     if (scheme != SK_SCHEME_DEFAULT && scheme != SK_SCHEME_NAIVE) return SK_ERR_BAD_ARG;
     if (A == 0) return SK_OK;
     const Geom g = make_geom(B > 0 ? A * B : A, Mc, Nc, dyadic, scheme);
-    return launch_fwd_fused_linear<double>(dXr, dYt, A, B, Mrows, Ncp, D, g, out_final, nullptr, queue, (hipStream_t)stream);
+    if (queue && queue_words < 1) return SK_ERR_BAD_ARG;
+    return launch_fwd_fused_linear<float>(dXr, dYt, A, B, Mrows, Ncp, D, g, out_final, nullptr, queue, (hipStream_t)stream, 0, nullptr, queue_words);
 }
 int sk_solve_fwd_linear_f32(const double *dXr, const double *dYt, int64_t A, int64_t B, int Mrows, int Mc, int Nc, int Ncp, int D,
                             int dyadic, int scheme, float *out_final, void *queue, void *stream) {
-    if (D < 1 || !dXr || !dYt || !out_final || A < 0 || B < 0 || Mc < 1 || Nc < 1 || dyadic < 0 || dyadic > 16) return SK_ERR_BAD_ARG;
-    if (scheme != SK_SCHEME_DEFAULT && scheme != SK_SCHEME_NAIVE) return SK_ERR_BAD_ARG;
-    if (A == 0) return SK_OK;
-    const Geom g = make_geom(B > 0 ? A * B : A, Mc, Nc, dyadic, scheme);
-    return launch_fwd_fused_linear<float>(dXr, dYt, A, B, Mrows, Ncp, D, g, out_final, nullptr, queue, (hipStream_t)stream);
-}
-
+    return sk_solve_fwd_linear_rows_f32(dXr, dYt, A, B, Mrows, Mc, Nc, Ncp, D, dyadic, scheme, out_final, queue, 1, stream);
+}
+
+int sk_solve_fwd_rbf_rows_f64(const double *Xr, const double *Yt, int64_t A, int64_t B, int Mrows, int Mc, int Nc, int Ncp, int D, int dyadic,
+                              int scheme, double inv_sigma, double *out_final, void *queue, int64_t queue_words, void *stream) {
+    if (D < 1 || !Xr || !Yt || !out_final || A < 0 || B < 0 || Mc < 1 || Nc < 1 || dyadic < 0 || dyadic > 16) return SK_ERR_BAD_ARG;
+    if (scheme != SK_SCHEME_DEFAULT && scheme != SK_SCHEME_NAIVE) return SK_ERR_BAD_ARG;
+    if (!(inv_sigma > 0.0) || !(inv_sigma < 1e300)) return SK_ERR_BAD_ARG;
+    if (A == 0) return SK_OK;
+    const Geom g = make_geom(B > 0 ? A * B : A, Mc, Nc, dyadic, scheme);
+    if (queue && queue_words < 1) return SK_ERR_BAD_ARG;
+    return launch_fwd_fused_rbf<double>(Xr, Yt, A, B, Mrows, Ncp, D, g, inv_sigma, out_final, nullptr, queue, (hipStream_t)stream, 0, nullptr, queue_words);
+}
 int sk_solve_fwd_rbf_f64(const double *Xr, const double *Yt, int64_t A, int64_t B, int Mrows, int Mc, int Nc, int Ncp, int D, int dyadic,
                          int scheme, double inv_sigma, double *out_final, void *queue, void *stream) {
+    return sk_solve_fwd_rbf_rows_f64(Xr, Yt, A, B, Mrows, Mc, Nc, Ncp, D, dyadic, scheme, inv_sigma, out_final, queue, 1, stream);
+}
+int sk_solve_fwd_rbf_rows_f32(const double *Xr, const double *Yt, int64_t A, int64_t B, int Mrows, int Mc, int Nc, int Ncp, int D, int dyadic,
+                              int scheme, double inv_sigma, float *out_final, void *queue, int64_t queue_words, void *stream) {
     if (D < 1 || !Xr || !Yt || !out_final || A < 0 || B < 0 || Mc < 1 || Nc < 1 || dyadic < 0 || dyadic > 16) return SK_ERR_BAD_ARG;
     if (scheme != SK_SCHEME_DEFAULT && scheme != SK_SCHEME_NAIVE) return SK_ERR_BAD_ARG;
     if (!(inv_sigma > 0.0) || !(inv_sigma < 1e300)) return SK_ERR_BAD_ARG;
     if (A == 0) return SK_OK;
     const Geom g = make_geom(B > 0 ? A * B : A, Mc, Nc, dyadic, scheme);
-    return launch_fwd_fused_rbf<double>(Xr, Yt, A, B, Mrows, Ncp, D, g, inv_sigma, out_final, nullptr, queue, (hipStream_t)stream);
+    if (queue && queue_words < 1) return SK_ERR_BAD_ARG;
+    return launch_fwd_fused_rbf<float>(Xr, Yt, A, B, Mrows, Ncp, D, g, inv_sigma, out_final, nullptr, queue, (hipStream_t)stream, 0, nullptr, queue_words);
 }
 int sk_solve_fwd_rbf_f32(const double *Xr, const double *Yt, int64_t A, int64_t B, int Mrows, int Mc, int Nc, int Ncp, int D, int dyadic,
                          int scheme, double inv_sigma, float *out_final, void *queue, void *stream) {
-    if (D < 1 || !Xr || !Yt || !out_final || A < 0 || B < 0 || Mc < 1 || Nc < 1 || dyadic < 0 || dyadic > 16) return SK_ERR_BAD_ARG;
-    if (scheme != SK_SCHEME_DEFAULT && scheme != SK_SCHEME_NAIVE) return SK_ERR_BAD_ARG;
-    if (!(inv_sigma > 0.0) || !(inv_sigma < 1e300)) return SK_ERR_BAD_ARG;
-    if (A == 0) return SK_OK;
-    const Geom g = make_geom(B > 0 ? A * B : A, Mc, Nc, dyadic, scheme);
-    return launch_fwd_fused_rbf<float>(Xr, Yt, A, B, Mrows, Ncp, D, g, inv_sigma, out_final, nullptr, queue, (hipStream_t)stream);
+    return sk_solve_fwd_rbf_rows_f32(Xr, Yt, A, B, Mrows, Mc, Nc, Ncp, D, dyadic, scheme, inv_sigma, out_final, queue, 1, stream);
 }
 
 int sk_solve_prefix_linear_f64(const double *dXr, const double *dYt, int64_t A, int64_t B, int Mrows, int Mc, int Nc, int Ncp, int D,
diff --git a/sigkernel_amd/csrc/sk_internal.h b/sigkernel_amd/csrc/sk_internal.h
--- a/sigkernel_amd/csrc/sk_internal.h
+++ b/sigkernel_amd/csrc/sk_internal.h
@@ -15,6 +15,7 @@
     int derivf_wpc, derivf_wpb, derivf_noshift;
     int deriv_wpc, deriv_wpb;
     int fused_wpc, fused_wpb, fused_q_static, fused_mid;
+    int fused_rows, fused_row_steal;
     int fusedmb_wpc, fusedmb_wpb, fusedmb_q_static, fusedmb_split, fusedmb_lead;
     int prefix_store;
     RankW rank_w, wave_rank_w, adj_rank_w, adjf_rank_w, adjr_rank_w, deriv_rank_w, fused_rank_w, fusedmb_rank_w;
@@ -136,11 +137,13 @@
 
 template <typename TO>
 int launch_fwd_fused_linear(const double *dXr, const double *dYt, int64_t A, int64_t B, int Mrows, int Ncp, int D, const Geom &g,
-                            TO *out, double *strip_edges, void *queue, hipStream_t s, int tri = 0, const int64_t *loss = nullptr);
+                            TO *out, double *strip_edges, void *queue, hipStream_t s, int tri = 0, const int64_t *loss = nullptr,
+                            int64_t queue_words = 1);
 
 template <typename TO>
 int launch_fwd_fused_rbf(const double *Xr, const double *Yt, int64_t A, int64_t B, int Mrows, int Ncp, int D, const Geom &g,
-                         double inv_sigma, TO *out, double *strip_edges, void *queue, hipStream_t s, int tri = 0, const int64_t *loss = nullptr);
+                         double inv_sigma, TO *out, double *strip_edges, void *queue, hipStream_t s, int tri = 0, const int64_t *loss = nullptr,
+                         int64_t queue_words = 1);
 
 template <typename TO>
 int launch_fwd_prefix(int kind, const double *dXr, const double *dYt, int64_t A, int64_t B, int Mrows, int Ncp, int D, const Geom &g,
diff --git a/sigkernel_amd/csrc/sk_pair_stream.h b/sigkernel_amd/csrc/sk_pair_stream.h
--- a/sigkernel_amd/csrc/sk_pair_stream.h
+++ b/sigkernel_amd/csrc/sk_pair_stream.h
@@ -138,6 +138,10 @@
     int64_t q_first;
     int C0, n_big, logC;
     bool queue;
+    int row_wprb;
+    int row_rem;
+    int row_q0;
+    int64_t n_rb;
 };
 inline int plan_pair_stream(int64_t P, int G, int NUp, int L, int lag, int waves_per_cu, int n_cu, int pct, bool has_queue, StreamPlan &o) {
     const int64_t max_waves = (int64_t)n_cu * waves_per_cu;
@@ -161,7 +165,25 @@
         if (base == 0) o.waves = o.n_big;
         o.q_first = P;
     }
+    o.row_wprb = 0; o.row_rem = 0; o.row_q0 = 0; o.n_rb = 0;
     return SK_OK;
+}
+
+inline void plan_row_dealing(int64_t P, int64_t row_len, int NUp, int L, int64_t queue_words, StreamPlan &o) {
+    if (!o.queue || row_len <= 0 || P <= 0 || P % row_len != 0 || L > NUp) return;
+    const int64_t n_rb = P / row_len;
+    if (n_rb > queue_words || o.waves % n_rb != 0 || row_len > 0x3fffffff) return;
+    const int64_t wprb = o.waves / n_rb;
+    if (wprb < 1 || wprb > 0x7fff) return;
+    int64_t c0 = o.C0;
+    if (c0 * wprb > row_len) c0 = row_len / wprb;
+    const int64_t CQ = (int64_t)1 << o.logC;
+    o.C0 = (int)c0;
+    o.row_wprb = (int)wprb;
+    o.row_rem = (int)((row_len - wprb * c0) % CQ);
+    o.row_q0 = (int)(wprb * c0) + o.row_rem;
+    o.n_rb = n_rb;
+    o.q_first = 0;
 }
 
 }
diff --git a/sigkernel_amd/csrc/sk_route.hip b/sigkernel_amd/csrc/sk_route.hip
--- a/sigkernel_amd/csrc/sk_route.hip
+++ b/sigkernel_amd/csrc/sk_route.hip
@@ -73,6 +73,10 @@
     {"fused_static_share_rbf", 20,
      "... the RBF variants (longer macro-steps, a draw costs less of one): 2048 x 2048 pairs, dyadic 2: 52.0 ms at 35, 50.9 at 20, 50.6 at 3; "
      "512 / 1024 paths: 3.41 -> 3.34, 13.0 -> 12.8 ms; C4 335.6 -> 334.5 (profiles/r05_qstatic.txt)"},
+    {"fused_row_steal", 8,
+     "row-local dealing of the one-band fused forward (plan_row_dealing): looks at the counters of the following 64 Gram row-blocks a wave "
+     "may take, once its own row-block is used up, to find one that has positions left, before it ends (SK_FUSED_ROW_STEAL overrides; a look "
+     "is one load's round trip, every position is handed out whatever the bound): profiles/fused_fwd_row_dealing.txt"},
     {"mb_split_max_resident_share", 0.5,
      "few pairs of long paths: bands of a pair on several waves when the pairs fill at most this share of the resident waves (r05: 16 x 16 pairs "
      "of 4096 points 18.7 -> 4.7 ms; 32 x 32 pairs of 700 points 2.18 -> 1.96 ms)"},
diff --git a/sigkernel_amd/csrc/sk_wave_fused.hip b/sigkernel_amd/csrc/sk_wave_fused.hip
--- a/sigkernel_amd/csrc/sk_wave_fused.hip
+++ b/sigkernel_amd/csrc/sk_wave_fused.hip
@@ -28,6 +28,8 @@
     int shy_A;
     unsigned div_m;
     int div_s;
+    int row_nrb, row_q0;
+    int row_wprb, row_rem, row_steal;
 };
 template <int N>
 __device__ __forceinline__ void lds_read_units(d2_t (&v)[N], unsigned addr);
@@ -122,6 +124,7 @@
     const int lam7 = lam & 7;
     constexpr bool CUR = EDGES;
     constexpr bool MID = false;
+    constexpr bool KEEPX = !EDGES && !FULLWAVE;
     constexpr bool INFLIGHT_X = !(KIND == 1 && DY == 0 && ND == 8 && RCX == 0);
     int tm = 0, tq = 0;
     int c_u0 = lam % NUp, c_uk0 = (lam + LAG) % NUp;
@@ -149,6 +152,15 @@
         const unsigned used = (unsigned)(below & 0xffffu) + (unsigned)((below >> 16) & 0xffffu) + (unsigned)((below >> 32) & 0xffffu);
         cb0_ = (used * (unsigned)prm.rk_wpr + (unsigned)((w32 - rr * prm.rk_wpr) * c0_)) * (unsigned)GY;
     }
+    int row_home = 0;
+    if constexpr (KEEPX) {
+        if (prm.row_nrb > 0) {
+            const int j = w32 / prm.row_nrb;
+            row_home = w32 - j * prm.row_nrb;
+            c0_ = prm.C0 + (j == prm.row_wprb - 1 ? prm.row_rem : 0);
+            cb0_ = (unsigned)row_home * (unsigned)prm.B + (unsigned)(j * prm.C0);
+        }
+    }
     const int C0 = __builtin_amdgcn_readfirstlane(c0_), logC = prm.logC, CQ = 1 << logC;
     unsigned cb0 = (unsigned)__builtin_amdgcn_readfirstlane((int)cb0_), cb1 = NOPAIR, cb2 = NOPAIR, cb3 = NOPAIR;
     int have = 1;
@@ -180,12 +192,57 @@
         int left;
         return stream_pair_left(grp, i, left);
     };
+    int pos_ab = 0;
+    if constexpr (KEEPX) pos_ab = lane == 16 ? row_home : lane == 17 ? prm.row_steal : 0;
     auto ensure = [&](int f) __attribute__((always_inline)) {
         int off;
         const int kf = chunk_of(f, off);
         while (have <= kf) {
             unsigned b = NOPAIR;
-            if (prm.queue && t_end == 0x7fffffff) {
+            bool by_row = false;
+            if constexpr (KEEPX) {
+                int nrb = prm.row_nrb;
+                asm volatile("" : "+s"(nrb));
+                if (nrb > 0 && t_end == 0x7fffffff) {
+                    by_row = true;
+                    int rb = __builtin_amdgcn_readlane(pos_ab, 16), more = __builtin_amdgcn_readlane(pos_ab, 17);
+                    const unsigned Bu = (unsigned)prm.B;
+                    for (;;) {
+                        unsigned v = 0;
+                        if (lane == 0) v = (unsigned)atomicAdd(prm.queue + rb, (unsigned long long)CQ);
+                        const unsigned o = (unsigned)prm.row_q0 + (unsigned)__builtin_amdgcn_readfirstlane((int)v);
+                        if (o < Bu) {
+                            b = (unsigned)rb * Bu + o;
+                            break;
+                        }
+                        int cand = -1;
+                        const int reach = nrb - 1 < WAVE ? nrb - 1 : WAVE;
+                        while (more > 0 && cand < 0) {
+                            more -= 1;
+                            int idx = rb + 1 + lane;
+                            idx -= idx >= nrb ? nrb : 0;
+                            unsigned c = 0;
+                            if (lane < reach)
+                                c = __hip_atomic_load(reinterpret_cast<const unsigned *>(prm.queue + idx), __ATOMIC_RELAXED, __HIP_MEMORY_SCOPE_AGENT);
+                            const unsigned long long open =
+                                __builtin_amdgcn_ballot_w64(lane < reach && c < Bu && (unsigned)prm.row_q0 + c < Bu);
+                            if (open) {
+                                cand = rb + 1 + (int)__builtin_ctzll(open);
+                                cand -= cand >= nrb ? nrb : 0;
+                            } else if (reach < WAVE) {
+                                more = 0;
+                            } else {
+                                rb += WAVE;
+                                rb -= rb >= nrb ? nrb : 0;
+                            }
+                        }
+                        if (cand < 0) break;
+                        rb = cand;
+                    }
+                    pos_ab = lane == 16 ? rb : lane == 17 ? more : pos_ab;
+                }
+            }
+            if (!by_row && prm.queue && t_end == 0x7fffffff) {
                 unsigned long long v = 0;
                 if (lane == 0) v = atomicAdd(prm.queue, (unsigned long long)((shy_a() > 0 ? 1 : G) * CQ));
                 const unsigned long long q = (unsigned long long)prm.q_first +
@@ -238,7 +295,6 @@
         return (int)(want_b ? p - q * (unsigned)prm.B : q);
     };
     constexpr bool PARK = !(EDGES && ((KIND == 0 && DY == 0 && ND == 4 && !FULLWAVE) || (KIND == 1 && DY == 2 && ND == 8 && FULLWAVE)));
-    int pos_ab = 0;
     auto dma_lane = [&]() __attribute__((always_inline)) -> int {
         int l = lane;
         if constexpr (!PARK) asm volatile("" : "+v"(l));
@@ -272,10 +328,14 @@
         if (y_u0 == NUp) { y_u0 = 0; y_pi += 1; }
     };
     int x_q0 = 0, x_lam0 = 0, x_slot = 0;
+    int x_new = 1;
     auto issue_x = [&]() __attribute__((always_inline)) {
         if constexpr (!PARK) pos_ab = 0;
         const int ln = dma_lane();
+        if constexpr (KEEPX) x_new = __builtin_amdgcn_readlane(pos_ab, 18);
         if (!PARK || x_lam0 == 0) {
+            int prev0 = 0;
+            if constexpr (KEEPX) prev0 = __builtin_amdgcn_readlane(pos_ab, ((x_q0 - 1) & (NS - 1)) * G);
             ensure(x_q0);
             const int sA = shy_a();
             for (int jd = 0; jd < (PARK ? 1 : JMAX); ++jd) {
@@ -296,8 +356,13 @@
                     pos_ab = lane == at + g ? a : pos_ab;
                 }
             }
-        }
-        for (int j = 0; j < JMAX; ++j) {
+            if constexpr (KEEPX) {
+                const int now0 = __builtin_amdgcn_readlane(pos_ab, (x_q0 & (NS - 1)) * G);
+                x_new = (sA > 0 && JMAX == 1 && x_q0 > 0 && now0 == prev0) ? 0 : 1;
+                pos_ab = lane == 18 ? x_new : pos_ab;
+            }
+        }
+        for (int j = 0; j < (KEEPX && !x_new ? 0 : JMAX); ++j) {
             const int lamj = x_lam0 + j * NUp;
             if (lamj >= L) break;
             const int at = ((x_q0 - j) & (NS - 1)) * G;
@@ -415,9 +480,11 @@
     static_assert(X_SLOTS == 2, "x_rd_off toggles between two slots");
     issue_y();
     issue_x();
+    if constexpr (KEEPX) x_rd_off = (unsigned)x_new;
     asm volatile("s_waitcnt vmcnt(0)" ::: "memory");
     issue_y();
     issue_x();
+    if constexpr (KEEPX) x_rd_off |= (unsigned)x_new << 1;
     refresh_next();
     sweep_pair_is(psk);
     refresh_next();
@@ -569,10 +636,20 @@
             }
             read_y();
             if (RESET_AT_END ? tm == c_u0 : tm == c_u0m1) {
-                load_x_rows(my_x + (turn ? x_rd_off ^ (unsigned)(JMAX * XSLAB) : x_rd_off));
-                if constexpr (!INFLIGHT_X) {
-#pragma unroll
-                    for (int k = 0; k < RC; ++k) lds_rows_wait(dxq[k]);
+                if constexpr (KEEPX) {
+                    if (x_rd_off & (turn ? 2u : 1u)) {
+                        load_x_rows(my_x + ((turn ? x_rd_off ^ (unsigned)(JMAX * XSLAB) : x_rd_off) & ~3u));
+                        if constexpr (!INFLIGHT_X) {
+#pragma unroll
+                            for (int k = 0; k < RC; ++k) lds_rows_wait(dxq[k]);
+                        }
+                    }
+                } else {
+                    load_x_rows(my_x + (turn ? x_rd_off ^ (unsigned)(JMAX * XSLAB) : x_rd_off));
+                    if constexpr (!INFLIGHT_X) {
+#pragma unroll
+                        for (int k = 0; k < RC; ++k) lds_rows_wait(dxq[k]);
+                    }
                 }
                 if constexpr (RESET_AT_END) {
                     corner = 1.0;
@@ -723,6 +800,8 @@
             if (XW == 8 || ((t + 1) & 7) == 0) issue_y();
             issue_x();
             x_rd_off ^= (unsigned)(JMAX * XSLAB);
+            if constexpr (KEEPX)
+                x_rd_off = (x_rd_off & ~3u) | ((x_rd_off >> 1) & 1u) | ((unsigned)x_new << 1);
             if (XW == 8 || ((t + 1) & 7) == 0) refresh_next();
         }
         if (AHEAD && CUR) read_y();
@@ -753,6 +832,8 @@
     size_t lds_bytes;
     int waves_per_cu;
     int rcx;
+    int64_t row_len;
+    int64_t queue_words;
 };
 
 template <typename TO, int DY, bool NAIVE, bool FULLWAVE, bool EDGES, int KIND, int ND, int RCX = 0>
@@ -790,9 +871,16 @@
     const int64_t max_waves = (int64_t)device_cu_count() * waves_per_cu;
     waves = sp.waves;
     per = sp.per;
+    if (knobs().fused_rows != 0 && !EDGES && !FULLWAVE) plan_row_dealing(pl.P, pl.row_len, pl.NUp, pl.L, pl.queue_words, sp);
     prm.C0 = sp.C0; prm.n_big = sp.n_big; prm.logC = sp.logC; prm.q_first = sp.q_first;
+    prm.row_nrb = sp.row_wprb > 0 ? (int)sp.n_rb : 0; prm.row_q0 = sp.row_q0; prm.row_wprb = sp.row_wprb; prm.row_rem = sp.row_rem;
+    {
+        const int steal = knobs().fused_row_steal > 0 ? knobs().fused_row_steal : (int)cost_by_name("fused_row_steal");
+        prm.row_steal = steal < 1024 ? steal : 1024;
+    }
     if (sp.queue) {
-        if (hipMemsetAsync(prm.queue, 0, sizeof(unsigned long long), s) != hipSuccess) return SK_ERR_LAUNCH;
+        const size_t counters = prm.row_nrb > 0 ? (size_t)prm.row_nrb : 1;
+        if (hipMemsetAsync(prm.queue, 0, counters * sizeof(unsigned long long), s) != hipSuccess) return SK_ERR_LAUNCH;
     } else {
         prm.queue = nullptr;
         const int nr = waves_per_cu / 4;
@@ -879,7 +967,8 @@
 
 template <typename TO, int KIND>
 int launch_fwd_fused(const double *dXr, const double *dYt, int64_t A, int64_t B, int Mrows, int Ncp, int D, const Geom &g,
-                     double inv_sigma, TO *out, double *strip_edges, void *queue, hipStream_t s, int tri = 0, const int64_t *loss = nullptr) {
+                     double inv_sigma, TO *out, double *strip_edges, void *queue, hipStream_t s, int tri = 0, const int64_t *loss = nullptr,
+                     int64_t queue_words = 1) {
     if (tri == 1 && (strip_edges || A != B || g.P != A * (A + 1) / 2)) return SK_ERR_UNSUPPORTED;
     if (tri == 2 && (!loss || B <= 0 || loss[0] < 0 || loss[1] != A || loss[0] + loss[1] > B || A > B ||
                      g.P != A * B + (loss[0] > 1 ? loss[0] * (loss[0] - 1) / 2 : 0)))
@@ -918,7 +1007,7 @@
     if (wpc_env > 0) waves_per_cu = waves_per_cu < wpc_env ? waves_per_cu : wpc_env;
     else if (waves_per_cu > 4) waves_per_cu &= ~3;
     if (waves_per_cu < 1) waves_per_cu = 1;
-    const FusedPlan pl{n_pos, og.GY, NUp, L, KIND == 1 ? 2 : 0, lds_bytes, waves_per_cu, rcx};
+    const FusedPlan pl{n_pos, og.GY, NUp, L, KIND == 1 ? 2 : 0, lds_bytes, waves_per_cu, rcx, shy ? B : 0, queue_words};
 
     FusedParams prm;
     prm.dXr = dXr; prm.dYt = dYt; prm.out = out; prm.edges = strip_edges; prm.P = n_pos; prm.B = B;
@@ -966,24 +1055,68 @@
     return SK_OK;
 }
 
+extern "C" int sk_plan_row_dealing(int64_t A, int64_t B, int G, int NUp, int L, int lag, int waves_per_cu, int n_cu, int pct,
+                                   int64_t queue_words, int64_t *plan, int64_t waves_cap, int64_t *static_first, int64_t *static_end,
+                                   int64_t queues_cap, int64_t *queue_first, int64_t *queue_end) {
+    if (!plan || A < 1 || B < 1 || G < 1 || G > 8 || NUp < 8 || (NUp & 7) || L < 8 || L > 64 || lag < 0 || waves_per_cu < 1 || n_cu < 1 ||
+        pct < 1 || pct > 100 || queue_words < 0 || (static_first == nullptr) != (static_end == nullptr) ||
+        (queue_first == nullptr) != (queue_end == nullptr))
+        return SK_ERR_BAD_ARG;
+    const int64_t n_pos = G >= 2 ? (A + G - 1) / G * B : A * B;
+    StreamPlan sp;
+    if (const int rc = plan_pair_stream(n_pos, 1, NUp, L, lag, waves_per_cu, n_cu, pct, queue_words > 0, sp)) return rc;
+    plan_row_dealing(n_pos, G >= 2 ? B : 0, NUp, L, queue_words, sp);
+    const bool rows = sp.row_wprb > 0;
+    const int64_t CQ = (int64_t)1 << sp.logC, n_q = rows ? sp.n_rb : (sp.queue ? 1 : 0);
+    const int64_t fields[13] = {rows ? 1 : 0, sp.waves, sp.per, sp.q_first, sp.C0, sp.n_big, sp.logC, sp.queue ? 1 : 0,
+                                sp.row_wprb, rows ? sp.n_rb : 0, sp.row_q0, sp.row_rem, n_q};
+    for (int i = 0; i < 13; ++i) plan[i] = fields[i];
+    if (static_first) {
+        if (sp.waves > waves_cap) return SK_ERR_BAD_ARG;
+        for (int64_t w = 0; w < sp.waves; ++w) {
+            int64_t first, count;
+            if (rows) {
+                const int64_t j = w / sp.n_rb, h = w - j * sp.n_rb;
+                first = h * B + j * sp.C0;
+                count = sp.C0 + (j == sp.row_wprb - 1 ? sp.row_rem : 0);
+            } else {
+                first = w * sp.C0 + (w < sp.n_big ? w : sp.n_big);
+                count = sp.C0 + (w < sp.n_big ? 1 : 0);
+            }
+            static_first[w] = first < n_pos ? first : n_pos;
+            static_end[w] = first + count < n_pos ? first + count : n_pos;
+        }
+    }
+    if (queue_first) {
+        if (n_q > queues_cap) return SK_ERR_BAD_ARG;
+        for (int64_t h = 0; h < n_q; ++h) {
+            queue_first[h] = rows ? h * B + sp.row_q0 : sp.q_first;
+            queue_end[h] = rows ? (h + 1) * B : n_pos;
+        }
+        if (rows && (B - sp.row_q0) % CQ != 0) return SK_ERR_LAUNCH;
+    }
+    return SK_OK;
+}
+
 template <typename TO>
 int launch_fwd_fused_linear(const double *dXr, const double *dYt, int64_t A, int64_t B, int Mrows, int Ncp, int D, const Geom &g,
-                            TO *out, double *strip_edges, void *queue, hipStream_t s, int tri, const int64_t *loss) {
-    return launch_fwd_fused<TO, 0>(dXr, dYt, A, B, Mrows, Ncp, D, g, 0.0, out, strip_edges, queue, s, tri, loss);
+                            TO *out, double *strip_edges, void *queue, hipStream_t s, int tri, const int64_t *loss, int64_t queue_words) {
+    return launch_fwd_fused<TO, 0>(dXr, dYt, A, B, Mrows, Ncp, D, g, 0.0, out, strip_edges, queue, s, tri, loss, queue_words);
 }
 template <typename TO>
 int launch_fwd_fused_rbf(const double *Xr, const double *Yt, int64_t A, int64_t B, int Mrows, int Ncp, int D, const Geom &g,
-                         double inv_sigma, TO *out, double *strip_edges, void *queue, hipStream_t s, int tri, const int64_t *loss) {
-    return launch_fwd_fused<TO, 1>(Xr, Yt, A, B, Mrows, Ncp, D, g, inv_sigma, out, strip_edges, queue, s, tri, loss);
+                         double inv_sigma, TO *out, double *strip_edges, void *queue, hipStream_t s, int tri, const int64_t *loss,
+                         int64_t queue_words) {
+    return launch_fwd_fused<TO, 1>(Xr, Yt, A, B, Mrows, Ncp, D, g, inv_sigma, out, strip_edges, queue, s, tri, loss, queue_words);
 }
 
 template int launch_fwd_fused_linear<double>(const double *, const double *, int64_t, int64_t, int, int, int, const Geom &, double *,
-                                             double *, void *, hipStream_t, int, const int64_t *);
+                                             double *, void *, hipStream_t, int, const int64_t *, int64_t);
 template int launch_fwd_fused_linear<float>(const double *, const double *, int64_t, int64_t, int, int, int, const Geom &, float *,
-                                            double *, void *, hipStream_t, int, const int64_t *);
+                                            double *, void *, hipStream_t, int, const int64_t *, int64_t);
 template int launch_fwd_fused_rbf<double>(const double *, const double *, int64_t, int64_t, int, int, int, const Geom &, double, double *,
-                                          double *, void *, hipStream_t, int, const int64_t *);
+                                          double *, void *, hipStream_t, int, const int64_t *, int64_t);
 template int launch_fwd_fused_rbf<float>(const double *, const double *, int64_t, int64_t, int, int, int, const Geom &, double, float *,
-                                         double *, void *, hipStream_t, int, const int64_t *);
-
-}
+                                         double *, void *, hipStream_t, int, const int64_t *, int64_t);
+
+}
```

Result: faster. 72.82 million entries/s (median of 6 runs) (+1.3%).
